# Samsonboadi/Image_to_pointCloud

Hardware: NVIDIA B200
Metric: depth_to_point_cloud_throughput (higher is better)
Workload: dtype f64

## Files before the change

image_to_pointcloud_b200/csrc/d2pc_device.cuh:

```cuda
#ifndef D2PC_DEVICE_CUH_
#define D2PC_DEVICE_CUH_

#include <cuda_runtime.h>
#include <stdint.h>

#include "d2pc_math.h"

namespace d2pc {

constexpr int kSampleSize = 8192;
constexpr int kSample2Size = 4096;
constexpr int kSortCap = 16384;
constexpr int kSelBits = 12;
constexpr int kScanThreads = 256;
constexpr int kScanPerThread = 32;
constexpr int kScanTile = kScanThreads * kScanPerThread;
constexpr int kSelThreads = 1024;
constexpr int kSelectThreads = 512;
constexpr int kEmitThreads = 256;
constexpr int kEmitPerThread = 4;
constexpr int kEmitTile = kEmitThreads * kEmitPerThread;
constexpr int kFbTargets = 4;
constexpr uint32_t kCandDivisor = 16;

struct Geom {
  int32_t H, W, C, h, w, step;
  int32_t nu, nv;
  uint32_t P;
  uint32_t N;
  uint32_t D;
  int32_t native;
  double scale_x, scale_y;
};

inline Geom make_geom(const D2pcConfig &c) {
  Geom g;
  g.H = c.img_h; g.W = c.img_w; g.C = c.img_c; g.h = c.dep_h; g.w = c.dep_w; g.step = c.step;
  g.nu = (c.img_w + c.step - 1) / c.step;
  g.nv = (c.img_h + c.step - 1) / c.step;
  g.P = (uint32_t)c.img_h * (uint32_t)c.img_w;
  g.N = (uint32_t)g.nu * (uint32_t)g.nv;
  g.D = (uint32_t)c.dep_h * (uint32_t)c.dep_w;
  g.native = (c.dep_h == c.img_h && c.dep_w == c.img_w) ? 1 : 0;
  g.scale_x = (double)c.dep_w / (double)c.img_w;
  g.scale_y = (double)c.dep_h / (double)c.img_h;
  return g;
}

struct __align__(256) FrameState {
  uint32_t brL[2], brU[2];
  uint32_t sample_ok;
  uint32_t below[2];
  uint32_t above1;
  uint32_t eqL[2];
  uint32_t inside[2];
  uint32_t eqU[2];
  uint32_t n_nonfinite, n_nan;
  alignas(8) uint32_t nqueue[2];
  uint32_t min_key, max_key;
  uint32_t sel_key[4];
  uint32_t sel_fail;
  uint32_t sel_done;
  uint32_t fb_prefix[kFbTargets];
  uint32_t fb_rank[kFbTargets];
  uint32_t fb_active;
  uint32_t fb_any_nan;
  int32_t mask_mode;
  float mask_lo, mask_hi;
  uint32_t emit_count;
  uint32_t bounds_min[3], bounds_max[3];
  alignas(128) NormParams norm;
  int32_t status;
};
static_assert(sizeof(NormParams) + 4 <= 128, "norm + status must share one 128-byte line");
constexpr int kStatusWord = (int)(sizeof(NormParams) / 4);

constexpr uint32_t kSelBins = 4096, kSelListCap = 1024;
struct __align__(256) SelShared {
  uint32_t counts[2][8];
  uint32_t scan_done;
  uint32_t a_done[2], c_done[2];
  uint32_t bin_ready[2];
  uint32_t bin[2][2], base[2][2], need[2][2], want[2][2], shared_bin[2], key[2][2];
  uint32_t mcount[2][2], mmin[2][2], mmax[2][2];
  uint32_t pad_[7];
  uint32_t members[2][2][kSelListCap];
  uint32_t hist[2][kSelBins];
};

struct __align__(8) TapEntry {
  int32_t i0c;
  float t;
};

constexpr int kSchedQueues = 32;
constexpr size_t kSchedBytes = 128 * (kSchedQueues + 1);

struct WsLayout {
  size_t state_off, cand_off, tile_off, fbhist_off, tap_off, sched_off, sel_off, resized_off, total;
  uint32_t cand_cap;
  uint32_t emit_tiles;
};

inline size_t align_up(size_t x, size_t a) { return (x + a - 1) / a * a; }

inline WsLayout make_layout(const D2pcConfig &c) {
  Geom g = make_geom(c);
  WsLayout L;
  uint32_t cap = g.P / kCandDivisor + 1;
  uint32_t small = g.P < (uint32_t)kSortCap ? g.P : (uint32_t)kSortCap;
  if (cap < small) cap = small;
  cap = (cap + 3u) & ~3u;
  L.cand_cap = cap;
  L.emit_tiles = (g.N + kEmitTile - 1) / kEmitTile;
  size_t off = 0;
  L.state_off = off;  off = align_up(off + sizeof(FrameState) * (size_t)c.batch, 256);
  L.cand_off = off;   off = align_up(off + (size_t)c.batch * 2 * cap * sizeof(uint32_t), 256);
  L.tile_off = off;   off = align_up(off + (size_t)c.batch * L.emit_tiles * sizeof(unsigned long long), 256);
  L.fbhist_off = off; off = align_up(off + (size_t)c.batch * kFbTargets * 256 * sizeof(uint32_t), 256);
  L.tap_off = off;    off = align_up(off + ((size_t)c.img_w + (size_t)c.img_h) * sizeof(TapEntry), 256);
  L.sched_off = off;  off = align_up(off + kSchedBytes + (size_t)c.batch * 64, 256);
  L.sel_off = off;    off = align_up(off + (size_t)c.batch * sizeof(SelShared), 256);
  L.resized_off = off;
  if (!g.native) off = align_up(off + (size_t)c.batch * g.P * sizeof(float), 256);
  L.total = off;
  return L;
}

struct KParams {
  Geom g;
  int32_t batch;
  const float *depth;
  FrameState *state;
  uint32_t *cand;
  unsigned long long *tile_state;
  uint32_t *fb_hist;
  const TapEntry *xtab, *ytab;
  SelShared *sel;
  uint32_t *sched;
  float *resized;
  uint32_t cand_cap, emit_tiles;
  int32_t force_fallback;
  int32_t hints;
};

constexpr int kHintScanKeep = 1;
constexpr int kHintEmitDepthFirst = 2;
constexpr int kHintStreamFirst = 4;
constexpr int kHintResizedKeep = 8;
constexpr int kHintPipeline = 15;

inline KParams make_kparams(const D2pcConfig &c, const float *d_depth, void *ws) {
  KParams k;
  WsLayout L = make_layout(c);
  char *base = (char *)ws;
  k.g = make_geom(c);
  k.batch = c.batch;
  k.depth = d_depth;
  k.state = (FrameState *)(base + L.state_off);
  k.cand = (uint32_t *)(base + L.cand_off);
  k.tile_state = (unsigned long long *)(base + L.tile_off);
  k.fb_hist = (uint32_t *)(base + L.fbhist_off);
  k.xtab = (const TapEntry *)(base + L.tap_off);
  k.ytab = k.xtab + c.img_w;
  k.sched = (uint32_t *)(base + L.sched_off);
  k.sel = (SelShared *)(base + L.sel_off);
  k.resized = k.g.native ? nullptr : (float *)(base + L.resized_off);
  k.cand_cap = L.cand_cap;
  k.emit_tiles = L.emit_tiles;
  k.force_fallback = c.force_fallback;
  k.hints = 0;
  return k;
}

inline KParams per_pixel_view(const KParams &kp) {
  KParams v = kp;
  if (!kp.g.native) {
    v.depth = kp.resized;
    v.g.D = kp.g.P;
    v.g.h = kp.g.H;
    v.g.w = kp.g.W;
    v.g.native = 1;
  }
  return v;
}

inline KParams slice_kparams(const KParams &kp, int b0, int nb, int ring_slot) {
  KParams s = kp;
  s.batch = nb;
  s.depth = kp.depth + (size_t)b0 * kp.g.D;
  s.state = kp.state + b0;
  s.cand = kp.cand + (size_t)b0 * 2 * kp.cand_cap;
  s.tile_state = kp.tile_state + (size_t)b0 * kp.emit_tiles;
  s.fb_hist = kp.fb_hist + (size_t)b0 * kFbTargets * 256;
  s.sel = kp.sel + b0;
  if (kp.resized) s.resized = kp.resized + (size_t)(ring_slot >= 0 ? ring_slot : b0) * kp.g.P;
  return s;
}

struct EmitArgs {
  const uint8_t *bgr;
  float *xyz, *rgb;
  uint32_t *count;
  PixelConsts pc;
  int32_t use_z, drop_nf, want_bounds;
  float z_min, z_max;
  uint32_t frame0;
};

int validate_config(const D2pcConfig *cfg);
int check_workspace(const D2pcConfig *cfg, const void *ws, size_t ws_bytes);
int stats_prepare();
int taps_launch(const KParams &kp, cudaStream_t st);
constexpr int kStatsSample = 1, kStatsScan = 2, kStatsSelect = 4, kStatsScanSelect = kStatsScan | kStatsSelect;
int stats_launch(KParams kp, cudaStream_t st, int phases);
int status_launch(const KParams &kp, int32_t *d_status, int32_t *d_any, cudaStream_t st);
EmitArgs make_emit_args(const D2pcConfig &cfg, const uint8_t *d_bgr, float *d_xyz, float *d_rgb, uint32_t *d_count);
EmitArgs slice_emit_args(const EmitArgs &ea, const Geom &g, int b0);
int emit_init_launch(const KParams &kp, cudaStream_t st);
int bounds_export_launch(const KParams &kp, float *d_bounds, cudaStream_t st);
int emit_validate(const D2pcConfig *cfg, const float *d_depth, const uint8_t *d_bgr, void *d_workspace,
                  size_t workspace_bytes, float *d_xyz, float *d_rgb, uint32_t *d_count, float *d_bounds);
int emit_launch(const D2pcConfig &cfg, const KParams &kp, const EmitArgs &ea, float *d_bounds, cudaStream_t st,
                int32_t smooth_k, const double *h_kernel, void *d_scratch);
int record_cuda_error(cudaError_t e);

#define D2PC_CHECK_LAUNCH()                                  \
  do {                                                       \
    cudaError_t e__ = cudaGetLastError();                    \
    if (e__ != cudaSuccess) return record_cuda_error(e__);   \
  } while (0)

#if defined(__CUDACC__)
__device__ __forceinline__ float4 ldg_stream_f4(const float *p) {
  float4 r;
  asm volatile("ld.global.nc.L1::no_allocate.v4.f32 {%0,%1,%2,%3}, [%4];"
               : "=f"(r.x), "=f"(r.y), "=f"(r.z), "=f"(r.w) : "l"(p));
  return r;
}
__device__ __forceinline__ uint64_t l2_policy(bool first, bool last) {
  uint64_t pf, pl, pn;
  asm("createpolicy.fractional.L2::evict_first.b64 %0, 1.0;" : "=l"(pf));
  asm("createpolicy.fractional.L2::evict_last.b64 %0, 1.0;" : "=l"(pl));
  asm("createpolicy.fractional.L2::evict_normal.b64 %0, 1.0;" : "=l"(pn));
  return first ? pf : (last ? pl : pn);
}
__device__ __forceinline__ float4 ldg_f4_pol(const float *p, uint64_t pol) {
  float4 r;
  asm volatile("ld.global.nc.L1::no_allocate.L2::cache_hint.v4.f32 {%0,%1,%2,%3}, [%4], %5;"
               : "=f"(r.x), "=f"(r.y), "=f"(r.z), "=f"(r.w) : "l"(p), "l"(pol));
  return r;
}
__device__ __forceinline__ uint32_t ldg_u32_pol(const void *p, uint64_t pol) {
  uint32_t r;
  asm volatile("ld.global.nc.L1::no_allocate.L2::cache_hint.u32 %0, [%1], %2;" : "=r"(r) : "l"(p), "l"(pol));
  return r;
}
__device__ __forceinline__ void stg_f4_pol(float *p, float4 v, uint64_t pol) {
  asm volatile("st.global.L2::cache_hint.v4.f32 [%0], {%1,%2,%3,%4}, %5;"
               :: "l"(p), "f"(v.x), "f"(v.y), "f"(v.z), "f"(v.w), "l"(pol) : "memory");
}
__device__ __forceinline__ void bulk_store_pol(void *gdst, uint32_t smem_addr, uint32_t bytes, uint64_t pol) {
  asm volatile("cp.async.bulk.global.shared::cta.bulk_group.L2::cache_hint [%0], [%1], %2, %3;"
               :: "l"(gdst), "r"(smem_addr), "r"(bytes), "l"(pol) : "memory");
}
__device__ __forceinline__ uint32_t ldg_stream_u32(const void *p) {
  uint32_t r;
  asm volatile("ld.global.nc.L1::no_allocate.u32 %0, [%1];" : "=r"(r) : "l"(p));
  return r;
}
__device__ __forceinline__ void stg_f1_pol(float *p, float v, uint64_t pol) {
  asm volatile("st.global.L2::cache_hint.f32 [%0], %1, %2;" :: "l"(p), "f"(v), "l"(pol) : "memory");
}
__device__ __forceinline__ void stg_stream_f4(float *p, float4 v) {
  asm volatile("st.global.cs.v4.f32 [%0], {%1,%2,%3,%4};"
               :: "l"(p), "f"(v.x), "f"(v.y), "f"(v.z), "f"(v.w) : "memory");
}
__device__ __forceinline__ void stg_stream_f1(float *p, float v) {
  asm volatile("st.global.cs.f32 [%0], %1;" :: "l"(p), "f"(v) : "memory");
}

__device__ __forceinline__ uint32_t warp_sum(uint32_t v) {
#pragma unroll
  for (int o = 16; o > 0; o >>= 1) v += __shfl_xor_sync(0xffffffffu, v, o);
  return v;
}
__device__ __forceinline__ uint32_t warp_min(uint32_t v) {
#pragma unroll
  for (int o = 16; o > 0; o >>= 1) v = min(v, __shfl_xor_sync(0xffffffffu, v, o));
  return v;
}
__device__ __forceinline__ uint32_t warp_max(uint32_t v) {
#pragma unroll
  for (int o = 16; o > 0; o >>= 1) v = max(v, __shfl_xor_sync(0xffffffffu, v, o));
  return v;
}

__device__ __forceinline__ void block_bitonic_sort(uint32_t *s, uint32_t n) {
  const uint32_t half = n >> 1;
  for (uint32_t k = 2; k <= n; k <<= 1) {
    for (uint32_t j = k >> 1; j > 0; j >>= 1) {
      for (uint32_t i = threadIdx.x; i < half; i += blockDim.x) {
        uint32_t a = ((i & ~(j - 1)) << 1) | (i & (j - 1));
        uint32_t b = a | j;
        uint32_t x = s[a], y = s[b];
        bool up = (a & k) == 0;
        if ((x > y) == up) { s[a] = y; s[b] = x; }
      }
      __syncthreads();
    }
  }
}

template <int T, int NBLOG, typename ForEach>
__device__ __forceinline__ bool block_hist_select(ForEach for_each, uint32_t lo0, uint32_t hi0,
                                                  const uint32_t (&rank)[T], uint32_t (&out)[T],
                                                  uint32_t *s_hist, uint32_t *s_res) {
  constexpr uint32_t NB = 1u << NBLOG;
  const int tid = threadIdx.x, nthr = blockDim.x;
  const int lane = tid & 31, warp = tid >> 5, nwarp = nthr >> 5;
  uint32_t lo[T], span[T], base[T];
  bool done[T];
#pragma unroll
  for (int t = 0; t < T; ++t) { lo[t] = lo0; span[t] = hi0 - lo0; base[t] = 0; done[t] = false; out[t] = 0; }
  bool shared_range = true, ok = true;
  uint32_t *s_warp = s_res + 2 * T;
  for (int level = 0; level < 6; ++level) {
    bool all_done = true;
#pragma unroll
    for (int t = 0; t < T; ++t) all_done = all_done && done[t];
    if (all_done) break;
    int shift[T];
#pragma unroll
    for (int t = 0; t < T; ++t) {
      const int bits = span[t] ? 32 - __clz(span[t]) : 0;
      shift[t] = bits > NBLOG ? bits - NBLOG : 0;
    }
    const int nh = shared_range ? 1 : T;
    for (uint32_t i = tid; i < (uint32_t)nh * NB; i += nthr) s_hist[i] = 0u;
    if (tid < 2 * T) s_res[tid] = 0xFFFFFFFFu;
    __syncthreads();
    if (shared_range) {
      for_each([&](uint32_t key) {
        const uint32_t d = key - lo[0];
        if (d <= span[0]) atomicAdd(&s_hist[d >> shift[0]], 1u);
      });
    } else {
      for_each([&](uint32_t key) {
#pragma unroll
        for (int t = 0; t < T; ++t) {
          const uint32_t d = key - lo[t];
          if (!done[t] && d <= span[t]) atomicAdd(&s_hist[t * NB + (d >> shift[t])], 1u);
        }
      });
    }
    __syncthreads();
    for (int h = 0; h < nh; ++h) {
      if (!shared_range && done[h]) continue;
      const uint32_t *hist = s_hist + (size_t)h * NB;
      constexpr int PER = 4;
      uint32_t carry = 0;
      for (uint32_t chunk = 0; chunk < NB; chunk += (uint32_t)nthr * PER) {
        const uint32_t b0 = chunk + (uint32_t)tid * PER;
        uint32_t c[PER], sum = 0;
#pragma unroll
        for (int i = 0; i < PER; ++i) { c[i] = (b0 + i < NB) ? hist[b0 + i] : 0u; sum += c[i]; }
        uint32_t incl = sum;
#pragma unroll
        for (int d = 1; d < 32; d <<= 1) {
          uint32_t y = __shfl_up_sync(0xffffffffu, incl, d);
          if (lane >= d) incl += y;
        }
        if (lane == 31) s_warp[warp] = incl;
        __syncthreads();
        uint32_t woff = 0, total = 0;
        for (int w = 0; w < nwarp; ++w) { const uint32_t x = s_warp[w]; if (w < warp) woff += x; total += x; }
        uint32_t pref = carry + woff + incl - sum;
#pragma unroll
        for (int i = 0; i < PER; ++i) {
#pragma unroll
          for (int t = 0; t < T; ++t) {
            const bool mine = shared_range ? !done[t] : (t == h);
            const uint32_t r = rank[t] - base[t];
            if (mine && c[i] && pref <= r && r < pref + c[i]) { s_res[2 * t] = b0 + i; s_res[2 * t + 1] = pref; }
          }
          pref += c[i];
        }
        carry += total;
        __syncthreads();
      }
    }
    __syncthreads();
#pragma unroll
    for (int t = 0; t < T; ++t) {
      if (done[t]) continue;
      const uint32_t bin = s_res[2 * t], pref = s_res[2 * t + 1];
      if (bin == 0xFFFFFFFFu) { ok = false; done[t] = true; continue; }
      base[t] += pref;
      lo[t] += bin << shift[t];
      span[t] = shift[t] ? ((1u << shift[t]) - 1u) : 0u;
      if (shift[t] == 0) { done[t] = true; out[t] = lo[t]; }
    }
    shared_range = false;
    __syncthreads();
  }
  return ok;
}

constexpr int kFastBinsLog = 12;
constexpr uint32_t kFastBins = 1u << kFastBinsLog;
constexpr uint32_t kFastListCap = 1024;

__device__ __forceinline__ int fast_shift(uint32_t span) {
  const int bits = span ? 32 - __clz(span) : 0;
  return bits > kFastBinsLog ? bits - kFastBinsLog : 0;
}

template <int T, bool GLOBAL = false>
__device__ __forceinline__ void block_locate(const uint32_t *s_hist, const uint32_t (&rank)[T], const bool (&want)[T],
                                             uint32_t (&bin)[T], uint32_t (&base)[T], uint32_t *s_warp,
                                             uint32_t *s_res) {
  const int tid = threadIdx.x, lane = tid & 31, warp = tid >> 5, nwarp = blockDim.x >> 5;
  const int per = (int)(kFastBins / blockDim.x);
  if (tid < 2 * T) s_res[tid] = 0xFFFFFFFFu;
  const uint32_t b0 = (uint32_t)tid * (uint32_t)per;
  uint32_t sum = 0;
  for (int i = 0; i < per; i += 4) {
    const uint4 c = GLOBAL ? __ldcg(reinterpret_cast<const uint4 *>(s_hist + b0 + i))
                           : *reinterpret_cast<const uint4 *>(s_hist + b0 + i);
    sum += c.x + c.y + c.z + c.w;
  }
  uint32_t incl = sum;
#pragma unroll
  for (int d = 1; d < 32; d <<= 1) {
    const uint32_t y = __shfl_up_sync(0xffffffffu, incl, d);
    if (lane >= d) incl += y;
  }
  if (lane == 31) s_warp[warp] = incl;
  __syncthreads();
  if (warp == 0) {
    const uint32_t x = lane < nwarp ? s_warp[lane] : 0u;
    uint32_t in2 = x;
#pragma unroll
    for (int d = 1; d < 32; d <<= 1) {
      const uint32_t y = __shfl_up_sync(0xffffffffu, in2, d);
      if (lane >= d) in2 += y;
    }
    __syncwarp();
    s_warp[lane] = in2 - x;
  }
  __syncthreads();
  uint32_t pref = s_warp[warp] + incl - sum;
  bool mine = false;
#pragma unroll
  for (int t = 0; t < T; ++t) mine = mine || (want[t] && sum && pref <= rank[t] && rank[t] < pref + sum);
  if (mine) {
    for (int i = 0; i < per; ++i) {
      const uint32_t c = GLOBAL ? __ldcg(s_hist + b0 + i) : s_hist[b0 + i];
#pragma unroll
      for (int t = 0; t < T; ++t)
        if (want[t] && c && pref <= rank[t] && rank[t] < pref + c) { s_res[2 * t] = b0 + i; s_res[2 * t + 1] = pref; }
      pref += c;
    }
  }
  __syncthreads();
#pragma unroll
  for (int t = 0; t < T; ++t) { bin[t] = s_res[2 * t]; base[t] = s_res[2 * t + 1]; }
}

__device__ __forceinline__ void block_pick(const uint32_t *list, uint32_t n, uint32_t r, uint32_t *s_out) {
  for (uint32_t i = threadIdx.x; i < n; i += blockDim.x) {
    const uint32_t k = list[i];
    uint32_t smaller = 0, equal = 0;
    for (uint32_t j = 0; j < n; ++j) {
      const uint32_t x = list[j];
      smaller += x < k ? 1u : 0u;
      equal += x == k ? 1u : 0u;
    }
    if (smaller <= r && r < smaller + equal) *s_out = k;
  }
}

__device__ __forceinline__ uint32_t hash_u32(uint32_t x) {
  x ^= x >> 16; x *= 0x7feb352du; x ^= x >> 15; x *= 0x846ca68bu; x ^= x >> 16;
  return x;
}

__device__ __forceinline__ float bilinear_taps(const float *src, int32_t src_w, TapEntry tx, TapEntry ty) {
  const int32_t x0 = tx.i0c & 0x7FFFFFFF, y0 = ty.i0c & 0x7FFFFFFF;
  const bool cx = tx.i0c < 0, cy = ty.i0c < 0;
  const float *row0 = src + (size_t)y0 * src_w;
  const float a0 = __ldg(row0 + x0);
  float r0 = a0;
  if (!cx) r0 = fmaf(__ldg(row0 + x0 + 1) - a0, tx.t, a0);
  if (cy) return (cx && is_inf_f32(r0)) ? nan_f32() : r0;
  const float *row1 = row0 + src_w;
  const float a1 = __ldg(row1 + x0);
  float r1 = a1;
  if (!cx) r1 = fmaf(__ldg(row1 + x0 + 1) - a1, tx.t, a1);
  return fmaf(r1 - r0, ty.t, r0);
}

template <bool NATIVE>
__device__ __forceinline__ float depth_at(const float *frame, const KParams &kp, uint32_t p) {
  if (NATIVE) {
    return __ldg(frame + p);
  } else {
    const uint32_t v = p / (uint32_t)kp.g.W;
    const uint32_t u = p - v * (uint32_t)kp.g.W;
    return bilinear_taps(frame, kp.g.w, kp.xtab[u], kp.ytab[v]);
  }
}
#endif

}
#endif
```

image_to_pointcloud_b200/csrc/d2pc_emit.cu:

```cuda
#include <stdlib.h>

#include "d2pc_emit_dev.cuh"

namespace d2pc {


__global__ void __launch_bounds__(32) mask_prepare_kernel(KParams kp, EmitArgs ea, int pc_simple) {
  FrameState *fs = kp.state + blockIdx.x;
  if (fs->status != D2PC_FRAME_READY) return;
  const bool by_depth = ea.use_z && fs->norm.simple && pc_simple;
  float lo_f = 1.0f, hi_f = 0.0f;
  if (by_depth) {
    const NormParams sn = fs->norm;
    const uint32_t kmin = float_to_key(-3.402823466e38f), kmax = float_to_key(3.402823466e38f);
    const bool dec = ea.pc.invert != 0;
    auto rising = [&](uint32_t k) {
      const float z = simple_z32(key_to_float(k), sn, ea.pc);
      return dec ? (z <= ea.z_max) : (z >= ea.z_min);
    };
    auto fallen = [&](uint32_t k) {
      const float z = simple_z32(key_to_float(k), sn, ea.pc);
      return !(dec ? (z >= ea.z_min) : (z <= ea.z_max));
    };
    if (rising(kmax) && !fallen(kmin)) {
      const uint32_t a = warp_first_true(kmin, kmax, rising);
      const uint32_t f = fallen(kmax) ? warp_first_true(kmin, kmax, fallen) : kmax + 1u;
      if (f > a) { lo_f = key_to_float(a); hi_f = key_to_float(f - 1u); }
    }
  }
  if (threadIdx.x == 0) {
    fs->mask_mode = by_depth ? 1 : 0;
    fs->mask_lo = lo_f;
    fs->mask_hi = hi_f;
  }
}

constexpr int kCountWarps = 8;
template <int STEP>
__global__ void __launch_bounds__(kCountWarps * 32, 6) mask_count_kernel(KParams kp, EmitArgs ea, uint32_t tiles_per_frame,
                                                                     uint32_t total_tiles, unsigned long long magic_w) {
  const int lane = threadIdx.x & 31, warp = threadIdx.x >> 5;
  const uint32_t t = blockIdx.x * (uint32_t)kCountWarps + (uint32_t)warp;
  if (t >= total_tiles) return;
  const uint32_t b = t / tiles_per_frame, tile = t - b * tiles_per_frame;
  const FrameState *fs = kp.state + b;
  const uint32_t N = kp.g.N, W = (uint32_t)kp.g.W, NU = (uint32_t)kp.g.nu;
  const uint32_t tile_base = tile * (uint32_t)kEmitTile;
  const float *frame = kp.depth + (size_t)b * kp.g.P;
  const int32_t status = fs->status;
  auto load_group = [&](int j, bool *ok) -> float4 {
    const uint32_t p0 = tile_base + 4u * (uint32_t)(j * 32 + lane);
    *ok = p0 < N;
    if (!*ok) return make_float4(0.0f, 0.0f, 0.0f, 0.0f);
    if (STEP == 1) return ldg_stream_f4(frame + p0);
    const uint32_t jv = (uint32_t)(((unsigned long long)p0 * magic_w) >> 40), ju = p0 - jv * NU;
    const float *src = frame + (size_t)(jv * (uint32_t)STEP) * W + ju * (uint32_t)STEP;
    if (STEP == 2) {
      const float4 da = ldg_stream_f4(src), db = ldg_stream_f4(src + 4);
      return make_float4(da.x, da.z, db.x, db.z);
    }
    return make_float4(__ldg(src), __ldg(src + 4), __ldg(src + 8), __ldg(src + 12));
  };
  float4 r[8];
  bool ok[8];
#pragma unroll
  for (int j = 0; j < 8; ++j) r[j] = load_group(j, &ok[j]);
  uint32_t cnt = 0;
  const MaskParams mp = load_mask(fs);
  if (status != D2PC_FRAME_READY) return;
  const bool by_depth = !ea.use_z || mp.mode == 1;
  if (by_depth) {
#pragma unroll
    for (int j = 0; j < 8; ++j)
      if (ok[j]) {
        cnt += mask_keep(r[j].x, 0.0f, mp, ea) ? 1u : 0u;
        cnt += mask_keep(r[j].y, 0.0f, mp, ea) ? 1u : 0u;
        cnt += mask_keep(r[j].z, 0.0f, mp, ea) ? 1u : 0u;
        cnt += mask_keep(r[j].w, 0.0f, mp, ea) ? 1u : 0u;
      }
  } else {
    const NormParams np_ = fs->norm;
#pragma unroll 1
    for (int j = 0; j < 8; ++j) {
      bool okj;
      const float4 q = load_group(j, &okj);
      if (!okj) continue;
      const float raw[4] = {q.x, q.y, q.z, q.w};
#pragma unroll
      for (int k = 0; k < 4; ++k) {
        const double n = normalised_depth(raw[k], np_, ea.pc.invert);
        cnt += mask_keep(raw[k], (float)(n * ea.pc.scale), mp, ea) ? 1u : 0u;
      }
    }
  }
  cnt = warp_sum(cnt);
  if (lane == 0) kp.tile_state[(size_t)b * tiles_per_frame + tile] = (unsigned long long)cnt;
}

__global__ void __launch_bounds__(1024) mask_offsets_kernel(KParams kp, uint32_t *count) {
  __shared__ uint32_t s_warp[32];
  __shared__ uint32_t s_carry;
  const int b = blockIdx.x, tid = threadIdx.x, lane = tid & 31, warp = tid >> 5;
  if (kp.state[b].status != D2PC_FRAME_READY) return;
  unsigned long long *ts = kp.tile_state + (size_t)b * kp.emit_tiles;
  if (tid == 0) s_carry = 0;
  __syncthreads();
  for (uint32_t base = 0; base < kp.emit_tiles; base += 1024u) {
    const uint32_t i = base + (uint32_t)tid;
    const uint32_t c = i < kp.emit_tiles ? (uint32_t)ts[i] : 0u;
    uint32_t incl = c;
#pragma unroll
    for (int d = 1; d < 32; d <<= 1) {
      uint32_t y = __shfl_up_sync(0xffffffffu, incl, d);
      if (lane >= d) incl += y;
    }
    if (lane == 31) s_warp[warp] = incl;
    __syncthreads();
    uint32_t woff = 0, total = 0;
    for (int w = 0; w < 32; ++w) { const uint32_t x = s_warp[w]; if (w < warp) woff += x; total += x; }
    const uint32_t excl = s_carry + woff + incl - c;
    if (i < kp.emit_tiles) ts[i] = ((unsigned long long)excl << 32) | (unsigned long long)c;
    __syncthreads();
    if (tid == 0) s_carry += total;
    __syncthreads();
  }
  if (tid == 0) count[b] = s_carry;
}

template <int STEP, bool MASK, int MIN_BLOCKS>
static int launch_emit_fast(const KParams &kp, const EmitArgs &ea, const FastArgs &fa, cudaStream_t st) {
  const size_t smem = kEmitStageBytes;
  if (ea.want_bounds) emit_fast_kernel<STEP, MASK, true, 5><<<fa.total_tiles, kEmitThreads, smem, st>>>(kp, ea, fa);
  else emit_fast_kernel<STEP, MASK, false, MIN_BLOCKS><<<fa.total_tiles, kEmitThreads, smem, st>>>(kp, ea, fa);
  return D2PC_OK;
}

struct SmoothArgs {
  const double *rows;
  int32_t ksize;
  double k[D2PC_MAX_SMOOTH_KSIZE];
};

__device__ __forceinline__ int32_t reflect101(int32_t i, int32_t n) {
  if (n == 1) return 0;
  while (i < 0 || i >= n) {
    if (i < 0) i = -i;
    if (i >= n) i = 2 * (n - 1) - i;
  }
  return i;
}

__device__ __forceinline__ double smooth_column(const SmoothArgs &sa, const double *rows, int32_t u, int32_t v,
                                                int32_t W, int32_t H) {
  const int32_t r = sa.ksize >> 1;
  double s = sa.k[r] * rows[(size_t)v * W + u];
  for (int32_t j = 1; j <= r; ++j) {
    const double a = rows[(size_t)reflect101(v + j, H) * W + u];
    const double b = rows[(size_t)reflect101(v - j, H) * W + u];
    s = s + sa.k[r + j] * (a + b);
  }
  return s;
}

__global__ void __launch_bounds__(256) smooth_norm_kernel(KParams kp, int32_t invert, double *out) {
  const int b = blockIdx.y;
  const FrameState *fs = kp.state + b;
  if (fs->status != D2PC_FRAME_READY) return;
  const NormParams np_ = fs->norm;
  const float *frame = kp.depth + (size_t)b * kp.g.D;
  for (uint32_t p = blockIdx.x * blockDim.x + threadIdx.x; p < kp.g.P; p += gridDim.x * blockDim.x)
    out[(size_t)b * kp.g.P + p] = normalised_depth(frame[p], np_, invert);
}

__global__ void __launch_bounds__(256) smooth_rows_kernel(KParams kp, SmoothArgs sa, const double *in, double *out) {
  const int b = blockIdx.y;
  if (kp.state[b].status != D2PC_FRAME_READY) return;
  const int32_t W = kp.g.W, r = sa.ksize >> 1, wb = W - (W & 3);
  const double *src = in + (size_t)b * kp.g.P;
  for (uint32_t p = blockIdx.x * blockDim.x + threadIdx.x; p < kp.g.P; p += gridDim.x * blockDim.x) {
    const int32_t v = (int32_t)(p / (uint32_t)W), u = (int32_t)(p - (uint32_t)v * (uint32_t)W);
    const double *row = src + (size_t)v * W;
    double s = sa.k[0] * row[reflect101(u - r, W)];
    if (u < wb) {
      for (int32_t j = 1; j < sa.ksize; ++j) s = fma(sa.k[j], row[reflect101(u + j - r, W)], s);
    } else {
      for (int32_t j = 1; j < sa.ksize; ++j) s = s + sa.k[j] * row[reflect101(u + j - r, W)];
    }
    out[(size_t)b * kp.g.P + p] = s;
  }
}

template <bool NATIVE, bool MASK, bool SMOOTH>
__global__ void __launch_bounds__(kEmitThreads) emit_generic_kernel(KParams kp, EmitArgs ea, SmoothArgs sa) {
  __shared__ __align__(16) float s_xyz[kEmitTile * 3 + 4];
  __shared__ __align__(16) float s_rgb[kEmitTile * 3 + 4];
  __shared__ uint32_t s_warp[kEmitThreads / 32];
  __shared__ uint32_t s_prefix;
  __shared__ uint32_t s_b[6][kEmitThreads / 32];
  const int b = blockIdx.y, tid = threadIdx.x, lane = tid & 31, warp = tid >> 5;
  const int tile = blockIdx.x;
  FrameState *fs = kp.state + b;
  if (fs->status != D2PC_FRAME_READY) return;
  const NormParams np_ = fs->norm;
  const MaskParams mp = load_mask(fs);
  const Geom &g = kp.g;
  const float *frame = kp.depth + (size_t)b * g.D;
  const uint32_t tile_base = (uint32_t)tile * (uint32_t)kEmitTile;
  const uint32_t i0 = tile_base + (uint32_t)kEmitPerThread * (uint32_t)tid;
  float o[12], col[12];
  bool keep[4];
  uint32_t mn[3] = {0xFFFFFFFFu, 0xFFFFFFFFu, 0xFFFFFFFFu}, mx[3] = {0u, 0u, 0u};
  uint32_t my_cnt = 0;
#pragma unroll
  for (int k = 0; k < 4; ++k) {
    const uint32_t i = i0 + k;
    keep[k] = false;
    if (i >= g.N) continue;
    const uint32_t jv = i / (uint32_t)g.nu, ju = i - jv * (uint32_t)g.nu;
    const uint32_t u = ju * (uint32_t)g.step, v = jv * (uint32_t)g.step;
    const uint32_t p = v * (uint32_t)g.W + u;
    const float raw = depth_at<NATIVE>(frame, kp, p);
    const double n = SMOOTH ? smooth_column(sa, sa.rows + (size_t)b * g.P, (int32_t)u, (int32_t)v, g.W, g.H)
                            : normalised_depth(raw, np_, ea.pc.invert);
    back_project(n, (int32_t)u, (int32_t)v, ea.pc, &o[3 * k], &o[3 * k + 1], &o[3 * k + 2]);
    if (g.C >= 3) {
      const uint8_t *cp = ea.bgr + ((size_t)b * g.P + p) * (size_t)g.C;
      col[3 * k + 0] = (float)cp[2];
      col[3 * k + 1] = (float)cp[1];
      col[3 * k + 2] = (float)cp[0];
    } else {
      col[3 * k + 0] = col[3 * k + 1] = col[3 * k + 2] = 128.0f;
    }
    bool kk = true;
    if (MASK) kk = mask_keep(raw, o[3 * k + 2], mp, ea);
    keep[k] = kk;
    if (kk) {
      my_cnt++;
      if (ea.want_bounds) {
#pragma unroll
        for (int c = 0; c < 3; ++c) {
          uint32_t key = float_to_key(o[3 * k + c]);
          mn[c] = min(mn[c], key); mx[c] = max(mx[c], key);
        }
      }
    }
  }

  uint32_t incl = my_cnt;
#pragma unroll
  for (int d = 1; d < 32; d <<= 1) {
    uint32_t y = __shfl_up_sync(0xffffffffu, incl, d);
    if (lane >= d) incl += y;
  }
  if (lane == 31) s_warp[warp] = incl;
  __syncthreads();
  uint32_t warp_off = 0, total = 0;
#pragma unroll
  for (int w = 0; w < kEmitThreads / 32; ++w) {
    uint32_t c = s_warp[w];
    if (w < warp) warp_off += c;
    total += c;
  }
  uint32_t local = warp_off + incl - my_cnt;

  uint32_t dest_row;
  if (MASK) {
    volatile unsigned long long *ts = kp.tile_state + (size_t)b * kp.emit_tiles;
    if (warp == 0) {
      if (lane == 0 && tile > 0) ts[tile] = (1ull << 32) | (unsigned long long)total;
      uint32_t ex = (tile == 0) ? 0u : lookback_exclusive(ts, tile);
      if (lane == 0) {
        ts[tile] = (2ull << 32) | (unsigned long long)(ex + total);
        s_prefix = ex;
        if (tile == (int)kp.emit_tiles - 1) ea.count[b] = ex + total;
      }
    }
    __syncthreads();
    dest_row = s_prefix;
  } else {
    dest_row = tile_base;
    if (tile == 0 && tid == 0) ea.count[b] = g.N;
  }

  const size_t g0 = ((size_t)((uint32_t)b + ea.frame0) * g.N + dest_row) * 3;
  const uint32_t s_off = (uint32_t)(g0 & 3);
#pragma unroll
  for (int k = 0; k < 4; ++k) {
    if (!keep[k]) continue;
    const uint32_t w = s_off + 3u * local;
    s_xyz[w] = o[3 * k]; s_xyz[w + 1] = o[3 * k + 1]; s_xyz[w + 2] = o[3 * k + 2];
    s_rgb[w] = col[3 * k]; s_rgb[w + 1] = col[3 * k + 1]; s_rgb[w + 2] = col[3 * k + 2];
    local++;
  }
  asm volatile("fence.proxy.async.shared::cta;" ::: "memory");
  __syncthreads();
  const uint64_t pol_o = l2_policy((kp.hints & kHintStreamFirst) != 0, false);
  copy_out(s_xyz, s_off, total * 3u, ea.xyz, g0, pol_o);
  copy_out(s_rgb, s_off, total * 3u, ea.rgb, g0, pol_o);
  if (ea.want_bounds) reduce_bounds(fs, mn, mx, s_b);
}

__global__ void emit_init_kernel(KParams kp, int clear_tiles) {
  const int b = blockIdx.x;
  FrameState *fs = kp.state + b;
  if (threadIdx.x == 0) {
    fs->emit_count = 0;
    for (int c = 0; c < 3; ++c) { fs->bounds_min[c] = 0xFFFFFFFFu; fs->bounds_max[c] = 0u; }
  }
  if (clear_tiles) {
    unsigned long long *ts = kp.tile_state + (size_t)b * kp.emit_tiles;
    for (uint32_t i = threadIdx.x; i < kp.emit_tiles; i += blockDim.x) ts[i] = 0ull;
  }
}

__global__ void bounds_export_kernel(KParams kp, float *d_bounds) {
  const int i = blockIdx.x * blockDim.x + threadIdx.x;
  if (i >= kp.batch * 6) return;
  const int b = i / 6, c = i % 6;
  const FrameState &fs = kp.state[b];
  const bool empty = fs.bounds_min[0] == 0xFFFFFFFFu && fs.bounds_max[0] == 0u;
  uint32_t key = c < 3 ? fs.bounds_min[c] : fs.bounds_max[c - 3];
  d_bounds[i] = empty ? nan_f32() : key_to_float(key);
}

}

using namespace d2pc;

namespace d2pc {

EmitArgs make_emit_args(const D2pcConfig &cfg, const uint8_t *d_bgr, float *d_xyz, float *d_rgb, uint32_t *d_count) {
  EmitArgs ea;
  ea.bgr = d_bgr; ea.xyz = d_xyz; ea.rgb = d_rgb; ea.count = d_count;
  ea.pc.scale = cfg.depth_scale; ea.pc.cx = cfg.cx; ea.pc.cy = cfg.cy; ea.pc.f = cfg.f;
  ea.pc.inv_f = 1.0 / cfg.f; ea.pc.invert = cfg.invert;
  ea.use_z = cfg.use_z_range; ea.drop_nf = cfg.drop_nonfinite; ea.want_bounds = cfg.want_bounds;
  ea.z_min = cfg.z_min; ea.z_max = cfg.z_max;
  ea.frame0 = 0;
  return ea;
}

EmitArgs slice_emit_args(const EmitArgs &ea, const Geom &g, int b0) {
  EmitArgs s = ea;
  if (ea.bgr) s.bgr = ea.bgr + (size_t)b0 * g.P * (size_t)g.C;
  s.frame0 = ea.frame0 + (uint32_t)b0;
  s.count = ea.count + b0;
  return s;
}

int emit_launch(const D2pcConfig &cfg, const KParams &kp_in, const EmitArgs &ea, float *d_bounds, cudaStream_t st,
                int32_t smooth_k, const double *h_kernel, void *d_scratch) {
  const bool smooth = smooth_k > 0;
  const KParams kp = per_pixel_view(kp_in);
  const int nb = kp.batch;
  const bool mask = cfg.use_z_range || cfg.drop_nonfinite;
  dim3 grid(kp.emit_tiles, nb);
  SmoothArgs sa;
  sa.rows = nullptr;
  sa.ksize = 0;
  if (smooth) {
    double *n64 = (double *)d_scratch, *rows = n64 + (size_t)nb * kp.g.P;
    sa.rows = rows;
    sa.ksize = smooth_k;
    for (int i = 0; i < smooth_k; ++i) sa.k[i] = h_kernel[i];
    dim3 sg(148 * 4, nb);
    smooth_norm_kernel<<<sg, 256, 0, st>>>(kp, cfg.invert, n64);
    D2PC_CHECK_LAUNCH();
    smooth_rows_kernel<<<sg, 256, 0, st>>>(kp, sa, n64, rows);
    D2PC_CHECK_LAUNCH();
  }
  const bool fast = !smooth && cfg.img_c == 3 && (cfg.img_w % (4 * cfg.step)) == 0 &&
                    (((uintptr_t)kp.depth & 15u) == 0u) && (((uintptr_t)ea.bgr & 3u) == 0u) && (kp.g.N & 3u) == 0u &&
                    ((unsigned long long)kp.g.N * (unsigned long long)kp.g.nu < (1ull << 40));
  if (mask || cfg.want_bounds) {
    emit_init_kernel<<<nb, 256, 0, st>>>(kp, (mask && !fast) ? 1 : 0);
    D2PC_CHECK_LAUNCH();
  }
  if (mask) {
    mask_prepare_kernel<<<nb, 32, 0, st>>>(kp, ea, (!smooth && consts_simple(ea.pc)) ? 1 : 0);
    D2PC_CHECK_LAUNCH();
  }
  if (fast) {
    FastArgs fa;
    fa.tiles_per_frame = kp.emit_tiles;
    fa.total_tiles = kp.emit_tiles * (uint32_t)nb;
    fa.batch = (uint32_t)nb;
    fa.magic_w = ((1ull << 40) + (unsigned long long)kp.g.nu - 1ull) / (unsigned long long)kp.g.nu;
    fa.pc_simple = consts_simple(ea.pc) ? 1 : 0;
    if (mask) {
      const uint32_t total_tiles = fa.total_tiles, cg = (total_tiles + kCountWarps - 1) / kCountWarps;
      if (cfg.step == 1) mask_count_kernel<1><<<cg, kCountWarps * 32, 0, st>>>(kp, ea, kp.emit_tiles, total_tiles, fa.magic_w);
      else if (cfg.step == 2) mask_count_kernel<2><<<cg, kCountWarps * 32, 0, st>>>(kp, ea, kp.emit_tiles, total_tiles, fa.magic_w);
      else mask_count_kernel<4><<<cg, kCountWarps * 32, 0, st>>>(kp, ea, kp.emit_tiles, total_tiles, fa.magic_w);
      D2PC_CHECK_LAUNCH();
      mask_offsets_kernel<<<nb, 1024, 0, st>>>(kp, ea.count);
      D2PC_CHECK_LAUNCH();
    }
    int rcl;
    if (mask) rcl = cfg.step == 1 ? launch_emit_fast<1, true, 5>(kp, ea, fa, st)
                  : cfg.step == 2 ? launch_emit_fast<2, true, 5>(kp, ea, fa, st)
                                  : launch_emit_fast<4, true, 5>(kp, ea, fa, st);
    else if (cfg.step == 1) rcl = launch_emit_fast<1, false, 6>(kp, ea, fa, st);
    else if (cfg.step == 2) rcl = launch_emit_fast<2, false, 6>(kp, ea, fa, st);
    else rcl = launch_emit_fast<4, false, 6>(kp, ea, fa, st);
    if (rcl) return rcl;
  } else if (smooth) {
    if (mask) emit_generic_kernel<true, true, true><<<grid, kEmitThreads, 0, st>>>(kp, ea, sa);
    else emit_generic_kernel<true, false, true><<<grid, kEmitThreads, 0, st>>>(kp, ea, sa);
  } else {
    if (mask) emit_generic_kernel<true, true, false><<<grid, kEmitThreads, 0, st>>>(kp, ea, sa);
    else emit_generic_kernel<true, false, false><<<grid, kEmitThreads, 0, st>>>(kp, ea, sa);
  }
  D2PC_CHECK_LAUNCH();
  if (cfg.want_bounds) {
    bounds_export_kernel<<<(nb * 6 + 127) / 128, 128, 0, st>>>(kp, d_bounds);
    D2PC_CHECK_LAUNCH();
  }
  return D2PC_OK;
}

int emit_init_launch(const KParams &kp, cudaStream_t st) {
  emit_init_kernel<<<kp.batch, 256, 0, st>>>(kp, 0);
  D2PC_CHECK_LAUNCH();
  return D2PC_OK;
}

int bounds_export_launch(const KParams &kp, float *d_bounds, cudaStream_t st) {
  bounds_export_kernel<<<(kp.batch * 6 + 127) / 128, 128, 0, st>>>(kp, d_bounds);
  D2PC_CHECK_LAUNCH();
  return D2PC_OK;
}

int emit_validate(const D2pcConfig *cfg, const float *d_depth, const uint8_t *d_bgr, void *d_workspace,
                  size_t workspace_bytes, float *d_xyz, float *d_rgb, uint32_t *d_count, float *d_bounds) {
  int rc = validate_config(cfg);
  if (rc) return rc;
  if (!d_workspace || !d_depth || !d_xyz || !d_rgb || !d_count) return D2PC_ERR_INVALID_ARGUMENT;
  if (cfg->img_c >= 3 && !d_bgr) return D2PC_ERR_INVALID_ARGUMENT;
  if (cfg->want_bounds && !d_bounds) return D2PC_ERR_INVALID_ARGUMENT;
  if (workspace_bytes < make_layout(*cfg).total) return D2PC_ERR_WORKSPACE_TOO_SMALL;
  if ((((uintptr_t)d_xyz | (uintptr_t)d_rgb) & 15u) != 0) return D2PC_ERR_INVALID_ARGUMENT;
  return D2PC_OK;
}

}

static int emit_impl(const D2pcConfig *cfg, const float *d_depth, const uint8_t *d_bgr, void *d_workspace,
                     size_t workspace_bytes, float *d_xyz, float *d_rgb, uint32_t *d_count, float *d_bounds,
                     void *stream, int32_t smooth_k, const double *h_kernel, void *d_scratch, size_t scratch_bytes) {
  int rc = emit_validate(cfg, d_depth, d_bgr, d_workspace, workspace_bytes, d_xyz, d_rgb, d_count, d_bounds);
  if (rc) return rc;
  if (smooth_k > 0) {
    if ((smooth_k & 1) == 0 || smooth_k < 3 || smooth_k > D2PC_MAX_SMOOTH_KSIZE) return D2PC_ERR_UNSUPPORTED;
    if (!h_kernel || !d_scratch) return D2PC_ERR_INVALID_ARGUMENT;
    const size_t need = 2 * (size_t)cfg->batch * (size_t)cfg->img_h * (size_t)cfg->img_w * sizeof(double);
    if (scratch_bytes < need) return D2PC_ERR_WORKSPACE_TOO_SMALL;
    if (((uintptr_t)d_scratch & 15u) != 0) return D2PC_ERR_INVALID_ARGUMENT;
  }
  const KParams kp = make_kparams(*cfg, d_depth, d_workspace);
  const EmitArgs ea = make_emit_args(*cfg, d_bgr, d_xyz, d_rgb, d_count);
  return emit_launch(*cfg, kp, ea, d_bounds, (cudaStream_t)stream, smooth_k, h_kernel, d_scratch);
}

__global__ void __launch_bounds__(256) preview_kernel(KParams kp, int32_t invert, const uint8_t *lut, uint8_t *out) {
  __shared__ uint8_t s_lut[256 * 3];
  for (int i = threadIdx.x; i < 256 * 3; i += blockDim.x) s_lut[i] = lut[i];
  __syncthreads();
  const int b = blockIdx.y;
  const FrameState *fs = kp.state + b;
  if (fs->status != D2PC_FRAME_READY) return;
  const NormParams np_ = fs->norm;
  const float *frame = kp.depth + (size_t)b * kp.g.D;
  uint8_t *dst = out + (size_t)b * kp.g.P * 3;
  for (uint32_t p = blockIdx.x * blockDim.x + threadIdx.x; p < kp.g.P; p += gridDim.x * blockDim.x) {
    const double n = normalised_depth(frame[p], np_, invert);
    const uint32_t idx = (np_.branch == D2PC_BRANCH_PCT) ? (uint32_t)(int32_t)(n * 255.0)
                                                        : (uint32_t)(int32_t)((float)n * 255.0f);
    const uint32_t j = (idx & 255u) * 3u;
    dst[3 * (size_t)p + 0] = s_lut[j];
    dst[3 * (size_t)p + 1] = s_lut[j + 1];
    dst[3 * (size_t)p + 2] = s_lut[j + 2];
  }
}

extern "C" int d2pc_preview_enqueue(const D2pcConfig *cfg, const float *d_depth, void *d_workspace,
                                    size_t workspace_bytes, const uint8_t *d_lut_bgr, uint8_t *d_out_bgr,
                                    void *stream) {
  int rc = validate_config(cfg);
  if (rc) return rc;
  if (!d_depth || !d_workspace || !d_lut_bgr || !d_out_bgr) return D2PC_ERR_INVALID_ARGUMENT;
  if (cfg->dep_h != cfg->img_h || cfg->dep_w != cfg->img_w) return D2PC_ERR_INVALID_ARGUMENT;
  if (workspace_bytes < make_layout(*cfg).total) return D2PC_ERR_WORKSPACE_TOO_SMALL;
  KParams kp = make_kparams(*cfg, d_depth, d_workspace);
  preview_kernel<<<dim3(148 * 2, cfg->batch), 256, 0, (cudaStream_t)stream>>>(kp, cfg->invert, d_lut_bgr, d_out_bgr);
  D2PC_CHECK_LAUNCH();
  return D2PC_OK;
}

extern "C" int d2pc_emit_enqueue(const D2pcConfig *cfg, const float *d_depth, const uint8_t *d_bgr,
                                 void *d_workspace, size_t workspace_bytes, float *d_xyz,
                                 float *d_rgb, uint32_t *d_count, float *d_bounds, void *stream) {
  return emit_impl(cfg, d_depth, d_bgr, d_workspace, workspace_bytes, d_xyz, d_rgb, d_count, d_bounds, stream, 0,
                   nullptr, nullptr, 0);
}

extern "C" int d2pc_smooth_scratch_bytes(const D2pcConfig *cfg, size_t *bytes) {
  int rc = validate_config(cfg);
  if (rc) return rc;
  if (!bytes) return D2PC_ERR_INVALID_ARGUMENT;
  *bytes = 2 * (size_t)cfg->batch * (size_t)cfg->img_h * (size_t)cfg->img_w * sizeof(double);
  return D2PC_OK;
}

extern "C" int d2pc_emit_smooth_enqueue(const D2pcConfig *cfg, const float *d_depth, const uint8_t *d_bgr,
                                        void *d_workspace, size_t workspace_bytes, int32_t ksize,
                                        const double *h_kernel, void *d_scratch, size_t scratch_bytes,
                                        float *d_xyz, float *d_rgb, uint32_t *d_count, float *d_bounds,
                                        void *stream) {
  if (ksize <= 0) return D2PC_ERR_INVALID_ARGUMENT;
  return emit_impl(cfg, d_depth, d_bgr, d_workspace, workspace_bytes, d_xyz, d_rgb, d_count, d_bounds, stream, ksize,
                   h_kernel, d_scratch, scratch_bytes);
}
```

image_to_pointcloud_b200/csrc/d2pc_emit_dev.cuh:

```cuda
#ifndef D2PC_EMIT_DEV_CUH_
#define D2PC_EMIT_DEV_CUH_

#include "d2pc_device.cuh"

namespace d2pc {

__device__ __forceinline__ void stage_f4(float *s, float a, float b, float c, float d) {
  *reinterpret_cast<float4 *>(s) = make_float4(a, b, c, d);
}

__device__ __forceinline__ void reduce_bounds(FrameState *fs, uint32_t mn[3], uint32_t mx[3],
                                              uint32_t (*s_b)[kEmitThreads / 32]) {
  const int lane = threadIdx.x & 31, warp = threadIdx.x >> 5;
#pragma unroll
  for (int c = 0; c < 3; ++c) {
    uint32_t a = warp_min(mn[c]), b = warp_max(mx[c]);
    if (lane == 0) { s_b[c][warp] = a; s_b[3 + c][warp] = b; }
  }
  __syncthreads();
  if (threadIdx.x < 6) {
    const int c = threadIdx.x;
    uint32_t r = s_b[c][0];
    for (int w = 1; w < kEmitThreads / 32; ++w) r = c < 3 ? min(r, s_b[c][w]) : max(r, s_b[c][w]);
    if (c < 3) { if (r != 0xFFFFFFFFu) atomicMin(&fs->bounds_min[c], r); }
    else       { if (r != 0u) atomicMax(&fs->bounds_max[c - 3], r); }
  }
}

__device__ __forceinline__ void copy_out(const float *s, uint32_t s_off, uint32_t n_f, float *gbase,
                                         size_t g0, uint64_t pol) {
  float *galigned = gbase + (g0 - s_off);
  const uint32_t span = s_off + n_f;
  const uint32_t w_first = s_off ? 4u : 0u;
  const uint32_t w_last = span & ~3u;
  const uint32_t tid = threadIdx.x;
  if (w_last > w_first) {
    if (tid == 0) {
      const uint32_t sa = (uint32_t)__cvta_generic_to_shared(s + w_first);
      bulk_store_pol(galigned + w_first, sa, (w_last - w_first) * 4u, pol);
      asm volatile("cp.async.bulk.commit_group;" ::: "memory");
      asm volatile("cp.async.bulk.wait_group.read 0;" ::: "memory");
    }
    if (tid >= 32 && tid < 36) {
      const uint32_t w = s_off + (tid - 32);
      if (w < w_first && w < span) stg_stream_f1(galigned + w, s[w]);
    } else if (tid >= 64 && tid < 68) {
      const uint32_t w = w_last + (tid - 64);
      if (w < span) stg_stream_f1(galigned + w, s[w]);
    }
  } else {
    if (tid < 8) {
      const uint32_t w = s_off + tid;
      if (w < span) stg_stream_f1(galigned + w, s[w]);
    }
  }
}

__device__ __forceinline__ float byte_to_float(uint32_t w, uint32_t selector) {
  return __uint_as_float(__byte_perm(w, 0x4B000000u, selector)) - 8388608.0f;
}
#define D2PC_B0 0x7440u
#define D2PC_B1 0x7441u
#define D2PC_B2 0x7442u
#define D2PC_B3 0x7443u

__device__ __forceinline__ uint32_t lookback_exclusive(volatile unsigned long long *ts, int tile) {
  const int lane = threadIdx.x & 31;
  uint32_t exclusive = 0;
  int base_idx = tile - 1;
  while (true) {
    const int idx = base_idx - lane;
    unsigned long long st = (idx >= 0) ? ts[idx] : ((2ull << 32) | 0ull);
    const uint32_t flag = (uint32_t)(st >> 32);
    const unsigned inval = __ballot_sync(0xffffffffu, flag == 0u);
    const unsigned incl = __ballot_sync(0xffffffffu, flag == 2u);
    const int first_incl = incl ? (__ffs(incl) - 1) : 32;
    const unsigned need = first_incl >= 31 ? 0xffffffffu : ((2u << first_incl) - 1u);
    if (inval & need) continue;
    uint32_t val = (lane <= first_incl) ? (uint32_t)st : 0u;
    exclusive += warp_sum(val);
    if (first_incl < 32) break;
    base_idx -= 32;
  }
  return exclusive;
}

struct MaskParams {
  int32_t mode;
  float lo, hi;
};
__device__ __forceinline__ MaskParams load_mask(const FrameState *fs) {
  MaskParams m;
  m.mode = fs->mask_mode; m.lo = fs->mask_lo; m.hi = fs->mask_hi;
  return m;
}
__device__ __forceinline__ bool mask_keep_v(float raw, float z32, const MaskParams &m, int32_t use_z, int32_t drop_nf,
                                            float z_min, float z_max) {
  bool kk = true;
  if (use_z) {
    if (m.mode == 1) kk = (raw >= m.lo) && (raw <= m.hi);
    else kk = (z32 >= z_min) && (z32 <= z_max);
  }
  if (drop_nf && !is_finite_f32(raw)) kk = false;
  return kk;
}
__device__ __forceinline__ bool mask_keep(float raw, float z32, const MaskParams &m, const EmitArgs &ea) {
  return mask_keep_v(raw, z32, m, ea.use_z, ea.drop_nf, ea.z_min, ea.z_max);
}

template <typename Pred>
__device__ __forceinline__ uint32_t warp_first_true(uint32_t lo, uint32_t hi, Pred pred) {
  const int lane = threadIdx.x & 31;
  while (lo < hi) {
    const unsigned long long span = (unsigned long long)(hi - lo);
    const uint32_t k = lo + (uint32_t)((span * (unsigned long long)(lane + 1)) / 33ull);
    const bool p = pred(k);
    const unsigned m = __ballot_sync(0xffffffffu, p);
    if (m == 0u) {
      lo = __shfl_sync(0xffffffffu, k, 31) + 1u;
    } else {
      const int j = __ffs(m) - 1;
      hi = __shfl_sync(0xffffffffu, k, j);
      if (j > 0) lo = __shfl_sync(0xffffffffu, k, j - 1) + 1u;
    }
  }
  return lo;
}

struct FastArgs {
  uint32_t tiles_per_frame, total_tiles, batch;
  unsigned long long magic_w;
  int32_t pc_simple;
};

template <bool COHERENT>
__device__ __forceinline__ NormParams load_norm(const FrameState *fs) {
  if (!COHERENT) return fs->norm;
  NormParams np_;
  static_assert(sizeof(NormParams) % 8 == 0, "NormParams is copied as 8-byte words");
  const unsigned long long *src = reinterpret_cast<const unsigned long long *>(&fs->norm);
  unsigned long long *dst = reinterpret_cast<unsigned long long *>(&np_);
#pragma unroll
  for (int i = 0; i < (int)(sizeof(NormParams) / 8); ++i) dst[i] = __ldcg(src + i);
  return np_;
}

constexpr size_t kEmitStageBytes = 2 * ((size_t)kEmitTile * 3 + 4) * sizeof(float);
struct EmitSmall {
  uint32_t warp[kEmitThreads / 32];
  uint32_t b[6][kEmitThreads / 32];
  uint32_t dest;
};

template <int STEP, bool MASK, bool BOUNDS, typename NormFn>
__device__ __forceinline__ bool emit_fast_tile(const KParams &kp, const EmitArgs &ea, const FastArgs &fa, uint32_t b,
                                               uint32_t tile, float *s_stage, EmitSmall &es, NormFn norm_fn) {
  uint32_t *s_warp = es.warp;
  uint32_t (*s_b)[kEmitThreads / 32] = es.b;
  const int tid = threadIdx.x, lane = tid & 31, warp = tid >> 5;
  const uint32_t P = kp.g.N, W = (uint32_t)kp.g.W, NU = (uint32_t)kp.g.nu;
  FrameState *fs = kp.state + b;
  const uint32_t tile_base = tile * (uint32_t)kEmitTile;
  const uint32_t p0 = tile_base + 4u * (uint32_t)tid;
  float *s_xyz = s_stage;
  float *s_rgb = s_stage + (kEmitTile * 3 + 4);
  float o[12];
  uint32_t c0 = 0, c1 = 0, c2 = 0;
  bool keep[4] = {false, false, false, false};
  uint32_t my_cnt = 0;
  uint32_t mn[3] = {0xFFFFFFFFu, 0xFFFFFFFFu, 0xFFFFFFFFu}, mx[3] = {0u, 0u, 0u};
  float raw[4] = {0.0f, 0.0f, 0.0f, 0.0f};
  uint32_t u = 0, v = 0;
  if (p0 < P) {
    const uint32_t jv = (uint32_t)(((unsigned long long)p0 * fa.magic_w) >> 40), ju = p0 - jv * NU;
    v = jv * (uint32_t)STEP; u = ju * (uint32_t)STEP;
    const size_t pix = (size_t)b * kp.g.P + (size_t)v * W + u;
    const uint8_t *cp = ea.bgr + pix * 3;
    const uint64_t pol_d = l2_policy((kp.hints & kHintEmitDepthFirst) != 0, false);
    const uint64_t pol_c = l2_policy((kp.hints & kHintStreamFirst) != 0, false);
    if (STEP == 1) {
      const float4 d4 = ldg_f4_pol(kp.depth + pix, pol_d);
      raw[0] = d4.x; raw[1] = d4.y; raw[2] = d4.z; raw[3] = d4.w;
      c0 = ldg_u32_pol(cp, pol_c); c1 = ldg_u32_pol(cp + 4, pol_c); c2 = ldg_u32_pol(cp + 8, pol_c);
    } else if (STEP == 2) {
      const float4 da = ldg_f4_pol(kp.depth + pix, pol_d), db = ldg_f4_pol(kp.depth + pix + 4, pol_d);
      raw[0] = da.x; raw[1] = da.z; raw[2] = db.x; raw[3] = db.z;
      const uint32_t w0 = ldg_u32_pol(cp, pol_c), w1 = ldg_u32_pol(cp + 4, pol_c), w2 = ldg_u32_pol(cp + 8, pol_c);
      const uint32_t w3 = ldg_u32_pol(cp + 12, pol_c), w4 = ldg_u32_pol(cp + 16, pol_c), w5 = ldg_u32_pol(cp + 20, pol_c);
      const uint32_t px1 = __byte_perm(w1, w2, 0x0432);
      const uint32_t px3 = __byte_perm(w4, w5, 0x0432);
      c0 = __byte_perm(w0, px1, 0x4210);
      c1 = __byte_perm(px1, w3, 0x5421);
      c2 = __byte_perm(w3, px3, 0x6542);
    } else {
      raw[0] = __ldg(kp.depth + pix); raw[1] = __ldg(kp.depth + pix + 4);
      raw[2] = __ldg(kp.depth + pix + 8); raw[3] = __ldg(kp.depth + pix + 12);
      const uint32_t q0 = ldg_u32_pol(cp, pol_c), q1 = ldg_u32_pol(cp + 12, pol_c), q2 = ldg_u32_pol(cp + 24, pol_c),
                     q3 = ldg_u32_pol(cp + 36, pol_c);
      c0 = __byte_perm(q0, q1, 0x4210);
      c1 = __byte_perm(q1, q2, 0x5421);
      c2 = __byte_perm(q2, q3, 0x6542);
    }
    if (!MASK) {
      float *sr = s_rgb + 12 * tid;
      stage_f4(sr, byte_to_float(c0, D2PC_B2), byte_to_float(c0, D2PC_B1), byte_to_float(c0, D2PC_B0),
               byte_to_float(c1, D2PC_B1));
      stage_f4(sr + 4, byte_to_float(c1, D2PC_B0), byte_to_float(c0, D2PC_B3), byte_to_float(c2, D2PC_B0),
               byte_to_float(c1, D2PC_B3));
      stage_f4(sr + 8, byte_to_float(c1, D2PC_B2), byte_to_float(c2, D2PC_B3), byte_to_float(c2, D2PC_B2),
               byte_to_float(c2, D2PC_B1));
    }
  }
  if (MASK && tid == 0) es.dest = (uint32_t)(__ldg(kp.tile_state + (size_t)b * kp.emit_tiles + tile) >> 32);
  const NormParams *np_src = norm_fn();
  if (np_src == nullptr) return false;
  if (p0 < P) {
    const NormParams np_ = *np_src;
    const MaskParams mp = load_mask(fs);
    if (np_.simple && fa.pc_simple) {
      const double ux0 = (double)(int32_t)u - ea.pc.cx;
      const double vy = (double)(int32_t)v - ea.pc.cy;
#pragma unroll
      for (int k = 0; k < 4; ++k)
        simple_point(raw[k], ux0 + (double)(k * STEP), vy, np_, ea.pc, &o[3 * k], &o[3 * k + 1], &o[3 * k + 2]);
    } else {
#pragma unroll
      for (int k = 0; k < 4; ++k) {
        const double n = normalised_depth(raw[k], np_, ea.pc.invert);
        back_project(n, (int32_t)u + k * STEP, (int32_t)v, ea.pc, &o[3 * k], &o[3 * k + 1], &o[3 * k + 2]);
      }
    }
#pragma unroll
    for (int k = 0; k < 4; ++k) {
      bool kk = true;
      if (MASK) kk = mask_keep(raw[k], o[3 * k + 2], mp, ea);
      keep[k] = kk;
      my_cnt += kk ? 1u : 0u;
      if (BOUNDS && kk) {
#pragma unroll
        for (int c = 0; c < 3; ++c) {
          uint32_t key = float_to_key(o[3 * k + c]);
          mn[c] = min(mn[c], key); mx[c] = max(mx[c], key);
        }
      }
    }
  }
  if (!MASK) {
    if (p0 < P) {
      float *sx = s_xyz + 12 * tid;
      stage_f4(sx, o[0], o[1], o[2], o[3]);
      stage_f4(sx + 4, o[4], o[5], o[6], o[7]);
      stage_f4(sx + 8, o[8], o[9], o[10], o[11]);
    }
    asm volatile("fence.proxy.async.shared::cta;" ::: "memory");
    __syncthreads();
    const uint32_t rows = min((uint32_t)kEmitTile, P - tile_base);
    const size_t g0 = ((size_t)(b + ea.frame0) * kp.g.N + tile_base) * 3;
    if (tid == 0) {
      const uint32_t bytes = rows * 12u;
      const uint32_t sx = (uint32_t)__cvta_generic_to_shared(s_xyz), sr = (uint32_t)__cvta_generic_to_shared(s_rgb);
      const uint64_t pol_o = l2_policy((kp.hints & kHintStreamFirst) != 0, false);
      bulk_store_pol(ea.xyz + g0, sx, bytes, pol_o);
      bulk_store_pol(ea.rgb + g0, sr, bytes, pol_o);
      asm volatile("cp.async.bulk.commit_group;" ::: "memory");
      asm volatile("cp.async.bulk.wait_group.read 0;" ::: "memory");
      if (tile == 0) ea.count[b] = kp.g.N;
    }
  } else {
    uint32_t incl = my_cnt;
#pragma unroll
    for (int d = 1; d < 32; d <<= 1) {
      uint32_t y = __shfl_up_sync(0xffffffffu, incl, d);
      if (lane >= d) incl += y;
    }
    if (lane == 31) s_warp[warp] = incl;
    __syncthreads();
    uint32_t warp_off = 0, total = 0;
#pragma unroll
    for (int w = 0; w < kEmitThreads / 32; ++w) {
      uint32_t c = s_warp[w];
      if (w < warp) warp_off += c;
      total += c;
    }
    uint32_t local = warp_off + incl - my_cnt;
    const uint32_t dest_row = es.dest;
    const size_t g0 = ((size_t)(b + ea.frame0) * kp.g.N + dest_row) * 3;
    const uint32_t s_off = (uint32_t)(g0 & 3);
    const float col[12] = {
        byte_to_float(c0, D2PC_B2), byte_to_float(c0, D2PC_B1), byte_to_float(c0, D2PC_B0),
        byte_to_float(c1, D2PC_B1), byte_to_float(c1, D2PC_B0), byte_to_float(c0, D2PC_B3),
        byte_to_float(c2, D2PC_B0), byte_to_float(c1, D2PC_B3), byte_to_float(c1, D2PC_B2),
        byte_to_float(c2, D2PC_B3), byte_to_float(c2, D2PC_B2), byte_to_float(c2, D2PC_B1)};
#pragma unroll
    for (int k = 0; k < 4; ++k) {
      if (!keep[k]) continue;
      const uint32_t w = s_off + 3u * local;
      s_xyz[w] = o[3 * k]; s_xyz[w + 1] = o[3 * k + 1]; s_xyz[w + 2] = o[3 * k + 2];
      s_rgb[w] = col[3 * k]; s_rgb[w + 1] = col[3 * k + 1]; s_rgb[w + 2] = col[3 * k + 2];
      local++;
    }
    asm volatile("fence.proxy.async.shared::cta;" ::: "memory");
    __syncthreads();
    const uint64_t pol_o = l2_policy((kp.hints & kHintStreamFirst) != 0, false);
    copy_out(s_xyz, s_off, total * 3u, ea.xyz, g0, pol_o);
    copy_out(s_rgb, s_off, total * 3u, ea.rgb, g0, pol_o);
  }
  if (BOUNDS) reduce_bounds(fs, mn, mx, s_b);
  return true;
}

template <int STEP, bool MASK, bool BOUNDS, int MIN_BLOCKS>
__global__ void __launch_bounds__(kEmitThreads, MIN_BLOCKS) emit_fast_kernel(KParams kp, EmitArgs ea, FastArgs fa) {
  extern __shared__ __align__(16) float s_stage[];
  __shared__ EmitSmall es;
  const uint32_t t = blockIdx.x;
  const uint32_t b = t / fa.tiles_per_frame, tile = t - b * fa.tiles_per_frame;
  if (kp.state[b].status != D2PC_FRAME_READY) return;
  emit_fast_tile<STEP, MASK, BOUNDS>(kp, ea, fa, b, tile, s_stage, es, [&]() { return &kp.state[b].norm; });
}


}
#endif
```

image_to_pointcloud_b200/csrc/d2pc_path.cu:

```cuda
#include <stdlib.h>
#include <string.h>

#include <vector>

#include "d2pc_emit_dev.cuh"
#include "d2pc_stats_dev.cuh"

using namespace d2pc;

namespace d2pc {

__global__ void sched_reset_kernel(KParams kp) {
  if (threadIdx.x <= kSchedQueues) kp.sched[32 * threadIdx.x] = 0u;
}
int sched_reset_launch(const KParams &kp, cudaStream_t st) {
  sched_reset_kernel<<<1, 64, 0, st>>>(kp);
  D2PC_CHECK_LAUNCH();
  return D2PC_OK;
}

struct SchedParams {
  int32_t F, D;
  uint32_t ns, ne, R;
  uint32_t K;
  uint32_t skip;
  uint32_t nq;
  uint32_t group_items, total_items;
  int32_t vec_ok;
};

constexpr int kPathMinBlocks = 6;
__device__ __forceinline__ unsigned long long global_ns() {
  unsigned long long t;
  asm volatile("mov.u64 %0, %globaltimer;" : "=l"(t));
  return t;
}
__device__ __forceinline__ unsigned long long *trace_slot(const KParams &kp, uint32_t f, int k) {
  return reinterpret_cast<unsigned long long *>(reinterpret_cast<unsigned char *>(kp.sched) + kSchedBytes) + (size_t)f * 8 + k;
}

constexpr int kPathScanPT = 16;

template <bool BOUNDS, bool TRACE>
__global__ void __launch_bounds__(kEmitThreads, kPathMinBlocks) path_kernel(KParams kp, EmitArgs ea, FastArgs fa,
                                                                           SchedParams sp) {
  extern __shared__ __align__(16) unsigned char s_dyn[];
  __shared__ EmitSmall s_emit;
  __shared__ SelPartSmall s_sel;
  __shared__ uint32_t s_go;
  __shared__ NormParams s_norm;
  const int tid = threadIdx.x;
  uint32_t *abort_flag = kp.sched + 32u * kSchedQueues;
  const uint32_t item = blockIdx.x;
  const uint32_t g = item / sp.group_items, i = item - g * sp.group_items;
  if (i < 2u * sp.K) {
    if (g < 1u || g > (uint32_t)sp.F || (sp.skip & 1u)) return;
    const int f = (int)g - 1;
    const uint32_t br = i / sp.K, k = i - br * sp.K;
    if (tid == 0) s_go = spin_until(&kp.sel[f].scan_done, abort_flag, [&](uint32_t v) { return v >= sp.ns; }) ? 1u : 0u;
    __syncthreads();
    if (!s_go) return;
    if (TRACE && tid == 0 && k == 0u) *trace_slot(kp, f, 2 + 2 * (int)br) = global_ns();
    select_part(kp, f, (int)br, k, sp.K, reinterpret_cast<float *>(s_dyn), kSliceCap, s_sel,
                [&](const uint32_t *p, auto pred) { return spin_until(p, abort_flag, pred); });
    if (TRACE) {
      __syncthreads();
      if (tid == 0) atomicMax(trace_slot(kp, f, 3 + 2 * (int)br), global_ns());
    }
    return;
  }
  const uint32_t j = i - 2u * sp.K, q = j / (sp.R + 1u), r = j - q * (sp.R + 1u);
  if (r == 0u) {
    if (g >= (uint32_t)sp.F || (sp.skip & 2u)) return;
    if (TRACE && tid == 0) atomicMin(trace_slot(kp, g, 0), global_ns());
    scan_tile<kPathScanPT>(kp, (int)g, q, sp.vec_ok, *reinterpret_cast<ScanTileSmemT<kPathScanPT> *>(s_dyn));
    __syncthreads();
    if (tid == 0) {
      __threadfence();
      atomicAdd(&kp.sel[g].scan_done, 1u);
      if (TRACE) atomicMax(trace_slot(kp, g, 1), global_ns());
    }
    return;
  }
  const uint32_t e = q * sp.R + (r - 1u);
  if (g < (uint32_t)sp.D || e >= sp.ne || (sp.skip & 4u)) return;
  const uint32_t f = g - (uint32_t)sp.D;
  if (f >= (uint32_t)sp.F) return;
  if (TRACE && tid == 0) atomicMin(trace_slot(kp, f, 6), global_ns());
  auto norm_fn = [&]() -> const NormParams * {
    const uint32_t *line = reinterpret_cast<const uint32_t *>(&kp.state[f].norm);
    uint32_t go = 0u;
    for (int attempt = 0; attempt < 2 && go == 0u; ++attempt) {
      if (tid < 32) {
        const uint32_t w = ld_relaxed_u32(line + tid);
        const uint32_t st = __shfl_sync(0xffffffffu, w, kStatusWord);
        if (st == (uint32_t)D2PC_FRAME_READY && tid < kStatusWord) reinterpret_cast<uint32_t *>(&s_norm)[tid] = w;
        if (tid == 0) s_go = st == (uint32_t)D2PC_FRAME_READY ? 1u : (st == (uint32_t)D2PC_FRAME_PENDING ? 0u : 3u);
      }
      __syncthreads();
      go = s_go;
      if (go == 0u) {
        __syncthreads();
        if (tid == 0) s_go = spin_until(line + kStatusWord, abort_flag, [&](uint32_t x) { return x != (uint32_t)D2PC_FRAME_PENDING; }) ? 0u : 2u;
        __syncthreads();
        go = s_go;
        __syncthreads();
      }
    }
    return go == 1u ? &s_norm : nullptr;
  };
  emit_fast_tile<1, false, BOUNDS>(kp, ea, fa, f, e, reinterpret_cast<float *>(s_dyn), s_emit, norm_fn);
  if (TRACE) {
    __syncthreads();
    if (tid == 0) atomicMax(trace_slot(kp, f, 7), global_ns());
  }
}

}

constexpr int kMaxAux = 8, kMaxEmit = 4;

struct D2pcPath {
  int device;
  cudaStream_t s_cap;
  cudaStream_t s_aux[kMaxAux];
  cudaStream_t s_emit[kMaxEmit];
  std::vector<cudaEvent_t> events;
  cudaGraphExec_t exec;
  std::vector<unsigned char> key;
};

namespace {

struct PathArgs {
  D2pcConfig cfg;
  const float *d_depth;
  const uint8_t *d_bgr;
  void *d_workspace;
  size_t workspace_bytes;
  float *d_xyz, *d_rgb;
  uint32_t *d_count;
  float *d_bounds;
  int32_t *d_status, *d_any_fallback;
  int32_t sub_batch, lookahead, flags;
};

int ensure_events(D2pcPath *p, size_t n) {
  while (p->events.size() < n) {
    cudaEvent_t e;
    cudaError_t err = cudaEventCreateWithFlags(&e, cudaEventDisableTiming);
    if (err != cudaSuccess) return record_cuda_error(err);
    p->events.push_back(e);
  }
  return D2PC_OK;
}

#define PATH_CUDA(x)                                         \
  do {                                                       \
    cudaError_t e__ = (x);                                   \
    if (e__ != cudaSuccess) return record_cuda_error(e__);   \
  } while (0)

int path_kernel_supported(const D2pcConfig &cfg, const KParams &kp, const EmitArgs &ea) {
  const bool mask = cfg.use_z_range || cfg.drop_nonfinite;
  return kp.g.native && cfg.step == 1 && !mask && cfg.img_c == 3 && (cfg.img_w % 4) == 0 &&
         (((uintptr_t)kp.depth & 15u) == 0u) && (((uintptr_t)ea.bgr & 3u) == 0u) && (kp.g.N & 3u) == 0u &&
         ((unsigned long long)kp.g.N * (unsigned long long)kp.g.nu < (1ull << 40)) && kp.g.P > (uint32_t)kSortCap;
}

size_t path_kernel_smem() {
  size_t m = sizeof(ScanTileSmemT<kPathScanPT>);
  if (kEmitStageBytes > m) m = kEmitStageBytes;
  return m;
}

static int env_int(const char *name, int dflt, int lo, int hi);

int path_ordered(const PathArgs &a, cudaStream_t st) {
  const D2pcConfig &cfg = a.cfg;
  KParams kp = make_kparams(cfg, a.d_depth, a.d_workspace);
  kp.hints = (a.flags & D2PC_PATH_NO_L2_HINTS) ? 0 : (kHintScanKeep | kHintEmitDepthFirst | kHintStreamFirst);
  if (const char *h = getenv("D2PC_HINTS")) kp.hints = atoi(h);
  const EmitArgs ea = make_emit_args(cfg, a.d_bgr, a.d_xyz, a.d_rgb, a.d_count);
  int rc;
  const int skip = env_int("D2PC_PATH_SKIP", 0, 0, 15);
  if (skip) {
    if ((rc = sched_reset_launch(kp, st)) != D2PC_OK) return rc;
  } else if ((rc = stats_launch(kp, st, kStatsSample)) != D2PC_OK) return rc;
  if (cfg.want_bounds) {
    if ((rc = emit_init_launch(kp, st)) != D2PC_OK) return rc;
  }
  FastArgs fa;
  fa.tiles_per_frame = kp.emit_tiles;
  fa.total_tiles = kp.emit_tiles * (uint32_t)cfg.batch;
  fa.batch = (uint32_t)cfg.batch;
  fa.magic_w = ((1ull << 40) + (unsigned long long)kp.g.nu - 1ull) / (unsigned long long)kp.g.nu;
  fa.pc_simple = consts_simple(ea.pc) ? 1 : 0;
  SchedParams sp;
  sp.F = cfg.batch;
  sp.D = env_int("D2PC_PATH_D", a.lookahead > 0 ? a.lookahead : 3, 2, 64);
  sp.ns = (kp.g.P + kPathScanPT * kScanThreads - 1) / (kPathScanPT * kScanThreads);
  sp.ne = kp.emit_tiles;
  sp.R = (sp.ne + sp.ns - 1) / sp.ns;
  {
    const uint32_t k = (kp.cand_cap + kSliceCap - 1u) / kSliceCap;
    sp.K = (uint32_t)env_int("D2PC_PATH_K", (int)(k < 8u ? 8u : (k > 64u ? 64u : k)), 1, 64);
  }
  sp.skip = (uint32_t)skip;
  sp.nq = (uint32_t)env_int("D2PC_PATH_NQ", 16, 1, kSchedQueues);
  sp.group_items = 2u * sp.K + sp.ns * (sp.R + 1u);
  const unsigned long long total = (unsigned long long)(sp.F + sp.D) * sp.group_items;
  if (total >= 0xFFFF0000ull) return D2PC_ERR_UNSUPPORTED;
  sp.total_items = (uint32_t)total;
  sp.vec_ok = ((kp.g.P & 3u) == 0u) && (((uintptr_t)kp.depth & 15u) == 0u);
  const size_t smem = path_kernel_smem();
  const bool trace = env_int("D2PC_PATH_TRACE", 0, 0, 1) != 0;
  void (*kern)(KParams, EmitArgs, FastArgs, SchedParams) =
      cfg.want_bounds ? (trace ? path_kernel<true, true> : path_kernel<true, false>)
                      : (trace ? path_kernel<false, true> : path_kernel<false, false>);
  PATH_CUDA(cudaFuncSetAttribute(kern, cudaFuncAttributeMaxDynamicSharedMemorySize, (int)smem));
  kern<<<sp.total_items, kEmitThreads, smem, st>>>(kp, ea, fa, sp);
  D2PC_CHECK_LAUNCH();
  if (cfg.want_bounds) {
    if ((rc = bounds_export_launch(kp, a.d_bounds, st)) != D2PC_OK) return rc;
  }
  if (a.d_status || a.d_any_fallback) {
    if ((rc = status_launch(kp, a.d_status, a.d_any_fallback, st)) != D2PC_OK) return rc;
  }
  return D2PC_OK;
}

static int env_int(const char *name, int dflt, int lo, int hi) {
  const char *v = getenv(name);
  int x = v ? atoi(v) : dflt;
  return x < lo ? lo : (x > hi ? hi : x);
}

int path_body(D2pcPath *p, const PathArgs &a, cudaStream_t s_main) {
  const D2pcConfig &cfg = a.cfg;
  KParams kp = make_kparams(cfg, a.d_depth, a.d_workspace);
  const bool generic = !kp.g.native && resize_is_generic(kp.g.h, kp.g.w);
  const int B = cfg.batch, S = generic ? B : a.sub_batch;
  const int n_sub = (B + S - 1) / S;
  const bool overlap = !(a.flags & D2PC_PATH_NO_OVERLAP) && n_sub > 1;
  const int window = (a.lookahead > 0 ? a.lookahead : 1) + 1;
  const int n_aux = overlap ? env_int("D2PC_PATH_AUX", window < kMaxAux ? window : kMaxAux, 1, kMaxAux) : 1;
  const int n_emit = overlap ? env_int("D2PC_PATH_EMIT", 2, 1, kMaxEmit) : 1;
  const bool sample_first = n_sub > 1 && env_int("D2PC_PATH_SAMPLE_FIRST", 1, 0, 1) != 0;
  const bool ring = kp.resized != nullptr && n_sub > 1;
  kp.hints = (a.flags & D2PC_PATH_NO_L2_HINTS) ? 0 : (n_sub > 1 ? kHintPipeline : (kHintEmitDepthFirst | kHintStreamFirst));
  if (ring) kp.hints &= ~kHintEmitDepthFirst;
  if (const char *h = getenv("D2PC_HINTS")) kp.hints = atoi(h);
  const EmitArgs ea = make_emit_args(cfg, a.d_bgr, a.d_xyz, a.d_rgb, a.d_count);
  int rc;
  if ((rc = ensure_events(p, 1 + 3 * (size_t)n_sub)) != D2PC_OK) return rc;
  cudaEvent_t ev_fork = p->events[0];
  cudaEvent_t *ev_stats = &p->events[1], *ev_emit = &p->events[1 + n_sub], *ev_scan = &p->events[1 + 2 * n_sub];
  const bool stagger = overlap && n_aux > 1 && env_int("D2PC_PATH_STAGGER", 0, 0, 1) != 0;
  if ((rc = taps_launch(kp, s_main)) != D2PC_OK) return rc;
  if (sample_first) {
    if ((rc = stats_launch(kp, s_main, kStatsSample)) != D2PC_OK) return rc;
  }
  if (overlap) {
    PATH_CUDA(cudaEventRecord(ev_fork, s_main));
    for (int i = 0; i < n_aux; ++i) PATH_CUDA(cudaStreamWaitEvent(p->s_aux[i], ev_fork, 0));
    if (n_emit > 1)
      for (int i = 0; i < n_emit; ++i) PATH_CUDA(cudaStreamWaitEvent(p->s_emit[i], ev_fork, 0));
  }
  for (int k = 0; k < n_sub; ++k) {
    const int b0 = k * S, nb = (b0 + S <= B) ? S : B - b0;
    const KParams ks = slice_kparams(kp, b0, nb, ring ? (k % window) * S : -1);
    cudaStream_t s_stats = overlap ? p->s_aux[k % n_aux] : s_main;
    cudaStream_t s_em = (overlap && n_emit > 1) ? p->s_emit[k % n_emit] : s_main;
    if (overlap && k >= window) PATH_CUDA(cudaStreamWaitEvent(s_stats, ev_emit[k - window], 0));
    if (stagger) {
      if (!sample_first && (rc = stats_launch(ks, s_stats, kStatsSample)) != D2PC_OK) return rc;
      if (k > 0) PATH_CUDA(cudaStreamWaitEvent(s_stats, ev_scan[k - 1], 0));
      if ((rc = stats_launch(ks, s_stats, kStatsScan)) != D2PC_OK) return rc;
      PATH_CUDA(cudaEventRecord(ev_scan[k], s_stats));
      if ((rc = stats_launch(ks, s_stats, kStatsSelect)) != D2PC_OK) return rc;
    } else if ((rc = stats_launch(ks, s_stats, sample_first ? kStatsScanSelect : (kStatsSample | kStatsScanSelect))) != D2PC_OK)
      return rc;
    if (overlap) {
      PATH_CUDA(cudaEventRecord(ev_stats[k], s_stats));
      PATH_CUDA(cudaStreamWaitEvent(s_em, ev_stats[k], 0));
    }
    if ((rc = emit_launch(cfg, ks, slice_emit_args(ea, kp.g, b0), a.d_bounds ? a.d_bounds + 6 * (size_t)b0 : nullptr,
                          s_em, 0, nullptr, nullptr)) != D2PC_OK)
      return rc;
    if (overlap) PATH_CUDA(cudaEventRecord(ev_emit[k], s_em));
  }
  if (overlap && n_emit > 1) {
    for (int k = n_sub - 1; k >= 0 && k >= n_sub - n_emit; --k) PATH_CUDA(cudaStreamWaitEvent(s_main, ev_emit[k], 0));
  }
  if (a.d_status || a.d_any_fallback) {
    if ((rc = status_launch(kp, a.d_status, a.d_any_fallback, s_main)) != D2PC_OK) return rc;
  }
  return D2PC_OK;
}

}

extern "C" int d2pc_path_create(D2pcPath **path) {
  if (!path) return D2PC_ERR_INVALID_ARGUMENT;
  *path = nullptr;
  D2pcPath *p = new D2pcPath();
  p->exec = nullptr;
  p->s_cap = nullptr;
  for (int i = 0; i < kMaxAux; ++i) p->s_aux[i] = nullptr;
  for (int i = 0; i < kMaxEmit; ++i) p->s_emit[i] = nullptr;
  cudaError_t e = cudaGetDevice(&p->device);
  int lo = 0, hi = 0;
  if (e == cudaSuccess) e = cudaDeviceGetStreamPriorityRange(&lo, &hi);
  if (e == cudaSuccess) e = cudaStreamCreateWithPriority(&p->s_cap, cudaStreamNonBlocking, lo);
  for (int i = 0; i < kMaxAux && e == cudaSuccess; ++i)
    e = cudaStreamCreateWithPriority(&p->s_aux[i], cudaStreamNonBlocking, getenv("D2PC_PATH_NOPRIO") ? lo : hi);
  for (int i = 0; i < kMaxEmit && e == cudaSuccess; ++i)
    e = cudaStreamCreateWithPriority(&p->s_emit[i], cudaStreamNonBlocking, lo);
  if (e != cudaSuccess) {
    d2pc_path_destroy(p);
    return record_cuda_error(e);
  }
  int rc = stats_prepare();
  if (rc) { d2pc_path_destroy(p); return rc; }
  *path = p;
  return D2PC_OK;
}

extern "C" void d2pc_path_destroy(D2pcPath *p) {
  if (!p) return;
  if (p->exec) cudaGraphExecDestroy(p->exec);
  for (cudaEvent_t e : p->events) cudaEventDestroy(e);
  if (p->s_cap) cudaStreamDestroy(p->s_cap);
  for (int i = 0; i < kMaxAux; ++i)
    if (p->s_aux[i]) cudaStreamDestroy(p->s_aux[i]);
  for (int i = 0; i < kMaxEmit; ++i)
    if (p->s_emit[i]) cudaStreamDestroy(p->s_emit[i]);
  delete p;
}

extern "C" int d2pc_path_enqueue(D2pcPath *p, const D2pcConfig *cfg, const float *d_depth, const uint8_t *d_bgr,
                                 void *d_workspace, size_t workspace_bytes, float *d_xyz, float *d_rgb,
                                 uint32_t *d_count, float *d_bounds, int32_t *d_status, int32_t *d_any_fallback,
                                 int32_t sub_batch, int32_t lookahead, int32_t flags, void *stream) {
  if (!p) return D2PC_ERR_INVALID_ARGUMENT;
  int rc = check_workspace(cfg, d_workspace, workspace_bytes);
  if (rc) return rc;
  rc = emit_validate(cfg, d_depth, d_bgr, d_workspace, workspace_bytes, d_xyz, d_rgb, d_count, d_bounds);
  if (rc) return rc;
  int dev = -1;
  PATH_CUDA(cudaGetDevice(&dev));
  if (dev != p->device) return D2PC_ERR_INVALID_ARGUMENT;
  if (sub_batch <= 0 || sub_batch > cfg->batch) sub_batch = cfg->batch;
  if (lookahead < 0) lookahead = 0;
  PathArgs a;
  memset(&a, 0, sizeof(a));
  a.cfg = *cfg;
  a.d_depth = d_depth; a.d_bgr = d_bgr; a.d_workspace = d_workspace; a.workspace_bytes = workspace_bytes;
  a.d_xyz = d_xyz; a.d_rgb = d_rgb; a.d_count = d_count; a.d_bounds = d_bounds;
  a.d_status = d_status; a.d_any_fallback = d_any_fallback;
  a.sub_batch = sub_batch; a.lookahead = lookahead; a.flags = flags;
  cudaStream_t st = (cudaStream_t)stream;
  {
    const KParams kp0 = make_kparams(a.cfg, a.d_depth, a.d_workspace);
    const EmitArgs ea0 = make_emit_args(a.cfg, a.d_bgr, a.d_xyz, a.d_rgb, a.d_count);
    if ((flags & D2PC_PATH_ORDERED) && path_kernel_supported(a.cfg, kp0, ea0)) return path_ordered(a, st);
  }
  if (!(flags & D2PC_PATH_GRAPH)) return path_body(p, a, st);

  const unsigned char *kb = reinterpret_cast<const unsigned char *>(&a);
  if (!p->exec || p->key.size() != sizeof(a) || memcmp(p->key.data(), kb, sizeof(a)) != 0) {
    if (p->exec) { cudaGraphExecDestroy(p->exec); p->exec = nullptr; }
    p->key.clear();
    cudaGraph_t graph = nullptr;
    PATH_CUDA(cudaStreamBeginCapture(p->s_cap, cudaStreamCaptureModeThreadLocal));
    rc = path_body(p, a, p->s_cap);
    cudaError_t e = cudaStreamEndCapture(p->s_cap, &graph);
    if (rc != D2PC_OK) { if (graph) cudaGraphDestroy(graph); return rc; }
    if (e != cudaSuccess) return record_cuda_error(e);
    e = cudaGraphInstantiate(&p->exec, graph, 0);
    cudaGraphDestroy(graph);
    if (e != cudaSuccess) { p->exec = nullptr; return record_cuda_error(e); }
    p->key.assign(kb, kb + sizeof(a));
  }
  PATH_CUDA(cudaGraphLaunch(p->exec, st));
  return D2PC_OK;
}

extern "C" int d2pc_path_trace_offset(const D2pcConfig *cfg, size_t *offset) {
  int rc = validate_config(cfg);
  if (rc) return rc;
  if (!offset) return D2PC_ERR_INVALID_ARGUMENT;
  *offset = make_layout(*cfg).sched_off + kSchedBytes;
  return D2PC_OK;
}
```

image_to_pointcloud_b200/csrc/d2pc_stats.cu:

```cuda
#include <stdlib.h>

#include "d2pc_stats_dev.cuh"

namespace d2pc {

__device__ __forceinline__ int32_t bracket_margin(double q, int S) {
  double sd = sqrt((double)S * q * (1.0 - q));
  return (int32_t)ceil(6.0 * sd) + 4;
}

__global__ void taps_kernel(KParams kp) {
  TapEntry *xt = const_cast<TapEntry *>(kp.xtab), *yt = const_cast<TapEntry *>(kp.ytab);
  const int i = blockIdx.x * blockDim.x + threadIdx.x;
  if (i < kp.g.W) {
    AxisTap a = axis_tap(i, kp.g.scale_x, kp.g.w);
    xt[i].i0c = a.i0 | (a.clamped ? (int32_t)0x80000000 : 0);
    xt[i].t = a.t;
  } else if (i < kp.g.W + kp.g.H) {
    AxisTap a = axis_tap(i - kp.g.W, kp.g.scale_y, kp.g.h);
    yt[i - kp.g.W].i0c = a.i0 | (a.clamped ? (int32_t)0x80000000 : 0);
    yt[i - kp.g.W].t = a.t;
  }
}

__global__ void __launch_bounds__(256) resize_generic_kernel(KParams kp) {
  const uint32_t b = blockIdx.y;
  const float *src = kp.depth + (size_t)b * kp.g.D;
  float *dst = kp.resized + (size_t)b * kp.g.P;
  for (uint32_t p = blockIdx.x * blockDim.x + threadIdx.x; p < kp.g.P; p += gridDim.x * blockDim.x) {
    const uint32_t v = p / (uint32_t)kp.g.W, u = p - v * (uint32_t)kp.g.W;
    dst[p] = generic_sample(src, kp.g.w, generic_tap((int32_t)u, kp.g.scale_x, kp.g.w, 1),
                            generic_tap((int32_t)v, kp.g.scale_y, kp.g.h, 0));
  }
}

template <bool NATIVE>
__global__ void __launch_bounds__(kSelThreads, 1) sample_kernel(KParams kp) {
  extern __shared__ uint32_t s_hist[];
  __shared__ uint32_t s_bad, s_min, s_max;
  __shared__ uint32_t s_res[2 * 4 + 40];
  __shared__ uint32_t s_warp[33], s_cnt[4], s_lmin[4], s_lmax[4], s_out[4];
  const int b = blockIdx.x;
  FrameState *fs = kp.state + b;
  const float *frame = kp.depth + (size_t)b * kp.g.D;
  const uint32_t n = kp.g.P;
  const int tid = threadIdx.x;
  if (tid == 0) {
    s_bad = 0; s_min = 0xFFFFFFFFu; s_max = 0u;
    for (int i = 0; i < 2; ++i) {
      fs->below[i] = 0; fs->eqL[i] = 0; fs->inside[i] = 0; fs->eqU[i] = 0;
    }
    fs->above1 = 0;
    fs->n_nonfinite = 0; fs->n_nan = 0; fs->nqueue[0] = 0; fs->nqueue[1] = 0;
    fs->min_key = 0xFFFFFFFFu; fs->max_key = 0u;
    for (int i = 0; i < 4; ++i) fs->sel_key[i] = 0;
    fs->sel_fail = 0; fs->sel_done = 0;
    if (b == 0)
      for (int i = 0; i <= kSchedQueues; ++i) kp.sched[32 * i] = 0u;
    {
      unsigned long long *tr = reinterpret_cast<unsigned long long *>(reinterpret_cast<unsigned char *>(kp.sched) + kSchedBytes) + (size_t)b * 8;
      for (int i = 0; i < 8; ++i) tr[i] = (i == 0 || i == 6) ? ~0ull : 0ull;
    }
    fs->status = D2PC_FRAME_PENDING;
    fs->fb_active = 0; fs->fb_any_nan = 0;
    fs->norm.has_nonfinite = 0;
    fs->norm.median = 0.0f;
    fs->norm.simple = 0;
  }
  {
    uint32_t *z = reinterpret_cast<uint32_t *>(kp.sel + b);
    for (uint32_t i = tid; i < sizeof(SelShared) / 4; i += kSelThreads) z[i] = 0u;
  }
  if (n <= (uint32_t)kSortCap) {
    if (tid == 0) {
      fs->brL[0] = fs->brL[1] = 0u;
      fs->brU[0] = fs->brU[1] = 0xFFFFFFFFu;
      fs->sample_ok = 1;
    }
    return;
  }
  constexpr int E = kSampleSize / kSelThreads;
  const uint32_t S = kSampleSize;
  uint32_t k[E];
  bool bad = false;
#pragma unroll
  for (int e = 0; e < E; ++e) {
    const uint32_t j = (uint32_t)e * kSelThreads + (uint32_t)tid;
    uint32_t start = (uint32_t)(((unsigned long long)j * n) / S);
    uint32_t end = (uint32_t)(((unsigned long long)(j + 1) * n) / S);
    uint32_t idx = start + hash_u32(j * 0x9E3779B9u + (uint32_t)b * 0x85EBCA6Bu + 12345u) % (end - start);
    float v;
    if (NATIVE) {
      asm volatile("ld.global.nc.L2::64B.f32 %0, [%1];" : "=f"(v) : "l"(frame + idx));
    } else {
      v = depth_at<NATIVE>(frame, kp, idx);
    }
    k[e] = 0xFFFFFFFFu;
    if (is_finite_f32(v)) k[e] = float_to_key(v); else bad = true;
  }
  __syncthreads();
  if (bad) atomicOr(&s_bad, 1u);
  {
    uint32_t mn = 0xFFFFFFFFu, mx = 0u;
#pragma unroll
    for (int e = 0; e < E; ++e) { mn = min(mn, k[e]); mx = max(mx, k[e]); }
    mn = warp_min(mn); mx = warp_max(mx);
    if ((tid & 31) == 0) { atomicMin(&s_min, mn); atomicMax(&s_max, mx); }
  }
  __syncthreads();
  uint32_t rank[4], out[4];
  bool open_lo[2], open_hi[2];
#pragma unroll
  for (int br = 0; br < 2; ++br) {
    const double q = br ? D2PC_Q98 : D2PC_Q02;
    RankPair rp = percentile_ranks(n, q);
    long long i_lo = (long long)(((unsigned long long)rp.lo * S) / n);
    long long i_hi = (long long)(((unsigned long long)rp.hi * S) / n) + 1;
    int32_t m = bracket_margin(q, (int)S);
    long long iL = i_lo - m, iU = i_hi + m;
    open_lo[br] = iL < 0;
    open_hi[br] = iU >= (long long)S;
    rank[2 * br + 0] = open_lo[br] ? 0u : (uint32_t)iL;
    rank[2 * br + 1] = open_hi[br] ? S - 1 : (uint32_t)iU;
  }
  {
    uint32_t *s_list = s_hist + kFastBins;
    const uint32_t lo0 = s_min, span = s_max - s_min;
    const int shift = fast_shift(span);
    for (uint32_t i = tid; i < kFastBins; i += kSelThreads) s_hist[i] = 0u;
    if (tid < 4) { s_cnt[tid] = 0u; s_lmin[tid] = 0xFFFFFFFFu; s_lmax[tid] = 0u; s_out[tid] = 0u; }
    __syncthreads();
#pragma unroll
    for (int e = 0; e < E; ++e) atomicAdd(&s_hist[(k[e] - lo0) >> shift], 1u);
    __syncthreads();
    uint32_t bin[4], base[4];
    const bool want[4] = {true, true, true, true};
    block_locate<4>(s_hist, rank, want, bin, base, s_warp, s_res);
    bool slow = false;
#pragma unroll
    for (int t = 0; t < 4; ++t) slow = slow || bin[t] == 0xFFFFFFFFu;
    if (!slow && shift == 0) {
#pragma unroll
      for (int t = 0; t < 4; ++t) out[t] = lo0 + bin[t];
    } else if (!slow) {
      int owner[4];
#pragma unroll
      for (int t = 0; t < 4; ++t) {
        owner[t] = t;
#pragma unroll
        for (int u = t - 1; u >= 0; --u)
          if (bin[u] == bin[t]) owner[t] = u;
      }
#pragma unroll
      for (int e = 0; e < E; ++e) {
        const uint32_t bk = (k[e] - lo0) >> shift;
#pragma unroll
        for (int t = 0; t < 4; ++t)
          if (owner[t] == t && bk == bin[t]) {
            const uint32_t idx = atomicAdd(&s_cnt[t], 1u);
            if (idx < kFastListCap) s_list[t * kFastListCap + idx] = k[e];
            atomicMin(&s_lmin[t], k[e]);
            atomicMax(&s_lmax[t], k[e]);
          }
      }
      __syncthreads();
#pragma unroll
      for (int t = 0; t < 4; ++t)
        if (owner[t] == t && s_cnt[t] > kFastListCap && s_lmin[t] != s_lmax[t]) slow = true;
      if (!slow) {
#pragma unroll
        for (int t = 0; t < 4; ++t) {
          const int o = owner[t];
          if (s_lmin[o] == s_lmax[o]) { if (tid == 0) s_out[t] = s_lmin[o]; }
          else block_pick(s_list + o * kFastListCap, s_cnt[o], rank[t] - base[t], &s_out[t]);
        }
        __syncthreads();
#pragma unroll
        for (int t = 0; t < 4; ++t) out[t] = s_out[t];
      }
    }
    if (slow) {
      __syncthreads();
      block_hist_select<4, kSelBits>([&](auto f) {
#pragma unroll
        for (int e = 0; e < E; ++e) f(k[e]);
      }, s_min, s_max, rank, out, s_hist, s_res);
    }
  }
  if (tid < 2) {
    fs->brL[tid] = open_lo[tid] ? 0u : out[2 * tid + 0];
    fs->brU[tid] = open_hi[tid] ? 0xFFFFFFFFu : out[2 * tid + 1];
  }
  if (tid == 0) fs->sample_ok = s_bad ? 0u : 1u;
}

template <int QD>
struct ScanSharedT {
  float pqueue[QD][kScanThreads];
  ScanFlushSmem flush;
};
using ScanShared = ScanSharedT<kScanPerThread>;

constexpr int kRzCols = 128, kRzRows = 32, kRzSrcRows = 40;
constexpr int kRzPerThread = kRzCols * kRzRows / kScanThreads;

__global__ void __launch_bounds__(kScanThreads) scan_resized_tiled_kernel(KParams kp) {
  __shared__ ScanSharedT<kRzPerThread> sh;
  __shared__ __align__(16) float s_h[kRzSrcRows][kRzCols];
  const int b = blockIdx.z, tid = threadIdx.x;
  FrameState *fs = kp.state + b;
  const float *frame = kp.depth + (size_t)b * kp.g.D;
  const int32_t W = kp.g.W, H = kp.g.H, sw = kp.g.w;
  float Lf[2], Uf[2];
  bracket_floats(fs, Lf, Uf);
  const uint32_t q0 = (uint32_t)__cvta_generic_to_shared(&sh.pqueue[0][tid]);
  uint32_t qaddr = q0;
  const int32_t u0 = blockIdx.x * kRzCols, v0 = blockIdx.y * kRzRows;
  const int32_t rows = min(kRzRows, H - v0);
  const int32_t ys = kp.ytab[v0].i0c & 0x7FFFFFFF;
  const TapEntry tl = kp.ytab[v0 + rows - 1];
  const int32_t nsr = (tl.i0c & 0x7FFFFFFF) + (tl.i0c < 0 ? 0 : 1) - ys + 1;
  {
    const int32_t col = tid & (kRzCols - 1), u = u0 + col;
    if (u < W) {
      const TapEntry tx = kp.xtab[u];
      const int32_t x0 = tx.i0c & 0x7FFFFFFF;
      const bool cx = tx.i0c < 0;
      for (int32_t r = tid / kRzCols; r < nsr; r += kScanThreads / kRzCols) {
        const float *row = frame + (size_t)(ys + r) * sw;
        const float a = __ldg(row + x0);
        float h = a;
        if (!cx) h = fmaf(__ldg(row + x0 + 1) - a, tx.t, a);
        s_h[r][col] = h;
      }
    }
  }
  __syncthreads();
  {
    const int32_t c4 = (tid & 31) * 4, uu = u0 + c4, warp = tid >> 5;
    const uint64_t pol_keep = l2_policy(false, (kp.hints & kHintResizedKeep) != 0);
    if (uu < W) {
      bool cxk[4];
#pragma unroll
      for (int k = 0; k < 4; ++k) cxk[k] = kp.xtab[uu + k].i0c < 0;
#pragma unroll 1
      for (int32_t rr = warp; rr < rows; rr += kScanThreads / 32) {
        const int32_t v = v0 + rr;
        const TapEntry ty = kp.ytab[v];
        const int32_t y0 = (ty.i0c & 0x7FFFFFFF) - ys;
        const float4 r0 = *reinterpret_cast<const float4 *>(&s_h[y0][c4]);
        float o[4] = {r0.x, r0.y, r0.z, r0.w};
        if (ty.i0c < 0) {
#pragma unroll
          for (int k = 0; k < 4; ++k)
            if (cxk[k] && is_inf_f32(o[k])) o[k] = nan_f32();
        } else {
          const float4 r1 = *reinterpret_cast<const float4 *>(&s_h[y0 + 1][c4]);
          o[0] = fmaf(r1.x - r0.x, ty.t, r0.x);
          o[1] = fmaf(r1.y - r0.y, ty.t, r0.y);
          o[2] = fmaf(r1.z - r0.z, ty.t, r0.z);
          o[3] = fmaf(r1.w - r0.w, ty.t, r0.w);
        }
#pragma unroll
        for (int k = 0; k < 4; ++k) scan_value(o[k], Uf[0], Lf[1], qaddr);
        float *dst = kp.resized + (size_t)b * kp.g.P + (size_t)v * W + uu;
        stg_f4_pol(dst, make_float4(o[0], o[1], o[2], o[3]), pol_keep);
      }
    }
  }
  scan_flush(&sh.pqueue[0][0], (qaddr - q0) / (uint32_t)(kScanThreads * 4), Uf[0], Lf[1], fs, kp, b, sh.flush);
}

template <int PT>
__global__ void __launch_bounds__(kScanThreads) scan_native_kernel(KParams kp, int vec_ok) {
  extern __shared__ __align__(16) unsigned char s_dyn[];
  scan_tile<PT>(kp, blockIdx.y, blockIdx.x, vec_ok, *reinterpret_cast<ScanTileSmemT<PT> *>(s_dyn));
}

template <int PT, int TPC, int MINB>
__global__ void __launch_bounds__(kScanThreads, MINB) scan_native_multi_kernel(KParams kp, int vec_ok) {
  extern __shared__ __align__(16) unsigned char s_dyn[];
  ScanTileSmemT<PT> &sm = *reinterpret_cast<ScanTileSmemT<PT> *>(s_dyn);
  constexpr int kPx = PT * kScanThreads;
  const int tid = threadIdx.x, b = blockIdx.y;
  FrameState *fs = kp.state + b;
  const float *frame = kp.depth + (size_t)b * kp.g.D;
  const uint32_t n = kp.g.P;
  const uint32_t ntiles = (n + (uint32_t)kPx - 1u) / (uint32_t)kPx;
  const uint32_t t0 = blockIdx.x * (uint32_t)TPC;
  const float U0 = bracket_hi_float(fs->brU[0]), L1 = bracket_lo_float(fs->brL[1]);
  const uint32_t q0 = (uint32_t)__cvta_generic_to_shared(&sm.pq[0][tid]);
  const uint64_t pol = l2_policy((kp.hints & kHintScanKeep) == 0, (kp.hints & kHintScanKeep) != 0);
  auto full = [&](uint32_t tile) { return vec_ok && tile < ntiles && (tile + 1u) * (uint32_t)kPx <= n; };
  float4 r[PT / 4];
  if (full(t0)) {
    const float *src = frame + t0 * (uint32_t)kPx + 4u * (uint32_t)tid;
#pragma unroll
    for (int j = 0; j < PT / 4; ++j) r[j] = ldg_f4_pol(src + (size_t)j * (4 * kScanThreads), pol);
  }
#pragma unroll 1
  for (uint32_t i = 0; i < (uint32_t)TPC; ++i) {
    const uint32_t tile = t0 + i;
    if (tile >= ntiles) break;
    uint32_t qaddr = q0;
    if (full(tile)) {
#pragma unroll
      for (int j = 0; j < PT / 4; ++j) {
        scan_value(r[j].x, U0, L1, qaddr);
        scan_value(r[j].y, U0, L1, qaddr);
        scan_value(r[j].z, U0, L1, qaddr);
        scan_value(r[j].w, U0, L1, qaddr);
      }
    } else {
      const uint32_t tile_base = tile * (uint32_t)kPx;
#pragma unroll 1
      for (int j = 0; j < PT / 4; ++j) {
        const uint32_t p = tile_base + 4u * (uint32_t)(j * kScanThreads + tid);
        for (uint32_t k = 0; k < 4u; ++k)
          if (p + k < n) scan_value(__ldg(frame + p + k), U0, L1, qaddr);
      }
    }
    if (i + 1u < (uint32_t)TPC && full(tile + 1u)) {
      const float *src = frame + (tile + 1u) * (uint32_t)kPx + 4u * (uint32_t)tid;
#pragma unroll
      for (int j = 0; j < PT / 4; ++j) r[j] = ldg_f4_pol(src + (size_t)j * (4 * kScanThreads), pol);
    }
    scan_flush(&sm.pq[0][0], (qaddr - q0) / (uint32_t)(kScanThreads * 4), U0, L1, fs, kp, b, sm.flush);
    __syncthreads();
  }
}

__global__ void __launch_bounds__(kScanThreads) scan_gather_kernel(KParams kp, int vec_ok) {
  __shared__ ScanShared sh;
  const int b = blockIdx.y;
  const int tid = threadIdx.x;
  FrameState *fs = kp.state + b;
  const float *frame = kp.depth + (size_t)b * kp.g.D;
  const uint32_t n = kp.g.P;
  float Lf[2], Uf[2];
  bracket_floats(fs, Lf, Uf);
  const uint32_t q0 = (uint32_t)__cvta_generic_to_shared(&sh.pqueue[0][tid]);
  uint32_t qaddr = q0;
  const uint32_t tile_base = blockIdx.x * (uint32_t)kScanTile;
  const uint32_t W = (uint32_t)kp.g.W;
#pragma unroll 2
  for (int j = 0; j < kScanPerThread / 4; ++j) {
    uint32_t p = tile_base + 4u * (uint32_t)(j * kScanThreads + tid);
    if (p >= n) continue;
    uint32_t v = p / W;
    uint32_t u = p - v * W;
    TapEntry ty = kp.ytab[v];
    float val[4] = {0.0f, 0.0f, 0.0f, 0.0f};
#pragma unroll
    for (uint32_t k = 0; k < 4u; ++k) {
      if (p + k < n) {
        if (u >= W) {
          u -= W;
          v += 1;
          ty = kp.ytab[v];
        }
        val[k] = bilinear_taps(frame, kp.g.w, kp.xtab[u], ty);
        scan_value(val[k], Uf[0], Lf[1], qaddr);
        u += 1;
      }
    }
    float *dst = kp.resized + (size_t)b * n + p;
    if (vec_ok && p + 3u < n) *reinterpret_cast<float4 *>(dst) = make_float4(val[0], val[1], val[2], val[3]);
    else
      for (uint32_t k = 0; k < 4u; ++k)
        if (p + k < n) dst[k] = val[k];
  }
  scan_flush(&sh.pqueue[0][0], (qaddr - q0) / (uint32_t)(kScanThreads * 4), Uf[0], Lf[1], fs, kp, b, sh.flush);
}

__global__ void __launch_bounds__(kSelectThreads, 2) select_kernel(KParams kp) {
  extern __shared__ uint32_t s_sel[];
  __shared__ SelectSmall ss;
  select_bracket(kp, blockIdx.y, blockIdx.x, s_sel, ss);
}

constexpr int kCoopThreads = 512;
constexpr uint32_t kCoopSmemWords = 2u << 11;
__global__ void __launch_bounds__(kCoopThreads) select_a_kernel(KParams kp, uint32_t K) {
  extern __shared__ uint32_t s_sel[];
  __shared__ SelPartSmall ss;
  select_phase_a<true>(kp, blockIdx.z, blockIdx.y, blockIdx.x, K, reinterpret_cast<float *>(s_sel), 0u, ss);
}
__global__ void __launch_bounds__(kCoopThreads) select_c_kernel(KParams kp, uint32_t K) {
  extern __shared__ uint32_t s_sel[];
  __shared__ SelPartSmall ss;
  const int b = blockIdx.z, br = blockIdx.y;
  if (*reinterpret_cast<volatile uint32_t *>(&kp.sel[b].bin_ready[br]) != 1u) return;
  select_phase_c(kp, b, br, blockIdx.x, K, reinterpret_cast<float *>(s_sel), 0u, false, ss);
}

constexpr uint32_t kStatsSliceCap = (uint32_t)(sizeof(ScanTileSmem) / sizeof(float));
__global__ void __launch_bounds__(kScanThreads, 5) stats_ordered_kernel(KParams kp, int vec_ok, uint32_t ns, uint32_t K) {
  extern __shared__ __align__(16) unsigned char s_dyn[];
  __shared__ SelPartSmall s_sel;
  __shared__ uint32_t s_go;
  const int tid = threadIdx.x;
  const uint32_t group_items = 2u * K + ns;
  const uint32_t g = blockIdx.x / group_items, i = blockIdx.x - g * group_items;
  uint32_t *abort_flag = sched_abort_flag(kp);
  if (i < 2u * K) {
    if (g < 1u) return;
    const int f = (int)g - 1;
    const uint32_t br = i / K, k = i - br * K;
    if (tid == 0) s_go = spin_until(&kp.sel[f].scan_done, abort_flag, [&](uint32_t v) { return v >= ns; }) ? 1u : 0u;
    __syncthreads();
    if (!s_go) return;
    select_part(kp, f, (int)br, k, K, reinterpret_cast<float *>(s_dyn), kStatsSliceCap, s_sel,
                [&](const uint32_t *p, auto pred) { return spin_until(p, abort_flag, pred); });
    return;
  }
  if (g >= (uint32_t)kp.batch) return;
  scan_tile<kTilePerThread>(kp, (int)g, i - 2u * K, vec_ok, *reinterpret_cast<ScanTileSmem *>(s_dyn));
  __syncthreads();
  if (tid == 0) {
    __threadfence();
    atomicAdd(&kp.sel[g].scan_done, 1u);
  }
}

enum { kStageMedian = 0, kStagePercentile = 1 };

__global__ void fb_reset_kernel(KParams kp) {
  FrameState *fs = kp.state + blockIdx.x;
  if (threadIdx.x == 0 && fs->status == D2PC_FRAME_NEEDS_FALLBACK) {
    fs->n_nonfinite = 0; fs->n_nan = 0;
    fs->min_key = 0xFFFFFFFFu; fs->max_key = 0u;
  }
}

template <bool NATIVE>
__global__ void __launch_bounds__(kScanThreads) fb_count_kernel(KParams kp) {
  const int b = blockIdx.y, tid = threadIdx.x;
  FrameState *fs = kp.state + b;
  if (fs->status != D2PC_FRAME_NEEDS_FALLBACK) return;
  const float *frame = kp.depth + (size_t)b * kp.g.D;
  const uint32_t n = kp.g.P;
  const uint32_t tile_base = blockIdx.x * (uint32_t)kScanTile;
  uint32_t nf = 0, nan = 0;
  for (int j = 0; j < kScanPerThread; ++j) {
    uint32_t p = tile_base + (uint32_t)(j * kScanThreads + tid);
    if (p >= n) break;
    float v = depth_at<NATIVE>(frame, kp, p);
    if (!is_finite_f32(v)) { nf++; if (is_nan_f32(v)) nan++; }
  }
  nf = warp_sum(nf);
  nan = warp_sum(nan);
  if ((tid & 31) == 0) {
    if (nf) atomicAdd(&fs->n_nonfinite, nf);
    if (nan) atomicAdd(&fs->n_nan, nan);
  }
}

__global__ void fb_begin_kernel(KParams kp) {
  const int b = blockIdx.x;
  FrameState *fs = kp.state + b;
  uint32_t *hist = kp.fb_hist + (size_t)b * kFbTargets * 256;
  for (int i = threadIdx.x; i < kFbTargets * 256; i += blockDim.x) hist[i] = 0;
  if (threadIdx.x != 0) return;
  fs->fb_active = 0;
  fs->fb_any_nan = 0;
  if (fs->status != D2PC_FRAME_NEEDS_FALLBACK) return;
  if (fs->n_nonfinite == 0) return;
  const uint32_t m = kp.g.P - fs->n_nan;
  if (m == 0) return;
  for (int t = 0; t < kFbTargets; ++t) fs->fb_prefix[t] = 0;
  if (m & 1u) {
    fs->fb_rank[0] = m / 2;
    fs->fb_active = 1;
  } else {
    fs->fb_rank[0] = m / 2 - 1;
    fs->fb_rank[1] = m / 2;
    fs->fb_active = 2;
  }
}

template <bool NATIVE>
__global__ void __launch_bounds__(kScanThreads) fb_hist_kernel(KParams kp, int stage, int pass) {
  __shared__ uint32_t sh[kFbTargets][256];
  const int b = blockIdx.y, tid = threadIdx.x;
  FrameState *fs = kp.state + b;
  if (fs->status != D2PC_FRAME_NEEDS_FALLBACK) return;
  const int T = (int)fs->fb_active;
  if (T == 0) return;
  const float *frame = kp.depth + (size_t)b * kp.g.D;
  const uint32_t n = kp.g.P;
  for (int i = tid; i < kFbTargets * 256; i += kScanThreads) (&sh[0][0])[i] = 0;
  uint32_t prefix[kFbTargets];
  for (int t = 0; t < kFbTargets; ++t) prefix[t] = fs->fb_prefix[t];
  const float med = fs->norm.median;
  __syncthreads();
  const int shift = 24 - 8 * pass;
  const uint32_t tile_base = blockIdx.x * (uint32_t)kScanTile;
  uint32_t kmin = 0xFFFFFFFFu, kmax = 0u;
  for (int j = 0; j < kScanPerThread; ++j) {
    uint32_t p = tile_base + (uint32_t)(j * kScanThreads + tid);
    if (p >= n) break;
    float v = depth_at<NATIVE>(frame, kp, p);
    if (stage == kStageMedian) {
      if (is_nan_f32(v)) continue;
    } else {
      if (!is_finite_f32(v)) v = med;
    }
    uint32_t key = float_to_key(v);
    kmin = min(kmin, key);
    kmax = max(kmax, key);
    for (int t = 0; t < T; ++t) {
      bool match = (pass == 0) || ((key >> (shift + 8)) == (prefix[t] >> (shift + 8)));
      if (match) atomicAdd(&sh[t][(key >> shift) & 255u], 1u);
    }
  }
  if (stage == kStagePercentile && pass == 0) {
    kmin = warp_min(kmin);
    kmax = warp_max(kmax);
    if ((tid & 31) == 0) {
      if (kmin != 0xFFFFFFFFu) atomicMin(&fs->min_key, kmin);
      if (kmax != 0u) atomicMax(&fs->max_key, kmax);
    }
  }
  __syncthreads();
  uint32_t *hist = kp.fb_hist + (size_t)b * kFbTargets * 256;
  for (int i = tid; i < T * 256; i += kScanThreads) {
    uint32_t c = (&sh[0][0])[i];
    if (c) atomicAdd(&hist[i], c);
  }
}

__global__ void fb_pick_kernel(KParams kp, int pass) {
  const int b = blockIdx.x;
  FrameState *fs = kp.state + b;
  uint32_t *hist = kp.fb_hist + (size_t)b * kFbTargets * 256;
  const bool live = fs->status == D2PC_FRAME_NEEDS_FALLBACK && fs->fb_active > 0;
  if (live && threadIdx.x < fs->fb_active) {
    const int t = threadIdx.x;
    const int shift = 24 - 8 * pass;
    uint32_t rank = fs->fb_rank[t], cum = 0;
    int d = 0;
    for (; d < 256; ++d) {
      uint32_t c = hist[t * 256 + d];
      if (rank < cum + c) break;
      cum += c;
    }
    if (d > 255) d = 255;
    fs->fb_prefix[t] |= (uint32_t)d << shift;
    fs->fb_rank[t] = rank - cum;
  }
  __syncthreads();
  for (int i = threadIdx.x; i < kFbTargets * 256; i += blockDim.x) hist[i] = 0;
}

__global__ void fb_median_kernel(KParams kp) {
  const int b = blockIdx.x;
  FrameState *fs = kp.state + b;
  if (threadIdx.x != 0 || fs->status != D2PC_FRAME_NEEDS_FALLBACK) return;
  const uint32_t n = kp.g.P;
  float med = 0.0f;
  int has_nf = 0;
  if (fs->n_nonfinite != 0) {
    has_nf = 1;
    const uint32_t m = n - fs->n_nan;
    if (m == 0) {
      med = nan_f32();
    } else {
      const int T = (int)fs->fb_active;
      med = median_from_ranks(key_to_float(fs->fb_prefix[0]), key_to_float(fs->fb_prefix[T - 1]), m);
    }
  }
  fs->norm.median = med;
  fs->norm.has_nonfinite = has_nf;
  const bool any_nan = has_nf && is_nan_f32(med);
  fs->fb_any_nan = any_nan ? 1u : 0u;
  if (any_nan) {
    fs->fb_active = 0;
    return;
  }
  RankPair r2 = percentile_ranks(n, D2PC_Q02), r98 = percentile_ranks(n, D2PC_Q98);
  fs->fb_rank[0] = r2.lo; fs->fb_rank[1] = r2.hi; fs->fb_rank[2] = r98.lo; fs->fb_rank[3] = r98.hi;
  for (int t = 0; t < kFbTargets; ++t) fs->fb_prefix[t] = 0;
  fs->fb_active = 4;
}

__global__ void fb_finalise_kernel(KParams kp) {
  const int b = blockIdx.x;
  FrameState *fs = kp.state + b;
  if (threadIdx.x != 0 || fs->status != D2PC_FRAME_NEEDS_FALLBACK) return;
  const uint32_t n = kp.g.P;
  NormParams np_;
  const float med = fs->norm.median;
  const int has_nf = fs->norm.has_nonfinite;
  if (fs->fb_any_nan) {
    finalise_norm(0.0, 0.0, 0.0f, 0.0f, true, &np_);
  } else {
    RankPair r2 = percentile_ranks(n, D2PC_Q02), r98 = percentile_ranks(n, D2PC_Q98);
    double p2 = lerp_percentile(key_to_float(fs->fb_prefix[0]), key_to_float(fs->fb_prefix[1]), r2.gamma);
    double p98 = lerp_percentile(key_to_float(fs->fb_prefix[2]), key_to_float(fs->fb_prefix[3]), r98.gamma);
    const uint32_t kmin = fs->min_key, kmax = fs->max_key;
    finalise_norm(p2, p98, key_to_float(kmin), key_to_float(kmax), false, &np_);
  }
  np_.median = med;
  np_.has_nonfinite = has_nf;
  finish_norm(&np_);
  fs->norm = np_;
  __threadfence();
  fs->status = D2PC_FRAME_READY;
}

__global__ void status_kernel(KParams kp, int32_t *d_status, int32_t *d_any) {
  __shared__ int s_any;
  if (threadIdx.x == 0) s_any = 0;
  __syncthreads();
  for (int b = threadIdx.x; b < kp.batch; b += blockDim.x) {
    int32_t s = kp.state[b].status;
    if (s == D2PC_FRAME_PENDING) {
      s = D2PC_FRAME_NEEDS_FALLBACK;
      kp.state[b].status = s;
    }
    if (d_status) d_status[b] = s;
    if (s == D2PC_FRAME_NEEDS_FALLBACK) s_any = 1;
  }
  __syncthreads();
  if (threadIdx.x == 0 && d_any) *d_any = s_any;
}

__global__ void params_kernel(KParams kp, D2pcFrameParams *out) {
  for (int b = blockIdx.x * blockDim.x + threadIdx.x; b < kp.batch; b += gridDim.x * blockDim.x) {
    const FrameState &fs = kp.state[b];
    D2pcFrameParams o;
    o.p2 = fs.norm.p2; o.p98 = fs.norm.p98; o.den = fs.norm.den; o.inv_den = fs.norm.inv_den;
    o.lo32 = fs.norm.lo32; o.hi32 = fs.norm.hi32; o.den32 = fs.norm.den32; o.median = fs.norm.median;
    o.branch = fs.norm.branch; o.status = fs.status;
    o.n_nonfinite = fs.n_nonfinite; o.n_nan = fs.n_nan;
    o.n_cand[0] = fs.nqueue[0]; o.n_cand[1] = fs.nqueue[1];
    o.reserved[0] = fs.sel_fail; o.reserved[1] = fs.sample_ok;
    out[b] = o;
  }
}

}

using namespace d2pc;

static int check_ws(const D2pcConfig *cfg, const void *ws, size_t ws_bytes) {
  int rc = validate_config(cfg);
  if (rc) return rc;
  if (!ws) return D2PC_ERR_INVALID_ARGUMENT;
  if (ws_bytes < make_layout(*cfg).total) return D2PC_ERR_WORKSPACE_TOO_SMALL;
  if (((uintptr_t)ws & 255u) != 0) return D2PC_ERR_INVALID_ARGUMENT;
  return D2PC_OK;
}

namespace d2pc {

int taps_launch(const KParams &kp, cudaStream_t st) {
  if (kp.g.native || resize_is_generic(kp.g.h, kp.g.w)) return D2PC_OK;
  taps_kernel<<<(kp.g.W + kp.g.H + 255) / 256, 256, 0, st>>>(kp);
  D2PC_CHECK_LAUNCH();
  return D2PC_OK;
}

int stats_prepare() {
  const size_t sample_smem = (size_t)(4u << kSelBits) * sizeof(uint32_t);
  cudaError_t e = cudaFuncSetAttribute(sample_kernel<true>, cudaFuncAttributeMaxDynamicSharedMemorySize, (int)sample_smem);
  if (e == cudaSuccess)
    e = cudaFuncSetAttribute(select_kernel, cudaFuncAttributeMaxDynamicSharedMemorySize, (int)(kSelectSmemWords * sizeof(uint32_t)));
  if (e == cudaSuccess)
    e = cudaFuncSetAttribute(sample_kernel<false>, cudaFuncAttributeMaxDynamicSharedMemorySize, (int)sample_smem);
  if (e == cudaSuccess)
    e = cudaFuncSetAttribute(scan_native_kernel<kTilePerThread>, cudaFuncAttributeMaxDynamicSharedMemorySize, (int)sizeof(ScanTileSmem));
  if (e == cudaSuccess)
    e = cudaFuncSetAttribute(scan_native_multi_kernel<kTilePerThread, 2, 4>, cudaFuncAttributeMaxDynamicSharedMemorySize, (int)sizeof(ScanTileSmem));
  if (e == cudaSuccess)
    e = cudaFuncSetAttribute(scan_native_multi_kernel<kTilePerThread, 4, 4>, cudaFuncAttributeMaxDynamicSharedMemorySize, (int)sizeof(ScanTileSmem));
  if (e == cudaSuccess)
    e = cudaFuncSetAttribute(stats_ordered_kernel, cudaFuncAttributeMaxDynamicSharedMemorySize, (int)sizeof(ScanTileSmem));
  if (e != cudaSuccess) return record_cuda_error(e);
  return D2PC_OK;
}

int stats_launch(KParams kp, cudaStream_t st, int phases) {
  const int nb = kp.batch;
  if (!kp.g.native && resize_is_generic(kp.g.h, kp.g.w)) {
    const uint32_t blocks = (kp.g.P + 255u) / 256u;
    if (phases & kStatsSample) {
      resize_generic_kernel<<<dim3(blocks < 148u * 8u ? blocks : 148u * 8u, nb), 256, 0, st>>>(kp);
      D2PC_CHECK_LAUNCH();
    }
    kp = per_pixel_view(kp);
  }
  const size_t sample_smem = (size_t)(4u << kSelBits) * sizeof(uint32_t);
  const int vec_ok = ((kp.g.P & 3u) == 0u) && (((uintptr_t)kp.depth & 15u) == 0u);
  dim3 scan_grid((kp.g.P + kScanTile - 1) / kScanTile, nb);
  if (phases & kStatsSample) {
    if (kp.g.native) sample_kernel<true><<<nb, kSelThreads, sample_smem, st>>>(kp);
    else sample_kernel<false><<<nb, kSelThreads, sample_smem, st>>>(kp);
    D2PC_CHECK_LAUNCH();
  }
  if (!(phases & kStatsScanSelect)) return D2PC_OK;
  const char *mode = getenv("D2PC_STATS_ORDERED");
  const bool ordered = (phases & kStatsScanSelect) == kStatsScanSelect && (mode ? atoi(mode) != 0 : nb <= 2);
  if (kp.g.native && kp.g.P > (uint32_t)kSortCap && ordered) {
    const uint32_t ns = (kp.g.P + kTilePx - 1) / kTilePx;
    uint32_t K = (kp.cand_cap + kStatsSliceCap - 1u) / kStatsSliceCap;
    K = K < 4u ? 4u : (K > 64u ? 64u : K);
    const unsigned long long total = (unsigned long long)(nb + 1) * (2ull * K + ns);
    if (total < 0x7FFFFFFFull) {
      stats_ordered_kernel<<<(unsigned)total, kScanThreads, sizeof(ScanTileSmem), st>>>(kp, vec_ok, ns, K);
      D2PC_CHECK_LAUNCH();
      return D2PC_OK;
    }
  }
  if (!(phases & kStatsScan)) {
  } else if (kp.g.native) {
    const uint32_t nt = (kp.g.P + kTilePx - 1) / kTilePx;
    const char *te = getenv("D2PC_SCAN_TPC");
    const unsigned long long tiles = (unsigned long long)nt * (unsigned long long)nb;
    const int tpc = te ? atoi(te) : (tiles >= 4ull * 1184ull ? 4 : (tiles >= 2ull * 1184ull ? 2 : 1));
    if (tpc >= 4) scan_native_multi_kernel<kTilePerThread, 4, 4><<<dim3((nt + 3) / 4, nb), kScanThreads, sizeof(ScanTileSmem), st>>>(kp, vec_ok);
    else if (tpc >= 2) scan_native_multi_kernel<kTilePerThread, 2, 4><<<dim3((nt + 1) / 2, nb), kScanThreads, sizeof(ScanTileSmem), st>>>(kp, vec_ok);
    else scan_native_kernel<kTilePerThread><<<dim3(nt, nb), kScanThreads, sizeof(ScanTileSmem), st>>>(kp, vec_ok);
  } else {
    bool tiled = (kp.g.W & 3) == 0;
    for (int32_t v0 = 0; tiled && v0 < kp.g.H; v0 += kRzRows) {
      const int32_t v1 = (v0 + kRzRows < kp.g.H ? v0 + kRzRows : kp.g.H) - 1;
      const AxisTap t0 = axis_tap(v0, kp.g.scale_y, kp.g.h), t1 = axis_tap(v1, kp.g.scale_y, kp.g.h);
      if (t1.i1 - t0.i0 + 1 > kRzSrcRows) tiled = false;
    }
    if (tiled) {
      dim3 tg((kp.g.W + kRzCols - 1) / kRzCols, (kp.g.H + kRzRows - 1) / kRzRows, nb);
      scan_resized_tiled_kernel<<<tg, kScanThreads, 0, st>>>(kp);
    } else {
      scan_gather_kernel<<<scan_grid, kScanThreads, 0, st>>>(kp, (kp.g.P & 3u) == 0u ? 1 : 0);
    }
  }
  D2PC_CHECK_LAUNCH();
  if (phases & kStatsSelect) {
    const char *cm = getenv("D2PC_SELECT_COOP");
    uint32_t K = 296u / (2u * (uint32_t)nb);
    if (K > 16u) K = 16u;
    if (kp.g.P >= 4u * 1024u * 1024u && K < 4u) K = 4u;
    if (K < 4u) K = 0u;
    if (cm) K = (uint32_t)atoi(cm);
    if (K > 64u) K = 64u;
    if (K >= 2u && kp.g.P > (uint32_t)kSortCap) {
      select_a_kernel<<<dim3(K, 2, nb), kCoopThreads, kCoopSmemWords * sizeof(uint32_t), st>>>(kp, K);
      D2PC_CHECK_LAUNCH();
      select_c_kernel<<<dim3(K, 2, nb), kCoopThreads, kCoopSmemWords * sizeof(uint32_t), st>>>(kp, K);
    } else {
      select_kernel<<<dim3(2, nb), kSelectThreads, (size_t)kSelectSmemWords * sizeof(uint32_t), st>>>(kp);
    }
    D2PC_CHECK_LAUNCH();
  }
  return D2PC_OK;
}

int status_launch(const KParams &kp, int32_t *d_status, int32_t *d_any, cudaStream_t st) {
  status_kernel<<<1, 256, 0, st>>>(kp, d_status, d_any);
  D2PC_CHECK_LAUNCH();
  return D2PC_OK;
}

int check_workspace(const D2pcConfig *cfg, const void *ws, size_t ws_bytes) { return check_ws(cfg, ws, ws_bytes); }

}

extern "C" int d2pc_stats_enqueue(const D2pcConfig *cfg, const float *d_depth, void *d_workspace,
                                  size_t workspace_bytes, void *stream) {
  int rc = check_ws(cfg, d_workspace, workspace_bytes);
  if (rc) return rc;
  if (!d_depth) return D2PC_ERR_INVALID_ARGUMENT;
  cudaStream_t st = (cudaStream_t)stream;
  KParams kp = make_kparams(*cfg, d_depth, d_workspace);
  if ((rc = stats_prepare()) != D2PC_OK) return rc;
  if ((rc = taps_launch(kp, st)) != D2PC_OK) return rc;
  return stats_launch(kp, st, kStatsSample | kStatsScanSelect);
}

extern "C" int d2pc_stats_fallback_enqueue(const D2pcConfig *cfg, const float *d_depth,
                                           void *d_workspace, size_t workspace_bytes, void *stream) {
  int rc = check_ws(cfg, d_workspace, workspace_bytes);
  if (rc) return rc;
  if (!d_depth) return D2PC_ERR_INVALID_ARGUMENT;
  cudaStream_t st = (cudaStream_t)stream;
  KParams kp = per_pixel_view(make_kparams(*cfg, d_depth, d_workspace));
  dim3 grid((kp.g.P + kScanTile - 1) / kScanTile, cfg->batch);
  fb_reset_kernel<<<cfg->batch, 32, 0, st>>>(kp);
  D2PC_CHECK_LAUNCH();
  fb_count_kernel<true><<<grid, kScanThreads, 0, st>>>(kp);
  D2PC_CHECK_LAUNCH();
  fb_begin_kernel<<<cfg->batch, 256, 0, st>>>(kp);
  D2PC_CHECK_LAUNCH();
  for (int stage = 0; stage < 2; ++stage) {
    for (int pass = 0; pass < 4; ++pass) {
      fb_hist_kernel<true><<<grid, kScanThreads, 0, st>>>(kp, stage, pass);
      D2PC_CHECK_LAUNCH();
      fb_pick_kernel<<<cfg->batch, 256, 0, st>>>(kp, pass);
      D2PC_CHECK_LAUNCH();
    }
    if (stage == 0) fb_median_kernel<<<cfg->batch, 32, 0, st>>>(kp);
    else fb_finalise_kernel<<<cfg->batch, 32, 0, st>>>(kp);
    D2PC_CHECK_LAUNCH();
  }
  return D2PC_OK;
}

extern "C" int d2pc_frame_status(const D2pcConfig *cfg, const void *d_workspace, int32_t *d_status,
                                 int32_t *d_any_fallback, void *stream) {
  int rc = validate_config(cfg);
  if (rc) return rc;
  if (!d_workspace) return D2PC_ERR_INVALID_ARGUMENT;
  KParams kp = make_kparams(*cfg, nullptr, (void *)d_workspace);
  return status_launch(kp, d_status, d_any_fallback, (cudaStream_t)stream);
}

extern "C" int d2pc_frame_params(const D2pcConfig *cfg, const void *d_workspace,
                                 D2pcFrameParams *d_params, void *stream) {
  int rc = validate_config(cfg);
  if (rc) return rc;
  if (!d_workspace || !d_params) return D2PC_ERR_INVALID_ARGUMENT;
  KParams kp = make_kparams(*cfg, nullptr, (void *)d_workspace);
  params_kernel<<<(cfg->batch + 127) / 128, 128, 0, (cudaStream_t)stream>>>(kp, d_params);
  D2PC_CHECK_LAUNCH();
  return D2PC_OK;
}
```

image_to_pointcloud_b200/csrc/d2pc_stats_dev.cuh:

```cuda
#ifndef D2PC_STATS_DEV_CUH_
#define D2PC_STATS_DEV_CUH_

#include "d2pc_device.cuh"

namespace d2pc {

constexpr int kTilePerThread = 32;
constexpr int kTilePx = kScanThreads * kTilePerThread;

__device__ __forceinline__ void scan_value(float v, float U0, float L1, uint32_t &qaddr) {
  asm volatile(
      "{\n\t"
      ".reg .pred mid;\n\t"
      "setp.gt.f32 mid, %1, %2;\n\t"
      "setp.lt.and.f32 mid, %1, %3, mid;\n\t"
      "@!mid st.shared.f32 [%0], %1;\n\t"
      "@!mid add.u32 %0, %0, %4;\n\t"
      "}"
      : "+r"(qaddr)
      : "f"(v), "f"(U0), "f"(L1), "n"(kScanThreads * 4)
      : "memory");
}

__device__ __forceinline__ float bracket_lo_float(uint32_t L) {
  return (L == 0u) ? -__int_as_float(0x7F800000) : key_to_float(L);
}
__device__ __forceinline__ float bracket_hi_float(uint32_t U) {
  return (U == 0xFFFFFFFFu) ? __int_as_float(0x7F800000) : key_to_float(U);
}
__device__ __forceinline__ void bracket_floats(const FrameState *fs, float Lf[2], float Uf[2]) {
#pragma unroll
  for (int br = 0; br < 2; ++br) {
    Lf[br] = bracket_lo_float(fs->brL[br]);
    Uf[br] = bracket_hi_float(fs->brU[br]);
  }
}

struct ScanFlushSmem {
  uint32_t wtot[kScanThreads / 32];
  uint32_t gbase[2];
};
__device__ __forceinline__ void scan_flush(const float *pq, uint32_t nq, float U0, float L1, FrameState *fs,
                                           const KParams &kp, int b, ScanFlushSmem &sm) {
  const int tid = threadIdx.x, lane = tid & 31, warp = tid >> 5;
  uint32_t packed = 0;
  for (uint32_t j = 0; j < nq; ++j) {
    const float v = pq[j * kScanThreads + tid];
    packed += (!(v > U0) ? 1u : 0u) + ((v >= L1) ? 0x10000u : 0u);
  }
  uint32_t incl = packed;
#pragma unroll
  for (int d = 1; d < 32; d <<= 1) {
    const uint32_t y = __shfl_up_sync(0xffffffffu, incl, d);
    if (lane >= d) incl += y;
  }
  if (lane == 31) sm.wtot[warp] = incl;
  __syncthreads();
  uint32_t woff = 0, total = 0;
#pragma unroll
  for (int w = 0; w < kScanThreads / 32; ++w) {
    const uint32_t x = sm.wtot[w];
    if (w < warp) woff += x;
    total += x;
  }
  if (total == 0u) return;
  if (tid == 0) {
    const unsigned long long add = (unsigned long long)(total & 0xFFFFu) | ((unsigned long long)(total >> 16) << 32);
    const unsigned long long old = atomicAdd(reinterpret_cast<unsigned long long *>(&fs->nqueue[0]), add);
    sm.gbase[0] = (uint32_t)old;
    sm.gbase[1] = (uint32_t)(old >> 32);
  }
  __syncthreads();
  if (nq == 0u) return;
  float *gq0 = reinterpret_cast<float *>(kp.cand) + (size_t)b * 2 * kp.cand_cap;
  const uint32_t excl = woff + incl - packed;
  uint32_t o0 = sm.gbase[0] + (excl & 0xFFFFu), o1 = sm.gbase[1] + (excl >> 16);
  const uint64_t pol_keep = l2_policy(false, true);
  if (o0 + (packed & 0xFFFFu) <= kp.cand_cap && o1 + (packed >> 16) <= kp.cand_cap) {
    o1 += kp.cand_cap;
    for (uint32_t j = 0; j < nq; ++j) {
      const float v = pq[j * kScanThreads + tid];
      if (!(v > U0)) stg_f1_pol(gq0 + o0++, v, pol_keep);
      if (v >= L1) stg_f1_pol(gq0 + o1++, v, pol_keep);
    }
  } else {
    for (uint32_t j = 0; j < nq; ++j) {
      const float v = pq[j * kScanThreads + tid];
      if (!(v > U0)) { if (o0 < kp.cand_cap) gq0[o0] = v; ++o0; }
      if (v >= L1) { if (o1 < kp.cand_cap) gq0[kp.cand_cap + o1] = v; ++o1; }
    }
  }
}

template <int PT>
struct ScanTileSmemT {
  float pq[PT][kScanThreads];
  ScanFlushSmem flush;
};
using ScanTileSmem = ScanTileSmemT<kTilePerThread>;

template <int PT>
__device__ __forceinline__ void scan_tile(const KParams &kp, int b, uint32_t tile, int vec_ok, ScanTileSmemT<PT> &sm) {
  constexpr int kTilePerThread = PT;
  constexpr int kTilePx = PT * kScanThreads;
  const int tid = threadIdx.x;
  FrameState *fs = kp.state + b;
  const float *frame = kp.depth + (size_t)b * kp.g.D;
  const uint32_t n = kp.g.P;
  const float U0 = bracket_hi_float(fs->brU[0]), L1 = bracket_lo_float(fs->brL[1]);
  const uint32_t q0 = (uint32_t)__cvta_generic_to_shared(&sm.pq[0][tid]);
  uint32_t qaddr = q0;
  const uint32_t tile_base = tile * (uint32_t)kTilePx;
  if (vec_ok && tile_base + (uint32_t)kTilePx <= n) {
    const float *src = frame + tile_base + 4u * (uint32_t)tid;
    const uint64_t pol = l2_policy((kp.hints & kHintScanKeep) == 0, (kp.hints & kHintScanKeep) != 0);
    float4 r[kTilePerThread / 4];
#pragma unroll
    for (int j = 0; j < kTilePerThread / 4; ++j) r[j] = ldg_f4_pol(src + (size_t)j * (4 * kScanThreads), pol);
#pragma unroll
    for (int j = 0; j < kTilePerThread / 4; ++j) {
      scan_value(r[j].x, U0, L1, qaddr);
      scan_value(r[j].y, U0, L1, qaddr);
      scan_value(r[j].z, U0, L1, qaddr);
      scan_value(r[j].w, U0, L1, qaddr);
    }
  } else {
#pragma unroll 1
    for (int j = 0; j < kTilePerThread / 4; ++j) {
      const uint32_t p = tile_base + 4u * (uint32_t)(j * kScanThreads + tid);
      for (uint32_t k = 0; k < 4u; ++k)
        if (p + k < n) scan_value(__ldg(frame + p + k), U0, L1, qaddr);
    }
  }
  const uint32_t nq = (qaddr - q0) / (uint32_t)(kScanThreads * 4);
  scan_flush(&sm.pq[0][0], nq, U0, L1, fs, kp, b, sm.flush);
}

__device__ __forceinline__ void finalise_fast(FrameState *fs, uint32_t n) {
  volatile FrameState *vfs = fs;
  if (vfs->sel_fail) {
    __threadfence();
    vfs->status = D2PC_FRAME_NEEDS_FALLBACK;
    return;
  }
  RankPair r2 = percentile_ranks(n, D2PC_Q02), r98 = percentile_ranks(n, D2PC_Q98);
  double p2 = lerp_percentile(key_to_float(vfs->sel_key[0]), key_to_float(vfs->sel_key[1]), r2.gamma);
  double p98 = lerp_percentile(key_to_float(vfs->sel_key[2]), key_to_float(vfs->sel_key[3]), r98.gamma);
  if (!(p98 > p2)) {
    __threadfence();
    vfs->status = D2PC_FRAME_NEEDS_FALLBACK;
    return;
  }
  NormParams np_;
  finalise_norm(p2, p98, 0.0f, 0.0f, false, &np_);
  np_.median = 0.0f;
  np_.has_nonfinite = 0;
  finish_norm(&np_);
  fs->norm = np_;
  __threadfence();
  vfs->status = D2PC_FRAME_READY;
}

template <int U, typename F>
__device__ __forceinline__ void for_each_queued(const float *q, uint32_t nq, F f) {
  const uint32_t stride = blockDim.x;
  uint32_t i = threadIdx.x;
  for (; i + (uint32_t)(U - 1) * stride < nq; i += (uint32_t)U * stride) {
    float v[U];
#pragma unroll
    for (int k = 0; k < U; ++k) v[k] = __ldcg(q + i + (uint32_t)k * stride);
#pragma unroll
    for (int k = 0; k < U; ++k) f(v[k]);
  }
  for (; i < nq; i += stride) f(__ldcg(q + i));
}

constexpr int kSelectSmemWords = (int)kFastBins + 2 * (int)kFastListCap;

struct SelectSmall {
  uint32_t res[2 * 2 + 40];
  uint32_t c[6];
  uint32_t warp[33], cnt[2], lmin[2], lmax[2], out[2];
};

__device__ __forceinline__ void select_bracket(const KParams &kp, int b, int br, uint32_t *s_hist, SelectSmall &ss) {
  const int tid = threadIdx.x, nthr = blockDim.x;
  FrameState *fs = kp.state + b;
  const uint32_t n = kp.g.P;
  const uint32_t qcap = kp.cand_cap;
  const float *q = reinterpret_cast<const float *>(kp.cand) + ((size_t)b * 2 + br) * qcap;
  volatile FrameState *vfs = fs;
  const uint32_t nqueue = vfs->nqueue[br];
  const uint32_t nq = min(nqueue, qcap);
  const uint32_t L = fs->brL[br], U = fs->brU[br];
  float Lf2[2], Uf2[2];
  bracket_floats(fs, Lf2, Uf2);
  const float Lf = Lf2[br], Uf = Uf2[br];
  const uint32_t lo0 = L > 0u ? L - 1u : 0u;
  const uint32_t hi0 = U < 0xFFFFFFFFu ? U + 1u : U;
  const uint32_t span = hi0 - lo0;
  const int shift = fast_shift(span);
  const uint32_t list_cap = kFastListCap;
  uint32_t *s_list = s_hist + kFastBins;
  for (uint32_t i = tid; i < kFastBins; i += nthr) s_hist[i] = 0u;
  if (tid < 6) ss.c[tid] = 0;
  if (tid < 2) { ss.cnt[tid] = 0u; ss.lmin[tid] = 0xFFFFFFFFu; ss.lmax[tid] = 0u; ss.out[tid] = 0u; }
  __syncthreads();
  {
    uint32_t c_eqL = 0, c_in = 0, c_eqU = 0, c_below = 0, c_nf = 0;
    for_each_queued<8>(q, nq, [&](float v) {
      if (!(fabsf(v) < __int_as_float(0x7F800000))) c_nf += 1u + ((v != v) ? 0x10000u : 0u);
      else if (v < Lf) c_below++;
      else if (v == Lf) c_eqL++;
      else if (v < Uf) {
        c_in++;
        const uint32_t d = float_to_key(v) - lo0;
        if (d <= span) atomicAdd(&s_hist[d >> shift], 1u);
      } else if (v == Uf) c_eqU++;
    });
    c_eqL = warp_sum(c_eqL); c_in = warp_sum(c_in); c_eqU = warp_sum(c_eqU); c_below = warp_sum(c_below);
    const uint32_t w_nf = warp_sum(c_nf & 0xFFFFu), w_nan = warp_sum(c_nf >> 16);
    if ((tid & 31) == 0) {
      if (c_eqL) atomicAdd(&ss.c[0], c_eqL);
      if (c_in) atomicAdd(&ss.c[1], c_in);
      if (c_eqU) atomicAdd(&ss.c[2], c_eqU);
      if (c_below) atomicAdd(&ss.c[3], c_below);
      if (w_nf) atomicAdd(&ss.c[4], w_nf);
      if (w_nan) atomicAdd(&ss.c[5], w_nan);
    }
  }
  __syncthreads();
  const uint32_t eqL = ss.c[0], nin = ss.c[1], eqU = ss.c[2], n_nf = ss.c[4];
  const uint32_t below = br == 0 ? ss.c[3] : n - nqueue;
  bool fail = (n_nf != 0u) || (nqueue > qcap) || (fs->sample_ok == 0u) || (kp.force_fallback != 0);
  RankPair rp = percentile_ranks(n, br ? D2PC_Q98 : D2PC_Q02);
  bool want[2] = {false, false};
  uint32_t need[2] = {0u, 0u};
  uint32_t key[2] = {0u, 0u};
  for (int t = 0; t < 2; ++t) {
    uint32_t r = t ? rp.hi : rp.lo;
    if (r < below) { fail = true; continue; }
    uint32_t r1 = r - below;
    if (r1 < eqL) { key[t] = L; continue; }
    uint32_t r2 = r1 - eqL;
    if (r2 < nin) { need[t] = r2; want[t] = true; continue; }
    uint32_t r3 = r2 - nin;
    if (r3 < eqU) { key[t] = U; continue; }
    fail = true;
  }

  if (!fail && (want[0] || want[1])) {
    uint32_t bin[2], base[2];
    block_locate<2>(s_hist, need, want, bin, base, ss.warp, ss.res);
    bool slow = (want[0] && bin[0] == 0xFFFFFFFFu) || (want[1] && bin[1] == 0xFFFFFFFFu);
    if (!slow && shift == 0) {
      for (int t = 0; t < 2; ++t)
        if (want[t]) key[t] = lo0 + bin[t];
    } else if (!slow) {
      const bool shared_bin = want[0] && want[1] && bin[0] == bin[1];
      const bool own[2] = {want[0], want[1] && !shared_bin};
      for_each_queued<8>(q, nq, [&](float v) {
        if (v > Lf && v < Uf) {
          const uint32_t k = float_to_key(v);
          const uint32_t bk = (k - lo0) >> shift;
#pragma unroll
          for (int t = 0; t < 2; ++t)
            if (own[t] && bk == bin[t]) {
              const uint32_t idx = atomicAdd(&ss.cnt[t], 1u);
              if (idx < list_cap) s_list[t * kFastListCap + idx] = k;
              atomicMin(&ss.lmin[t], k);
              atomicMax(&ss.lmax[t], k);
            }
        }
      });
      __syncthreads();
      for (int t = 0; t < 2; ++t)
        if (own[t] && ss.cnt[t] > list_cap && ss.lmin[t] != ss.lmax[t]) slow = true;
      if (!slow) {
        for (int t = 0; t < 2; ++t) {
          if (!want[t]) continue;
          const int o = (t == 1 && shared_bin) ? 0 : t;
          if (ss.lmin[o] == ss.lmax[o]) { if (tid == 0) ss.out[t] = ss.lmin[o]; }
          else block_pick(s_list + o * kFastListCap, ss.cnt[o], need[t] - base[t], &ss.out[t]);
        }
        __syncthreads();
        for (int t = 0; t < 2; ++t)
          if (want[t]) key[t] = ss.out[t];
      }
    }
    if (slow) {
      __syncthreads();
      uint32_t rk[2], ok_[2];
      for (int t = 0; t < 2; ++t) rk[t] = want[t] ? need[t] : need[1 - t];
      const bool ok = block_hist_select<2, 11>([&](auto f) {
        for_each_queued<8>(q, nq, [&](float v) {
          if (v > Lf && v < Uf) f(float_to_key(v));
        });
      }, lo0, hi0, rk, ok_, s_hist, ss.res);
      if (!ok) fail = true;
      for (int t = 0; t < 2; ++t)
        if (want[t]) key[t] = ok_[t];
    }
  }

  if (tid == 0) {
    fs->sel_key[2 * br + 0] = key[0];
    fs->sel_key[2 * br + 1] = key[1];
    fs->eqL[br] = eqL; fs->inside[br] = nin; fs->eqU[br] = eqU;
    fs->below[br] = below;
    if (n_nf) { atomicAdd(&fs->n_nonfinite, n_nf); atomicAdd(&fs->n_nan, ss.c[5]); }
    if (fail) atomicOr(&fs->sel_fail, 1u);
    __threadfence();
    uint32_t ticket = atomicAdd(&fs->sel_done, 1u);
    if (ticket == 1u) {
      __threadfence();
      finalise_fast(fs, n);
    }
  }
}

constexpr uint32_t kSpinLimit = 1u << 19;

__device__ __forceinline__ uint32_t ld_relaxed_u32(const uint32_t *p) {
  uint32_t v;
  asm volatile("ld.relaxed.gpu.global.u32 %0, [%1];" : "=r"(v) : "l"(p) : "memory");
  return v;
}
__device__ __forceinline__ uint32_t ld_acquire_u32(const uint32_t *p) {
  uint32_t v;
  asm volatile("ld.acquire.gpu.global.u32 %0, [%1];" : "=r"(v) : "l"(p) : "memory");
  return v;
}

template <typename Pred>
__device__ __forceinline__ bool spin_until(const uint32_t *p, uint32_t *abort_flag, Pred pred) {
  uint32_t spins = 0, ns = 128;
  while (!pred(ld_relaxed_u32(p))) {
    __nanosleep(ns);
    if (ns < 2048u) ns <<= 1;
    if (++spins > kSpinLimit || ((spins & 15u) == 0u && ld_relaxed_u32(abort_flag))) {
      atomicExch(abort_flag, 1u);
      return false;
    }
  }
  (void)ld_acquire_u32(p);
  return true;
}

__device__ __forceinline__ uint32_t *sched_abort_flag(const KParams &kp) { return kp.sched + 32u * kSchedQueues; }

constexpr uint32_t kSliceCap = 6144;

struct SelPartSmall {
  uint32_t c[6];
  uint32_t res[2 * 2 + 40];
  uint32_t warp[33];
  uint32_t flag_a, flag_spin, flag_c, out[2];
};

__device__ __forceinline__ void select_finish(FrameState *fs, SelShared *sh, int br, uint32_t n, const uint32_t key[2],
                                              bool fail) {
  volatile uint32_t *cn = sh->counts[br];
  fs->sel_key[2 * br + 0] = key[0];
  fs->sel_key[2 * br + 1] = key[1];
  fs->eqL[br] = cn[1]; fs->inside[br] = cn[2]; fs->eqU[br] = cn[3];
  if (cn[4]) { atomicAdd(&fs->n_nonfinite, cn[4]); atomicAdd(&fs->n_nan, cn[5]); }
  if (fail) atomicOr(&fs->sel_fail, 1u);
  __threadfence();
  const uint32_t ticket = atomicAdd(&fs->sel_done, 1u);
  if (ticket == 1u) {
    __threadfence();
    finalise_fast(fs, n);
  }
}

struct SelCommon {
  FrameState *fs;
  SelShared *sh;
  const float *q;
  uint32_t n, qcap, nqueue, nq, L, U, lo0, hi0, span, s_lo, m;
  float Lf, Uf;
  int shift;
  bool cached;
};
__device__ __forceinline__ SelCommon select_common(const KParams &kp, int b, int br, uint32_t k, uint32_t K, uint32_t slice_cap) {
  SelCommon c;
  c.fs = kp.state + b;
  c.sh = kp.sel + b;
  volatile FrameState *vfs = c.fs;
  c.n = kp.g.P; c.qcap = kp.cand_cap;
  c.q = reinterpret_cast<const float *>(kp.cand) + ((size_t)b * 2 + br) * c.qcap;
  c.nqueue = vfs->nqueue[br];
  c.nq = min(c.nqueue, c.qcap);
  c.L = c.fs->brL[br]; c.U = c.fs->brU[br];
  c.Lf = bracket_lo_float(c.L); c.Uf = bracket_hi_float(c.U);
  c.lo0 = c.L > 0u ? c.L - 1u : 0u;
  c.hi0 = c.U < 0xFFFFFFFFu ? c.U + 1u : c.U;
  c.span = c.hi0 - c.lo0;
  c.shift = fast_shift(c.span);
  const uint32_t chunk = (c.nq + K - 1u) / K;
  c.s_lo = min(c.nq, k * chunk);
  c.m = min(c.nq, c.s_lo + chunk) - c.s_lo;
  c.cached = chunk <= slice_cap;
  return c;
}

template <bool LOCAL_HIST = false>
__device__ __forceinline__ int select_phase_a(const KParams &kp, int b, int br, uint32_t k, uint32_t K, float *s_slice,
                                              uint32_t slice_cap, SelPartSmall &ss) {
  const int tid = threadIdx.x, nthr = blockDim.x;
  const SelCommon cm = select_common(kp, b, br, k, K, slice_cap);
  FrameState *fs = cm.fs;
  SelShared *sh = cm.sh;
  const float *q = cm.q;
  const uint32_t n = cm.n, qcap = cm.qcap, nqueue = cm.nqueue, L = cm.L, U = cm.U, lo0 = cm.lo0, span = cm.span,
                 s_lo = cm.s_lo, m = cm.m;
  const float Lf = cm.Lf, Uf = cm.Uf;
  const int shift = cm.shift;
  const bool cached = cm.cached && !LOCAL_HIST;
  if (tid < 6) ss.c[tid] = 0u;
  if (LOCAL_HIST)
    for (uint32_t i = tid; i < kSelBins; i += nthr) reinterpret_cast<uint32_t *>(s_slice)[i] = 0u;
  __syncthreads();
  {
    uint32_t c_eqL = 0, c_in = 0, c_eqU = 0, c_below = 0, c_nf = 0;
    uint32_t *hist = LOCAL_HIST ? reinterpret_cast<uint32_t *>(s_slice) : sh->hist[br];
    auto visit = [&](float v) {
      if (!(fabsf(v) < __int_as_float(0x7F800000))) c_nf += 1u + ((v != v) ? 0x10000u : 0u);
      else if (v < Lf) c_below++;
      else if (v == Lf) c_eqL++;
      else if (v < Uf) {
        c_in++;
        const uint32_t d = float_to_key(v) - lo0;
        if (d <= span) atomicAdd(&hist[d >> shift], 1u);
      } else if (v == Uf) c_eqU++;
    };
    uint32_t i = tid;
    for (; i + 7u * nthr < m; i += 8u * nthr) {
      float v[8];
#pragma unroll
      for (int u = 0; u < 8; ++u) v[u] = __ldcg(q + s_lo + i + (uint32_t)u * nthr);
#pragma unroll
      for (int u = 0; u < 8; ++u) {
        if (cached) s_slice[i + (uint32_t)u * nthr] = v[u];
        visit(v[u]);
      }
    }
    for (; i < m; i += nthr) {
      const float v = __ldcg(q + s_lo + i);
      if (cached) s_slice[i] = v;
      visit(v);
    }
    c_eqL = warp_sum(c_eqL); c_in = warp_sum(c_in); c_eqU = warp_sum(c_eqU); c_below = warp_sum(c_below);
    const uint32_t w_nf = warp_sum(c_nf & 0xFFFFu), w_nan = warp_sum(c_nf >> 16);
    if ((tid & 31) == 0) {
      if (c_below) atomicAdd(&ss.c[0], c_below);
      if (c_eqL) atomicAdd(&ss.c[1], c_eqL);
      if (c_in) atomicAdd(&ss.c[2], c_in);
      if (c_eqU) atomicAdd(&ss.c[3], c_eqU);
      if (w_nf) atomicAdd(&ss.c[4], w_nf);
      if (w_nan) atomicAdd(&ss.c[5], w_nan);
    }
  }
  __syncthreads();
  if (LOCAL_HIST) {
    const uint32_t *lh = reinterpret_cast<const uint32_t *>(s_slice);
    for (uint32_t i = tid; i < kSelBins; i += nthr) {
      const uint32_t h = lh[i];
      if (h) atomicAdd(&sh->hist[br][i], h);
    }
    __threadfence();
    __syncthreads();
  }
  if (tid == 0) {
    for (int c = 0; c < 6; ++c)
      if (ss.c[c]) atomicAdd(&sh->counts[br][c], ss.c[c]);
    __threadfence();
    ss.flag_a = atomicAdd(&sh->a_done[br], 1u);
    __threadfence();
  }
  __syncthreads();
  const bool last_a = ss.flag_a == K - 1u;
  if (last_a) {
    volatile uint32_t *cn = sh->counts[br];
    const uint32_t eqL = cn[1], nin = cn[2], eqU = cn[3], n_nf = cn[4];
    const uint32_t below = br == 0 ? cn[0] : n - nqueue;
    bool fail = (n_nf != 0u) || (nqueue > qcap) || (fs->sample_ok == 0u) || (kp.force_fallback != 0);
    const RankPair rp = percentile_ranks(n, br ? D2PC_Q98 : D2PC_Q02);
    bool want[2] = {false, false};
    uint32_t need[2] = {0u, 0u}, key[2] = {0u, 0u};
    for (int t = 0; t < 2; ++t) {
      const uint32_t r = t ? rp.hi : rp.lo;
      if (r < below) { fail = true; continue; }
      const uint32_t r1 = r - below;
      if (r1 < eqL) { key[t] = L; continue; }
      const uint32_t r2 = r1 - eqL;
      if (r2 < nin) { need[t] = r2; want[t] = true; continue; }
      const uint32_t r3 = r2 - nin;
      if (r3 < eqU) { key[t] = U; continue; }
      fail = true;
    }
    bool collect = false;
    uint32_t bin[2] = {0u, 0u}, base[2] = {0u, 0u};
    if (!fail && (want[0] || want[1])) {
      block_locate<2, true>(sh->hist[br], need, want, bin, base, ss.warp, ss.res);
      if ((want[0] && bin[0] == 0xFFFFFFFFu) || (want[1] && bin[1] == 0xFFFFFFFFu)) fail = true;
      else if (shift == 0) {
        for (int t = 0; t < 2; ++t)
          if (want[t]) key[t] = lo0 + bin[t];
      } else collect = true;
    }
    if (tid == 0) {
      if (collect) {
        for (int t = 0; t < 2; ++t) {
          sh->bin[br][t] = bin[t]; sh->base[br][t] = base[t]; sh->need[br][t] = need[t];
          sh->want[br][t] = want[t] ? 1u : 0u;
          sh->key[br][t] = key[t];
        }
        sh->shared_bin[br] = (want[0] && want[1] && bin[0] == bin[1]) ? 1u : 0u;
        __threadfence();
        *reinterpret_cast<volatile uint32_t *>(&sh->bin_ready[br]) = 1u;
      } else {
        select_finish(fs, sh, br, n, key, fail);
        __threadfence();
        *reinterpret_cast<volatile uint32_t *>(&sh->bin_ready[br]) = 2u;
      }
    }
    return collect ? 1 : 2;
  }
  return 0;
}

__device__ __forceinline__ void select_phase_c(const KParams &kp, int b, int br, uint32_t k, uint32_t K,
                                               float *s_slice, uint32_t slice_cap, bool slice_is_cached, SelPartSmall &ss) {
  const int tid = threadIdx.x, nthr = blockDim.x;
  const SelCommon cm = select_common(kp, b, br, k, K, slice_cap);
  FrameState *fs = cm.fs;
  SelShared *sh = cm.sh;
  const float *q = cm.q;
  const uint32_t n = cm.n, nq = cm.nq, lo0 = cm.lo0, hi0 = cm.hi0, s_lo = cm.s_lo, m = cm.m;
  const float Lf = cm.Lf, Uf = cm.Uf;
  const int shift = cm.shift;
  const bool cached = cm.cached && slice_is_cached;
  {
    volatile SelShared *vsh = sh;
    const bool shared_bin = vsh->shared_bin[br] != 0u;
    const bool own[2] = {vsh->want[br][0] != 0u, vsh->want[br][1] != 0u && !shared_bin};
    const uint32_t bin0 = vsh->bin[br][0], bin1 = vsh->bin[br][1];
    auto collect = [&](float v) {
      if (v > Lf && v < Uf) {
        const uint32_t key = float_to_key(v);
        const uint32_t bk = (key - lo0) >> shift;
#pragma unroll
        for (int t = 0; t < 2; ++t)
          if (own[t] && bk == (t ? bin1 : bin0)) {
            const uint32_t idx = atomicAdd(&sh->mcount[br][t], 1u);
            if (idx < kSelListCap) sh->members[br][t][idx] = key;
            atomicMax(&sh->mmin[br][t], ~key);
            atomicMax(&sh->mmax[br][t], key);
          }
      }
    };
    uint32_t i = tid;
    if (!cached) {
      for (; i + 7u * nthr < m; i += 8u * nthr) {
        float v[8];
#pragma unroll
        for (int u = 0; u < 8; ++u) v[u] = __ldcg(q + s_lo + i + (uint32_t)u * nthr);
#pragma unroll
        for (int u = 0; u < 8; ++u) collect(v[u]);
      }
    }
    for (; i < m; i += nthr) collect(cached ? s_slice[i] : __ldcg(q + s_lo + i));
  }
  __syncthreads();
  if (tid == 0) {
    __threadfence();
    ss.flag_c = atomicAdd(&sh->c_done[br], 1u);
    __threadfence();
  }
  __syncthreads();
  if (ss.flag_c != K - 1u) return;
  {
    volatile SelShared *vsh = sh;
    const bool shared_bin = vsh->shared_bin[br] != 0u;
    bool want[2] = {vsh->want[br][0] != 0u, vsh->want[br][1] != 0u};
    uint32_t key[2] = {vsh->key[br][0], vsh->key[br][1]};
    bool fail = false, slow = false;
    uint32_t *s_list = reinterpret_cast<uint32_t *>(s_slice);
    for (int t = 0; t < 2; ++t) {
      if (!want[t] || (t == 1 && shared_bin)) continue;
      const uint32_t cnt = vsh->mcount[br][t];
      if (cnt > kSelListCap && ~vsh->mmin[br][t] != vsh->mmax[br][t]) slow = true;
      for (uint32_t i = tid; i < min(cnt, kSelListCap); i += nthr) s_list[t * kSelListCap + i] = __ldcg(&sh->members[br][t][i]);
    }
    if (tid < 2) ss.out[tid] = 0u;
    __syncthreads();
    if (!slow) {
      for (int t = 0; t < 2; ++t) {
        if (!want[t]) continue;
        const int o = (t == 1 && shared_bin) ? 0 : t;
        const uint32_t mn = ~vsh->mmin[br][o], mx = vsh->mmax[br][o];
        if (mn == mx) { if (tid == 0) ss.out[t] = mn; }
        else block_pick(s_list + o * kSelListCap, min(vsh->mcount[br][o], kSelListCap), vsh->need[br][t] - vsh->base[br][t], &ss.out[t]);
      }
      __syncthreads();
      for (int t = 0; t < 2; ++t)
        if (want[t]) key[t] = ss.out[t];
    } else {
      uint32_t rk[2], ok_[2];
      for (int t = 0; t < 2; ++t) rk[t] = want[t] ? vsh->need[br][t] : vsh->need[br][1 - t];
      const bool ok = block_hist_select<2, 11>([&](auto f) {
        for_each_queued<8>(q, nq, [&](float v) {
          if (v > Lf && v < Uf) f(float_to_key(v));
        });
      }, lo0, hi0, rk, ok_, reinterpret_cast<uint32_t *>(s_slice), ss.res);
      if (!ok) fail = true;
      for (int t = 0; t < 2; ++t)
        if (want[t]) key[t] = ok_[t];
    }
    if (tid == 0) select_finish(fs, sh, br, n, key, fail);
  }
}

template <typename Spin>
__device__ __forceinline__ bool select_part(const KParams &kp, int b, int br, uint32_t k, uint32_t K, float *s_slice,
                                            uint32_t slice_cap, SelPartSmall &ss, Spin spin) {
  const int st = select_phase_a<false>(kp, b, br, k, K, s_slice, slice_cap, ss);
  if (st == 2) return true;
  SelShared *sh = kp.sel + b;
  if (st == 0) {
    if (threadIdx.x == 0) ss.flag_spin = spin(&sh->bin_ready[br], [](uint32_t v) { return v != 0u; }) ? 1u : 0u;
    __syncthreads();
    if (!ss.flag_spin) return false;
    if (*reinterpret_cast<volatile uint32_t *>(&sh->bin_ready[br]) == 2u) return true;
  }
  __syncthreads();
  select_phase_c(kp, b, br, k, K, s_slice, slice_cap, true, ss);
  return true;
}

}
#endif
```

Measured before the change: 173,800.

## Overlap scan, select and emit kernels with programmatic dependent launch

Adds programmatic dependent launch so the select kernel can start while the scan kernel is still running. Select then spins on a per-frame scan_done counter that each scan block increments. The emit kernel gets a 'behind' variant that is also PDL-launched and spin-waits on each frame's status word before reading the norm parameters. The aim is to hide kernel launch gaps and tail latency between the stats and emit stages. In exchange it adds spin-waiting blocks that hold SM slots, extra atomics and fences, and a capture-support probe at path creation. It only applies in narrow configurations: single sub-batch, no mask, no bounds, and no ordered or cooperative select.

New measurement: 160,900, median of 6. 0.926x the previous value.

```diff
diff --git a/image_to_pointcloud_b200/csrc/d2pc_device.cuh b/image_to_pointcloud_b200/csrc/d2pc_device.cuh
--- a/image_to_pointcloud_b200/csrc/d2pc_device.cuh
+++ b/image_to_pointcloud_b200/csrc/d2pc_device.cuh
@@ -213,7 +213,9 @@
 int stats_prepare();
 int taps_launch(const KParams &kp, cudaStream_t st);
 constexpr int kStatsSample = 1, kStatsScan = 2, kStatsSelect = 4, kStatsScanSelect = kStatsScan | kStatsSelect;
-int stats_launch(KParams kp, cudaStream_t st, int phases);
+constexpr int kOverlapSelect = 1, kOverlapEmit = 2;
+int stats_launch(KParams kp, cudaStream_t st, int phases, int overlap = 0);
+bool stats_overlap_ok(const KParams &kp, int phases);
 int status_launch(const KParams &kp, int32_t *d_status, int32_t *d_any, cudaStream_t st);
 EmitArgs make_emit_args(const D2pcConfig &cfg, const uint8_t *d_bgr, float *d_xyz, float *d_rgb, uint32_t *d_count);
 EmitArgs slice_emit_args(const EmitArgs &ea, const Geom &g, int b0);
@@ -222,7 +224,7 @@
 int emit_validate(const D2pcConfig *cfg, const float *d_depth, const uint8_t *d_bgr, void *d_workspace,
                   size_t workspace_bytes, float *d_xyz, float *d_rgb, uint32_t *d_count, float *d_bounds);
 int emit_launch(const D2pcConfig &cfg, const KParams &kp, const EmitArgs &ea, float *d_bounds, cudaStream_t st,
-                int32_t smooth_k, const double *h_kernel, void *d_scratch);
+                int32_t smooth_k, const double *h_kernel, void *d_scratch, bool behind = false);
 int record_cuda_error(cudaError_t e);
 
 #define D2PC_CHECK_LAUNCH()                                  \
@@ -232,6 +234,38 @@
   } while (0)
 
 #if defined(__CUDACC__)
+constexpr uint32_t kSpinLimit = 1u << 19;
+
+__device__ __forceinline__ uint32_t ld_relaxed_u32(const uint32_t *p) {
+  uint32_t v;
+  asm volatile("ld.relaxed.gpu.global.u32 %0, [%1];" : "=r"(v) : "l"(p) : "memory");
+  return v;
+}
+__device__ __forceinline__ uint32_t ld_acquire_u32(const uint32_t *p) {
+  uint32_t v;
+  asm volatile("ld.acquire.gpu.global.u32 %0, [%1];" : "=r"(v) : "l"(p) : "memory");
+  return v;
+}
+
+template <typename Pred>
+__device__ __forceinline__ bool spin_until(const uint32_t *p, uint32_t *abort_flag, Pred pred) {
+  uint32_t spins = 0, ns = 128;
+  while (!pred(ld_relaxed_u32(p))) {
+    __nanosleep(ns);
+    if (ns < 2048u) ns <<= 1;
+    if (++spins > kSpinLimit || ((spins & 15u) == 0u && ld_relaxed_u32(abort_flag))) {
+      atomicExch(abort_flag, 1u);
+      return false;
+    }
+  }
+  (void)ld_acquire_u32(p);
+  return true;
+}
+
+__device__ __forceinline__ uint32_t *sched_abort_flag(const KParams &kp) { return kp.sched + 32u * kSchedQueues; }
+
+__device__ __forceinline__ void launch_dependents() { asm volatile("griddepcontrol.launch_dependents;" ::: "memory"); }
+
 __device__ __forceinline__ float4 ldg_stream_f4(const float *p) {
   float4 r;
   asm volatile("ld.global.nc.L1::no_allocate.v4.f32 {%0,%1,%2,%3}, [%4];"
diff --git a/image_to_pointcloud_b200/csrc/d2pc_emit.cu b/image_to_pointcloud_b200/csrc/d2pc_emit.cu
--- a/image_to_pointcloud_b200/csrc/d2pc_emit.cu
+++ b/image_to_pointcloud_b200/csrc/d2pc_emit.cu
@@ -135,6 +135,23 @@
   return D2PC_OK;
 }
 
+template <int STEP>
+static int launch_emit_fast_behind(const KParams &kp, const EmitArgs &ea, const FastArgs &fa, cudaStream_t st) {
+  cudaLaunchAttribute attr[1];
+  attr[0].id = cudaLaunchAttributeProgrammaticStreamSerialization;
+  attr[0].val.programmaticStreamSerializationAllowed = 1;
+  cudaLaunchConfig_t lc = {};
+  lc.gridDim = dim3(fa.total_tiles);
+  lc.blockDim = dim3(kEmitThreads);
+  lc.dynamicSmemBytes = kEmitStageBytes;
+  lc.stream = st;
+  lc.attrs = attr;
+  lc.numAttrs = 1;
+  const cudaError_t e = cudaLaunchKernelEx(&lc, emit_fast_kernel<STEP, false, false, 6, true>, kp, ea, fa);
+  if (e != cudaSuccess) return record_cuda_error(e);
+  return D2PC_OK;
+}
+
 struct SmoothArgs {
   const double *rows;
   int32_t ksize;
@@ -349,7 +366,7 @@
 }
 
 int emit_launch(const D2pcConfig &cfg, const KParams &kp_in, const EmitArgs &ea, float *d_bounds, cudaStream_t st,
-                int32_t smooth_k, const double *h_kernel, void *d_scratch) {
+                int32_t smooth_k, const double *h_kernel, void *d_scratch, bool behind) {
   const bool smooth = smooth_k > 0;
   const KParams kp = per_pixel_view(kp_in);
   const int nb = kp.batch;
@@ -400,6 +417,10 @@
     if (mask) rcl = cfg.step == 1 ? launch_emit_fast<1, true, 5>(kp, ea, fa, st)
                   : cfg.step == 2 ? launch_emit_fast<2, true, 5>(kp, ea, fa, st)
                                   : launch_emit_fast<4, true, 5>(kp, ea, fa, st);
+    else if (behind && !cfg.want_bounds)
+      rcl = cfg.step == 1 ? launch_emit_fast_behind<1>(kp, ea, fa, st)
+          : cfg.step == 2 ? launch_emit_fast_behind<2>(kp, ea, fa, st)
+                          : launch_emit_fast_behind<4>(kp, ea, fa, st);
     else if (cfg.step == 1) rcl = launch_emit_fast<1, false, 6>(kp, ea, fa, st);
     else if (cfg.step == 2) rcl = launch_emit_fast<2, false, 6>(kp, ea, fa, st);
     else rcl = launch_emit_fast<4, false, 6>(kp, ea, fa, st);
diff --git a/image_to_pointcloud_b200/csrc/d2pc_emit_dev.cuh b/image_to_pointcloud_b200/csrc/d2pc_emit_dev.cuh
--- a/image_to_pointcloud_b200/csrc/d2pc_emit_dev.cuh
+++ b/image_to_pointcloud_b200/csrc/d2pc_emit_dev.cuh
@@ -143,6 +143,31 @@
 #pragma unroll
   for (int i = 0; i < (int)(sizeof(NormParams) / 8); ++i) dst[i] = __ldcg(src + i);
   return np_;
+}
+
+__device__ __forceinline__ const NormParams *await_frame_norm(const FrameState *fs, uint32_t *abort_flag,
+                                                              NormParams &s_norm, uint32_t &s_go) {
+  const int tid = threadIdx.x;
+  const uint32_t *line = reinterpret_cast<const uint32_t *>(&fs->norm);
+  uint32_t go = 0u;
+  for (int attempt = 0; attempt < 2 && go == 0u; ++attempt) {
+    if (tid < 32) {
+      const uint32_t w = ld_relaxed_u32(line + tid);
+      const uint32_t st = __shfl_sync(0xffffffffu, w, kStatusWord);
+      if (st == (uint32_t)D2PC_FRAME_READY && tid < kStatusWord) reinterpret_cast<uint32_t *>(&s_norm)[tid] = w;
+      if (tid == 0) s_go = st == (uint32_t)D2PC_FRAME_READY ? 1u : (st == (uint32_t)D2PC_FRAME_PENDING ? 0u : 3u);
+    }
+    __syncthreads();
+    go = s_go;
+    if (go == 0u) {
+      __syncthreads();
+      if (tid == 0) s_go = spin_until(line + kStatusWord, abort_flag, [&](uint32_t x) { return x != (uint32_t)D2PC_FRAME_PENDING; }) ? 0u : 2u;
+      __syncthreads();
+      go = s_go;
+      __syncthreads();
+    }
+  }
+  return go == 1u ? &s_norm : nullptr;
 }
 
 constexpr size_t kEmitStageBytes = 2 * ((size_t)kEmitTile * 3 + 4) * sizeof(float);
@@ -309,14 +334,22 @@
   return true;
 }
 
-template <int STEP, bool MASK, bool BOUNDS, int MIN_BLOCKS>
+template <int STEP, bool MASK, bool BOUNDS, int MIN_BLOCKS, bool BEHIND = false>
 __global__ void __launch_bounds__(kEmitThreads, MIN_BLOCKS) emit_fast_kernel(KParams kp, EmitArgs ea, FastArgs fa) {
   extern __shared__ __align__(16) float s_stage[];
   __shared__ EmitSmall es;
   const uint32_t t = blockIdx.x;
   const uint32_t b = t / fa.tiles_per_frame, tile = t - b * fa.tiles_per_frame;
-  if (kp.state[b].status != D2PC_FRAME_READY) return;
-  emit_fast_tile<STEP, MASK, BOUNDS>(kp, ea, fa, b, tile, s_stage, es, [&]() { return &kp.state[b].norm; });
+  if constexpr (BEHIND) {
+    __shared__ NormParams s_norm;
+    __shared__ uint32_t s_go;
+    const NormParams *np_ = await_frame_norm(kp.state + b, sched_abort_flag(kp), s_norm, s_go);
+    if (np_ == nullptr) return;
+    emit_fast_tile<STEP, MASK, BOUNDS>(kp, ea, fa, b, tile, s_stage, es, [&]() { return np_; });
+  } else {
+    if (kp.state[b].status != D2PC_FRAME_READY) return;
+    emit_fast_tile<STEP, MASK, BOUNDS>(kp, ea, fa, b, tile, s_stage, es, [&]() { return &kp.state[b].norm; });
+  }
 }
 
 
diff --git a/image_to_pointcloud_b200/csrc/d2pc_path.cu b/image_to_pointcloud_b200/csrc/d2pc_path.cu
--- a/image_to_pointcloud_b200/csrc/d2pc_path.cu
+++ b/image_to_pointcloud_b200/csrc/d2pc_path.cu
@@ -87,28 +87,7 @@
   const uint32_t f = g - (uint32_t)sp.D;
   if (f >= (uint32_t)sp.F) return;
   if (TRACE && tid == 0) atomicMin(trace_slot(kp, f, 6), global_ns());
-  auto norm_fn = [&]() -> const NormParams * {
-    const uint32_t *line = reinterpret_cast<const uint32_t *>(&kp.state[f].norm);
-    uint32_t go = 0u;
-    for (int attempt = 0; attempt < 2 && go == 0u; ++attempt) {
-      if (tid < 32) {
-        const uint32_t w = ld_relaxed_u32(line + tid);
-        const uint32_t st = __shfl_sync(0xffffffffu, w, kStatusWord);
-        if (st == (uint32_t)D2PC_FRAME_READY && tid < kStatusWord) reinterpret_cast<uint32_t *>(&s_norm)[tid] = w;
-        if (tid == 0) s_go = st == (uint32_t)D2PC_FRAME_READY ? 1u : (st == (uint32_t)D2PC_FRAME_PENDING ? 0u : 3u);
-      }
-      __syncthreads();
-      go = s_go;
-      if (go == 0u) {
-        __syncthreads();
-        if (tid == 0) s_go = spin_until(line + kStatusWord, abort_flag, [&](uint32_t x) { return x != (uint32_t)D2PC_FRAME_PENDING; }) ? 0u : 2u;
-        __syncthreads();
-        go = s_go;
-        __syncthreads();
-      }
-    }
-    return go == 1u ? &s_norm : nullptr;
-  };
+  auto norm_fn = [&]() { return await_frame_norm(kp.state + f, abort_flag, s_norm, s_go); };
   emit_fast_tile<1, false, BOUNDS>(kp, ea, fa, f, e, reinterpret_cast<float *>(s_dyn), s_emit, norm_fn);
   if (TRACE) {
     __syncthreads();
@@ -126,6 +105,7 @@
   cudaStream_t s_aux[kMaxAux];
   cudaStream_t s_emit[kMaxEmit];
   std::vector<cudaEvent_t> events;
+  bool pdl;
   cudaGraphExec_t exec;
   std::vector<unsigned char> key;
 };
@@ -257,6 +237,10 @@
   cudaEvent_t ev_fork = p->events[0];
   cudaEvent_t *ev_stats = &p->events[1], *ev_emit = &p->events[1 + n_sub], *ev_scan = &p->events[1 + 2 * n_sub];
   const bool stagger = overlap && n_aux > 1 && env_int("D2PC_PATH_STAGGER", 0, 0, 1) != 0;
+  const int pdl = (p->pdl && n_sub == 1 && !(cfg.use_z_range || cfg.drop_nonfinite) && !cfg.want_bounds &&
+                   stats_overlap_ok(kp, kStatsSample | kStatsScanSelect))
+                      ? env_int("D2PC_PATH_PDL", kOverlapSelect | kOverlapEmit, 0, 3)
+                      : 0;
   if ((rc = taps_launch(kp, s_main)) != D2PC_OK) return rc;
   if (sample_first) {
     if ((rc = stats_launch(kp, s_main, kStatsSample)) != D2PC_OK) return rc;
@@ -279,14 +263,15 @@
       if ((rc = stats_launch(ks, s_stats, kStatsScan)) != D2PC_OK) return rc;
       PATH_CUDA(cudaEventRecord(ev_scan[k], s_stats));
       if ((rc = stats_launch(ks, s_stats, kStatsSelect)) != D2PC_OK) return rc;
-    } else if ((rc = stats_launch(ks, s_stats, sample_first ? kStatsScanSelect : (kStatsSample | kStatsScanSelect))) != D2PC_OK)
+    } else if ((rc = stats_launch(ks, s_stats, sample_first ? kStatsScanSelect : (kStatsSample | kStatsScanSelect),
+                                  pdl)) != D2PC_OK)
       return rc;
     if (overlap) {
       PATH_CUDA(cudaEventRecord(ev_stats[k], s_stats));
       PATH_CUDA(cudaStreamWaitEvent(s_em, ev_stats[k], 0));
     }
     if ((rc = emit_launch(cfg, ks, slice_emit_args(ea, kp.g, b0), a.d_bounds ? a.d_bounds + 6 * (size_t)b0 : nullptr,
-                          s_em, 0, nullptr, nullptr)) != D2PC_OK)
+                          s_em, 0, nullptr, nullptr, (pdl & kOverlapEmit) != 0)) != D2PC_OK)
       return rc;
     if (overlap) PATH_CUDA(cudaEventRecord(ev_emit[k], s_em));
   }
@@ -299,6 +284,34 @@
   return D2PC_OK;
 }
 
+}
+
+namespace {
+__global__ void pdl_probe_kernel() {}
+bool pdl_capture_supported(cudaStream_t s) {
+  cudaGraph_t graph = nullptr;
+  cudaGraphExec_t exec = nullptr;
+  bool ok = cudaStreamBeginCapture(s, cudaStreamCaptureModeThreadLocal) == cudaSuccess;
+  if (ok) {
+    pdl_probe_kernel<<<1, 32, 0, s>>>();
+    cudaLaunchAttribute attr[1];
+    attr[0].id = cudaLaunchAttributeProgrammaticStreamSerialization;
+    attr[0].val.programmaticStreamSerializationAllowed = 1;
+    cudaLaunchConfig_t lc = {};
+    lc.gridDim = dim3(1);
+    lc.blockDim = dim3(32);
+    lc.stream = s;
+    lc.attrs = attr;
+    lc.numAttrs = 1;
+    const bool launched = cudaLaunchKernelEx(&lc, pdl_probe_kernel) == cudaSuccess;
+    ok = cudaStreamEndCapture(s, &graph) == cudaSuccess && launched;
+  }
+  if (ok) ok = cudaGraphInstantiate(&exec, graph, 0) == cudaSuccess;
+  if (exec) cudaGraphExecDestroy(exec);
+  if (graph) cudaGraphDestroy(graph);
+  (void)cudaGetLastError();
+  return ok;
+}
 }
 
 extern "C" int d2pc_path_create(D2pcPath **path) {
@@ -306,6 +319,7 @@
   *path = nullptr;
   D2pcPath *p = new D2pcPath();
   p->exec = nullptr;
+  p->pdl = false;
   p->s_cap = nullptr;
   for (int i = 0; i < kMaxAux; ++i) p->s_aux[i] = nullptr;
   for (int i = 0; i < kMaxEmit; ++i) p->s_emit[i] = nullptr;
@@ -323,6 +337,7 @@
   }
   int rc = stats_prepare();
   if (rc) { d2pc_path_destroy(p); return rc; }
+  p->pdl = pdl_capture_supported(p->s_cap);
   *path = p;
   return D2PC_OK;
 }
diff --git a/image_to_pointcloud_b200/csrc/d2pc_stats.cu b/image_to_pointcloud_b200/csrc/d2pc_stats.cu
--- a/image_to_pointcloud_b200/csrc/d2pc_stats.cu
+++ b/image_to_pointcloud_b200/csrc/d2pc_stats.cu
@@ -271,15 +271,24 @@
   scan_flush(&sh.pqueue[0][0], (qaddr - q0) / (uint32_t)(kScanThreads * 4), Uf[0], Lf[1], fs, kp, b, sh.flush);
 }
 
-template <int PT>
+__device__ __forceinline__ void count_scanned(const KParams &kp, int b, uint32_t tiles) {
+  __threadfence();
+  __syncthreads();
+  if (threadIdx.x == 0) atomicAdd(&kp.sel[b].scan_done, tiles);
+}
+
+template <int PT, bool COUNT>
 __global__ void __launch_bounds__(kScanThreads) scan_native_kernel(KParams kp, int vec_ok) {
   extern __shared__ __align__(16) unsigned char s_dyn[];
+  if (COUNT) launch_dependents();
   scan_tile<PT>(kp, blockIdx.y, blockIdx.x, vec_ok, *reinterpret_cast<ScanTileSmemT<PT> *>(s_dyn));
-}
-
-template <int PT, int TPC, int MINB>
+  if (COUNT) count_scanned(kp, blockIdx.y, 1u);
+}
+
+template <int PT, int TPC, int MINB, bool COUNT>
 __global__ void __launch_bounds__(kScanThreads, MINB) scan_native_multi_kernel(KParams kp, int vec_ok) {
   extern __shared__ __align__(16) unsigned char s_dyn[];
+  if (COUNT) launch_dependents();
   ScanTileSmemT<PT> &sm = *reinterpret_cast<ScanTileSmemT<PT> *>(s_dyn);
   constexpr int kPx = PT * kScanThreads;
   const int tid = threadIdx.x, b = blockIdx.y;
@@ -328,6 +337,7 @@
     scan_flush(&sm.pq[0][0], (qaddr - q0) / (uint32_t)(kScanThreads * 4), U0, L1, fs, kp, b, sm.flush);
     __syncthreads();
   }
+  if (COUNT) count_scanned(kp, b, min((uint32_t)TPC, ntiles - t0));
 }
 
 __global__ void __launch_bounds__(kScanThreads) scan_gather_kernel(KParams kp, int vec_ok) {
@@ -373,9 +383,19 @@
   scan_flush(&sh.pqueue[0][0], (qaddr - q0) / (uint32_t)(kScanThreads * 4), Uf[0], Lf[1], fs, kp, b, sh.flush);
 }
 
+template <bool WAIT>
 __global__ void __launch_bounds__(kSelectThreads, 2) select_kernel(KParams kp) {
   extern __shared__ uint32_t s_sel[];
   __shared__ SelectSmall ss;
+  if (WAIT) {
+    __shared__ uint32_t s_go;
+    launch_dependents();
+    const uint32_t ntiles = (kp.g.P + (uint32_t)kTilePx - 1u) / (uint32_t)kTilePx;
+    if (threadIdx.x == 0)
+      s_go = spin_until(&kp.sel[blockIdx.y].scan_done, sched_abort_flag(kp), [&](uint32_t v) { return v >= ntiles; }) ? 1u : 0u;
+    __syncthreads();
+    if (!s_go) return;
+  }
   select_bracket(kp, blockIdx.y, blockIdx.x, s_sel, ss);
 }
 
@@ -666,22 +686,47 @@
   const size_t sample_smem = (size_t)(4u << kSelBits) * sizeof(uint32_t);
   cudaError_t e = cudaFuncSetAttribute(sample_kernel<true>, cudaFuncAttributeMaxDynamicSharedMemorySize, (int)sample_smem);
   if (e == cudaSuccess)
-    e = cudaFuncSetAttribute(select_kernel, cudaFuncAttributeMaxDynamicSharedMemorySize, (int)(kSelectSmemWords * sizeof(uint32_t)));
+    e = cudaFuncSetAttribute(select_kernel<false>, cudaFuncAttributeMaxDynamicSharedMemorySize, (int)(kSelectSmemWords * sizeof(uint32_t)));
+  if (e == cudaSuccess)
+    e = cudaFuncSetAttribute(select_kernel<true>, cudaFuncAttributeMaxDynamicSharedMemorySize, (int)(kSelectSmemWords * sizeof(uint32_t)));
   if (e == cudaSuccess)
     e = cudaFuncSetAttribute(sample_kernel<false>, cudaFuncAttributeMaxDynamicSharedMemorySize, (int)sample_smem);
-  if (e == cudaSuccess)
-    e = cudaFuncSetAttribute(scan_native_kernel<kTilePerThread>, cudaFuncAttributeMaxDynamicSharedMemorySize, (int)sizeof(ScanTileSmem));
-  if (e == cudaSuccess)
-    e = cudaFuncSetAttribute(scan_native_multi_kernel<kTilePerThread, 2, 4>, cudaFuncAttributeMaxDynamicSharedMemorySize, (int)sizeof(ScanTileSmem));
-  if (e == cudaSuccess)
-    e = cudaFuncSetAttribute(scan_native_multi_kernel<kTilePerThread, 4, 4>, cudaFuncAttributeMaxDynamicSharedMemorySize, (int)sizeof(ScanTileSmem));
+  const void *scans[] = {(const void *)scan_native_kernel<kTilePerThread, false>, (const void *)scan_native_kernel<kTilePerThread, true>,
+                         (const void *)scan_native_multi_kernel<kTilePerThread, 2, 4, false>,
+                         (const void *)scan_native_multi_kernel<kTilePerThread, 2, 4, true>,
+                         (const void *)scan_native_multi_kernel<kTilePerThread, 4, 4, false>,
+                         (const void *)scan_native_multi_kernel<kTilePerThread, 4, 4, true>};
+  for (const void *f : scans)
+    if (e == cudaSuccess) e = cudaFuncSetAttribute(f, cudaFuncAttributeMaxDynamicSharedMemorySize, (int)sizeof(ScanTileSmem));
   if (e == cudaSuccess)
     e = cudaFuncSetAttribute(stats_ordered_kernel, cudaFuncAttributeMaxDynamicSharedMemorySize, (int)sizeof(ScanTileSmem));
   if (e != cudaSuccess) return record_cuda_error(e);
   return D2PC_OK;
 }
 
-int stats_launch(KParams kp, cudaStream_t st, int phases) {
+static bool ordered_chosen(const KParams &kp, int phases) {
+  const char *mode = getenv("D2PC_STATS_ORDERED");
+  const bool ordered = (phases & kStatsScanSelect) == kStatsScanSelect && (mode ? atoi(mode) != 0 : kp.batch <= 2);
+  return kp.g.native && kp.g.P > (uint32_t)kSortCap && ordered;
+}
+
+static uint32_t select_parts(const KParams &kp) {
+  const char *cm = getenv("D2PC_SELECT_COOP");
+  uint32_t K = 296u / (2u * (uint32_t)kp.batch);
+  if (K > 16u) K = 16u;
+  if (kp.g.P >= 4u * 1024u * 1024u && K < 4u) K = 4u;
+  if (K < 4u) K = 0u;
+  if (cm) K = (uint32_t)atoi(cm);
+  if (K > 64u) K = 64u;
+  return (K >= 2u && kp.g.P > (uint32_t)kSortCap) ? K : 0u;
+}
+
+bool stats_overlap_ok(const KParams &kp, int phases) {
+  return kp.g.native && (phases & kStatsScanSelect) == kStatsScanSelect && !ordered_chosen(kp, phases) &&
+         select_parts(kp) == 0u;
+}
+
+int stats_launch(KParams kp, cudaStream_t st, int phases, int overlap) {
   const int nb = kp.batch;
   if (!kp.g.native && resize_is_generic(kp.g.h, kp.g.w)) {
     const uint32_t blocks = (kp.g.P + 255u) / 256u;
@@ -700,9 +745,7 @@
     D2PC_CHECK_LAUNCH();
   }
   if (!(phases & kStatsScanSelect)) return D2PC_OK;
-  const char *mode = getenv("D2PC_STATS_ORDERED");
-  const bool ordered = (phases & kStatsScanSelect) == kStatsScanSelect && (mode ? atoi(mode) != 0 : nb <= 2);
-  if (kp.g.native && kp.g.P > (uint32_t)kSortCap && ordered) {
+  if (ordered_chosen(kp, phases)) {
     const uint32_t ns = (kp.g.P + kTilePx - 1) / kTilePx;
     uint32_t K = (kp.cand_cap + kStatsSliceCap - 1u) / kStatsSliceCap;
     K = K < 4u ? 4u : (K > 64u ? 64u : K);
@@ -713,15 +756,24 @@
       return D2PC_OK;
     }
   }
+  if (!stats_overlap_ok(kp, phases)) overlap = 0;
   if (!(phases & kStatsScan)) {
   } else if (kp.g.native) {
     const uint32_t nt = (kp.g.P + kTilePx - 1) / kTilePx;
     const char *te = getenv("D2PC_SCAN_TPC");
     const unsigned long long tiles = (unsigned long long)nt * (unsigned long long)nb;
     const int tpc = te ? atoi(te) : (tiles >= 4ull * 1184ull ? 4 : (tiles >= 2ull * 1184ull ? 2 : 1));
-    if (tpc >= 4) scan_native_multi_kernel<kTilePerThread, 4, 4><<<dim3((nt + 3) / 4, nb), kScanThreads, sizeof(ScanTileSmem), st>>>(kp, vec_ok);
-    else if (tpc >= 2) scan_native_multi_kernel<kTilePerThread, 2, 4><<<dim3((nt + 1) / 2, nb), kScanThreads, sizeof(ScanTileSmem), st>>>(kp, vec_ok);
-    else scan_native_kernel<kTilePerThread><<<dim3(nt, nb), kScanThreads, sizeof(ScanTileSmem), st>>>(kp, vec_ok);
+    const dim3 g4((nt + 3) / 4, nb), g2((nt + 1) / 2, nb), g1(nt, nb);
+    const size_t sm = sizeof(ScanTileSmem);
+    if (overlap) {
+      if (tpc >= 4) scan_native_multi_kernel<kTilePerThread, 4, 4, true><<<g4, kScanThreads, sm, st>>>(kp, vec_ok);
+      else if (tpc >= 2) scan_native_multi_kernel<kTilePerThread, 2, 4, true><<<g2, kScanThreads, sm, st>>>(kp, vec_ok);
+      else scan_native_kernel<kTilePerThread, true><<<g1, kScanThreads, sm, st>>>(kp, vec_ok);
+    } else {
+      if (tpc >= 4) scan_native_multi_kernel<kTilePerThread, 4, 4, false><<<g4, kScanThreads, sm, st>>>(kp, vec_ok);
+      else if (tpc >= 2) scan_native_multi_kernel<kTilePerThread, 2, 4, false><<<g2, kScanThreads, sm, st>>>(kp, vec_ok);
+      else scan_native_kernel<kTilePerThread, false><<<g1, kScanThreads, sm, st>>>(kp, vec_ok);
+    }
   } else {
     bool tiled = (kp.g.W & 3) == 0;
     for (int32_t v0 = 0; tiled && v0 < kp.g.H; v0 += kRzRows) {
@@ -738,19 +790,28 @@
   }
   D2PC_CHECK_LAUNCH();
   if (phases & kStatsSelect) {
-    const char *cm = getenv("D2PC_SELECT_COOP");
-    uint32_t K = 296u / (2u * (uint32_t)nb);
-    if (K > 16u) K = 16u;
-    if (kp.g.P >= 4u * 1024u * 1024u && K < 4u) K = 4u;
-    if (K < 4u) K = 0u;
-    if (cm) K = (uint32_t)atoi(cm);
-    if (K > 64u) K = 64u;
-    if (K >= 2u && kp.g.P > (uint32_t)kSortCap) {
+    const uint32_t K = select_parts(kp);
+    if (overlap & kOverlapSelect) {
+      cudaLaunchAttribute attr[1];
+      attr[0].id = cudaLaunchAttributeProgrammaticStreamSerialization;
+      attr[0].val.programmaticStreamSerializationAllowed = 1;
+      cudaLaunchConfig_t lc = {};
+      lc.gridDim = dim3(2, nb);
+      lc.blockDim = dim3(kSelectThreads);
+      lc.dynamicSmemBytes = (size_t)kSelectSmemWords * sizeof(uint32_t);
+      lc.stream = st;
+      lc.attrs = attr;
+      lc.numAttrs = 1;
+      const cudaError_t e = cudaLaunchKernelEx(&lc, select_kernel<true>, kp);
+      if (e != cudaSuccess) return record_cuda_error(e);
+    } else if (overlap) {
+      select_kernel<true><<<dim3(2, nb), kSelectThreads, (size_t)kSelectSmemWords * sizeof(uint32_t), st>>>(kp);
+    } else if (K != 0u) {
       select_a_kernel<<<dim3(K, 2, nb), kCoopThreads, kCoopSmemWords * sizeof(uint32_t), st>>>(kp, K);
       D2PC_CHECK_LAUNCH();
       select_c_kernel<<<dim3(K, 2, nb), kCoopThreads, kCoopSmemWords * sizeof(uint32_t), st>>>(kp, K);
     } else {
-      select_kernel<<<dim3(2, nb), kSelectThreads, (size_t)kSelectSmemWords * sizeof(uint32_t), st>>>(kp);
+      select_kernel<false><<<dim3(2, nb), kSelectThreads, (size_t)kSelectSmemWords * sizeof(uint32_t), st>>>(kp);
     }
     D2PC_CHECK_LAUNCH();
   }
diff --git a/image_to_pointcloud_b200/csrc/d2pc_stats_dev.cuh b/image_to_pointcloud_b200/csrc/d2pc_stats_dev.cuh
--- a/image_to_pointcloud_b200/csrc/d2pc_stats_dev.cuh
+++ b/image_to_pointcloud_b200/csrc/d2pc_stats_dev.cuh
@@ -319,35 +319,6 @@
   }
 }
 
-constexpr uint32_t kSpinLimit = 1u << 19;
-
-__device__ __forceinline__ uint32_t ld_relaxed_u32(const uint32_t *p) {
-  uint32_t v;
-  asm volatile("ld.relaxed.gpu.global.u32 %0, [%1];" : "=r"(v) : "l"(p) : "memory");
-  return v;
-}
-__device__ __forceinline__ uint32_t ld_acquire_u32(const uint32_t *p) {
-  uint32_t v;
-  asm volatile("ld.acquire.gpu.global.u32 %0, [%1];" : "=r"(v) : "l"(p) : "memory");
-  return v;
-}
-
-template <typename Pred>
-__device__ __forceinline__ bool spin_until(const uint32_t *p, uint32_t *abort_flag, Pred pred) {
-  uint32_t spins = 0, ns = 128;
-  while (!pred(ld_relaxed_u32(p))) {
-    __nanosleep(ns);
-    if (ns < 2048u) ns <<= 1;
-    if (++spins > kSpinLimit || ((spins & 15u) == 0u && ld_relaxed_u32(abort_flag))) {
-      atomicExch(abort_flag, 1u);
-      return false;
-    }
-  }
-  (void)ld_acquire_u32(p);
-  return true;
-}
-
-__device__ __forceinline__ uint32_t *sched_abort_flag(const KParams &kp) { return kp.sched + 32u * kSchedQueues; }
 
 constexpr uint32_t kSliceCap = 6144;
 
```
